# lucazanella/AnomalyCLIP

Measured on AMD Instinct MI355X. Metric: frames/sec encoded + anomaly-scored (whole node), ViT-B/16 224^2, higher is better.
Workload: dtype f32 (bf16x6 operands, exact 24-bit split, f32 accumulate); 1 GPU; configs[2]: synthetic 224x224 RGB frames, ViT-B/16 encode + selector + axial temporal head + eval post-processing; step = one 512-frame clip per GPU in ONE ViT launch, UCF-Crime head config, random-init weights; text features cached (frozen prompts): leg text_recomputed_every_step runs the text encoder in every step; leg vit_chunk_256 = the config's literal batch of 256; vit_chunk=512, precision=auto

## Files before the change

anomalyclip_amd/_lib.py:

```python
from __future__ import annotations

import ctypes as C
import os
import threading

from . import _build

c_void_p, c_int32, c_int64, c_float, c_size_t = C.c_void_p, C.c_int32, C.c_int64, C.c_float, C.c_size_t

ACX_F32, ACX_BF16, BF16X3, BF16X3P = 0, 1, 2, 3
BF16X2P, ACX_F16, F16X2P = 4, 5, 6
PREC_F32, PREC_BF16, PREC_F32X6, PREC_F32X3, PREC_F16X3 = 0, 1, 2, 3, 4
PREC_BF16X6 = 5
PREC_F32X6_LN16 = 6
PREC_F32X6_R16 = 7
ACT_NONE, ACT_QUICKGELU, ACT_LEAKYRELU, ACT_RELU, ACT_RESRELU = 0, 1, 2, 3, 4
ACT_GELU = 5
AMAP_IDENTITY, AMAP_CONV3X3, AMAP_TESTTILE, AMAP_TILETABLE = 0, 1, 2, 3
NORM_LAYER, NORM_CHAN = 0, 1
OPT_RING_MIN_TILES, OPT_SK_MAX_M, OPT_TN_P256_MIN_ROWS, OPT_X6_CUS, OPT_X6_TAIL_SPLIT = 1, 2, 3, 4, 5
OPT_X6_STRIP_TAIL, OPT_X6_MIN_TILES, OPT_LN_RIDER, OPT_ATTN_F32IN, OPT_CLS_FOLD = 6, 7, 8, 9, 10
ACX_F64, ACX_I64 = 16, 17
COMM_SUM, COMM_MAX, COMM_MIN = 0, 1, 2
COMM_ID_BYTES = 128
SAB_ROUTE_UNSUPPORTED, SAB_ROUTE_TEXT_MFMA, SAB_ROUTE_TEXT_BLOCK, SAB_ROUTE_TEXT_ROWS = 0, 1, 2, 3
SAB_ROUTE_AXIAL_MFMA, SAB_ROUTE_AXIAL_MFMA_PADDED, SAB_ROUTE_GENERIC = 4, 5, 6
AXF_ROUTE_UNSUPPORTED, AXF_ROUTE_PADDED_MFMA, AXF_ROUTE_EXACT_MFMA, AXF_ROUTE_THREAD_PER_ROW = 0, 1, 2, 3
GEMM_ROUTE_NONE, GEMM_ROUTE_X6_TAIL_SPLIT, GEMM_ROUTE_SK, GEMM_ROUTE_X6, GEMM_ROUTE_S64, GEMM_ROUTE_P256, GEMM_ROUTE_W8 = 0, 1, 2, 3, 4, 5, 6
GEMM_ROUTE_W8_CONV, GEMM_ROUTE_RING, GEMM_ROUTE_P8, GEMM_ROUTE_DMA_CONV, GEMM_ROUTE_DMA, GEMM_ROUTE_GENERIC = 7, 8, 9, 10, 11, 12
GEMM_REDUCE_NONE, GEMM_REDUCE_LAUNCH, GEMM_REDUCE_COUNTERS = 0, 1, 2
TN_ROUTE_NONE, TN_ROUTE_W8, TN_ROUTE_P256, TN_ROUTE_X6_256x256, TN_ROUTE_X6_256x128, TN_ROUTE_X6_128x256 = 0, 1, 2, 3, 4, 5
TF_LN_ROWS, TF_LN_PLANES, TF_LN_RIDDEN, TF_LN_CLS = 0, 1, 2, 3
TF_GEMM_ROWS, TF_GEMM_X6 = 0, 1
TF_BUF_NONE, TF_BUF_SPLITK, TF_BUF_H, TF_BUF_QKV, TF_BUF_MLP = 0, 1, 2, 3, 4
TF_ATT_F32, TF_ATT_BF16, TF_ATT_X3_PANEL, TF_ATT_P3N, TF_ATT_P3F, TF_ATT_CLS, TF_ATT_CLS_FOLD = 0, 1, 2, 3, 4, 5, 6


class GemmDesc(C.Structure):
    _fields_ = [
        ("A", c_void_p), ("W", c_void_p), ("C", c_void_p),
        ("M", c_int32), ("N", c_int32), ("K", c_int32),
        ("lda", c_int32), ("ldw", c_int32), ("ldc", c_int32),
        ("a_dtype", c_int32), ("c_dtype", c_int32), ("prec", c_int32),
        ("bias", c_void_p), ("act", c_int32),
        ("residual", c_void_p), ("ldr", c_int32),
        ("a_sub", c_void_p),
        ("amap", c_int32), ("gn", c_int32), ("gl", c_int32), ("cin", c_int32), ("seg", c_int32),
        ("pos0", c_void_p), ("pos1", c_void_p),
        ("workspace", c_void_p), ("workspace_bytes", c_size_t),
        ("zero_page", c_void_p), ("a_act", c_int32), ("gelu_grad_of", c_void_p), ("ldg", c_int32),
        ("a_norm_w", c_void_p), ("a_norm_b", c_void_p), ("a_norm_eps", c_float),
        ("counters", c_void_p), ("n_counters", c_int32),
        ("tile_table", c_void_p),
        ("pairs", c_int32), ("panels", c_int32), ("a_plane_stride", c_int64), ("w_plane_stride", c_int64),
        ("c_plane_rows", c_int64), ("out_scale", c_float), ("c_scale", c_float),
    ]


class GemmScratch(C.Structure):
    _fields_ = [("workspace_bytes", c_size_t), ("counters", c_int32)]


class GemmRoute(C.Structure):
    _fields_ = [("route", c_int32), ("ksplit", c_int32), ("reduce", c_int32), ("reserved", c_int32), ("tiles", c_int64)]


class GemmTnRoute(C.Structure):
    _fields_ = [(n, c_int32) for n in ("kernel", "splits", "rows_per_split", "tiles", "reduce", "clears_zero_page")]


class TfProduct(C.Structure):
    _fields_ = [(n, c_int32) for n in ("kernel", "c_dtype", "scratch", "ln_job")]


class TfLayerPlan(C.Structure):
    _fields_ = [(n, c_int32) for n in ("ln1", "ln1_dtype", "ln2", "ln2_dtype")] + \
               [(n, TfProduct) for n in ("in_proj", "out_proj", "fc", "proj")] + \
               [(n, c_int32) for n in ("att", "att_products", "split_att", "split_mlp", "pruned", "reserved")]


class LnJob(C.Structure):
    _fields_ = [("w", c_void_p), ("b", c_void_p), ("y", c_void_p), ("y_dtype", c_int32), ("eps", c_float), ("mode", c_int32),
                ("y_scale", c_float)]


class BlockWeights(C.Structure):
    _fields_ = [(n, c_void_p) for n in (
        "ln1_w", "ln1_b", "ln2_w", "ln2_b", "in_proj_w", "in_proj_b", "out_proj_w", "out_proj_b",
        "fc_w", "fc_b", "proj_w", "proj_b",
        "in_proj_w_bf16", "out_proj_w_bf16", "fc_w_bf16", "proj_w_bf16")]


class VitWeights(C.Structure):
    _fields_ = [
        ("conv1_w", c_void_p), ("conv1_w_bf16", c_void_p),
        ("class_embedding", c_void_p), ("positional_embedding", c_void_p),
        ("ln_pre_w", c_void_p), ("ln_pre_b", c_void_p), ("ln_post_w", c_void_p), ("ln_post_b", c_void_p),
        ("proj_t", c_void_p), ("proj_t_bf16", c_void_p),
# ... 15 lines not shown
    _fields_ = [("src", c_void_p), ("dst", c_void_p), ("rows", c_int32), ("cols", c_int32), ("src_ld", c_int32),
                ("dst_ld", c_int32), ("transpose", c_int32), ("reserved", c_int32)]


class VitDesc(C.Structure):
    _fields_ = [(n, c_int32) for n in ("resolution", "patch", "width", "layers", "heads", "embed_dim", "prec", "act")]


class ResnetConv(C.Structure):
    _fields_ = [("w", c_void_p), ("b", c_void_p), ("w3", c_void_p)]


class ResnetBlock(C.Structure):
    _fields_ = [("conv1", ResnetConv), ("conv2", ResnetConv), ("conv3", ResnetConv), ("downsample", ResnetConv)]


class ResnetWeights(C.Structure):
    _fields_ = [("stem", ResnetConv * 3), ("blocks", C.POINTER(ResnetBlock)), ("positional_embedding", c_void_p),
                ("q_w", c_void_p), ("q_b", c_void_p), ("kv_w", c_void_p), ("kv_b", c_void_p), ("c_w", c_void_p), ("c_b", c_void_p),
                ("kv_w3", c_void_p)]


class ResnetBn(C.Structure):
    _fields_ = [("weight", c_void_p), ("bias", c_void_p), ("running_mean", c_void_p), ("running_var", c_void_p),
                ("num_batches_tracked", c_void_p)]


class ResnetBlockBn(C.Structure):
    _fields_ = [("bn1", ResnetBn), ("bn2", ResnetBn), ("bn3", ResnetBn), ("downsample", ResnetBn)]


class ResnetTrainBn(C.Structure):
    _fields_ = [("stem", ResnetBn * 3), ("blocks", C.POINTER(ResnetBlockBn)), ("eps", c_float), ("momentum", c_float)]


class ResnetDesc(C.Structure):
    _fields_ = [("resolution", c_int32), ("width", c_int32), ("layers", c_int32 * 4), ("heads", c_int32), ("output_dim", c_int32),
                ("prec", c_int32)]


class JpegInfo(C.Structure):
    _fields_ = [(n, c_int32) for n in ("width", "height", "ncomp", "hmax", "vmax", "mcus_x", "mcus_y", "restart_interval")] + \
               [(n, c_int32 * 4) for n in ("comp_h", "comp_v", "comp_tq", "comp_td", "comp_ta", "comp_width", "comp_height",
                                           "blocks_wide", "blocks_high")] + \
               [("coef_offset", c_int64 * 4), ("coef_elems", c_int64), ("scan_offset", c_int64),
                ("qtab", (C.c_uint16 * 64) * 4), ("qtab_present", C.c_uint8 * 4), ("huff_present", (C.c_uint8 * 4) * 2),
                ("huff_bits", ((C.c_uint8 * 17) * 4) * 2), ("huff_vals", ((C.c_uint8 * 256) * 4) * 2)]


class VizGeom(C.Structure):
    _fields_ = [(n, c_int32) for n in ("Hc", "Wc", "H", "W", "fx", "fy", "fw", "fh", "border", "bx", "by", "bh", "bar_pitch", "bar_w",
                                       "C1", "sx", "sy", "sw", "sh", "cursor_w", "T")] + [("threshold", c_float)]


class JpegHuff(C.Structure):
    _fields_ = [("present", (C.c_uint8 * 4) * 2), ("bits", ((C.c_uint8 * 17) * 4) * 2), ("vals", ((C.c_uint8 * 256) * 4) * 2),
                ("td", C.c_uint8 * 4), ("ta", C.c_uint8 * 4)]


_SIGS = {
    "acx_version": (C.c_int, []),
    "acx_create": (C.c_int, [C.POINTER(c_void_p), C.c_int]),
    "acx_destroy": (None, [c_void_p]),
    "acx_last_error": (C.c_char_p, [c_void_p]),
    "acx_set_option": (C.c_int, [c_void_p, c_int32, c_int64]),
    "acx_get_option": (C.c_int, [c_void_p, c_int32, C.POINTER(c_int64)]),
    "acx_gemm": (C.c_int, [c_void_p, C.POINTER(GemmDesc), c_void_p]),
    "acx_gemm_scratch": (C.c_int, [c_void_p, C.POINTER(GemmDesc), c_int32, C.POINTER(GemmScratch)]),
    "acx_gemm_route": (C.c_int, [c_void_p, C.POINTER(GemmDesc), C.POINTER(GemmRoute)]),
    "acx_gemm_ln": (C.c_int, [c_void_p, C.POINTER(GemmDesc), C.POINTER(LnJob), c_void_p]),
    "acx_gemm_ln_plan": (c_int64, [c_int32, c_int32, c_int32, c_int32, c_int32, C.c_double, C.POINTER(c_int64)]),
    "acx_layernorm": (C.c_int, [c_void_p, c_void_p, c_int64, c_void_p, c_void_p, c_void_p, c_int64, c_int32,
                                c_int64, c_int32, c_float, c_int32, c_void_p]),
    "acx_layernorm_scaled": (C.c_int, [c_void_p, c_void_p, c_int64, c_void_p, c_void_p, c_void_p, c_int64, c_int32, c_float, c_int32,
                                       c_float, c_void_p]),
    "acx_attention": (C.c_int, [c_void_p, c_void_p, c_int64, c_void_p, c_int64, c_int32, c_int32, c_int32,
                                c_int32, c_void_p]),
    "acx_attention_bf16": (C.c_int, [c_void_p, c_void_p, c_int64, c_void_p, c_int64, c_int32, c_int32, c_int32, c_void_p]),
    "acx_attention_x3": (C.c_int, [c_void_p, c_void_p, c_int64, c_void_p, c_int64, c_int32, c_int32, c_int32, c_void_p]),
    "acx_attention_p3": (C.c_int, [c_void_p, c_void_p, c_void_p, c_int32, c_int32, c_int32, c_void_p]),
    "acx_attention_p3n": (C.c_int, [c_void_p, c_void_p, c_void_p, c_int32, c_int32, c_int32, c_int32, c_void_p]),
    "acx_attention_p3f": (C.c_int, [c_void_p, c_void_p, c_int64, c_void_p, c_int32, c_int32, c_int32, c_void_p]),
    "acx_attention_p3f16": (C.c_int, [c_void_p, c_void_p, c_int64, c_void_p, c_float, c_int32, c_int32, c_int32, c_void_p]),
    "acx_attention_x3_panel": (C.c_int, [c_void_p, c_void_p, c_int64, c_void_p, c_int64, c_int32, c_int32, c_int32, c_void_p]),
    "acx_attention_cls": (C.c_int, [c_void_p, c_void_p, c_int64, c_void_p, c_int64, c_int32, c_int32, c_int32, c_void_p]),
    "acx_attention_cls_fold_workspace_bytes": (c_size_t, [c_int32, c_int32]),
    "acx_attention_cls_fold": (C.c_int, [c_void_p, c_void_p, c_void_p, c_void_p, c_float, c_void_p, c_void_p, c_void_p, c_int64, c_void_p,
                                         c_int64, c_int32, c_int32, c_int32, c_int32, c_void_p, c_size_t, c_void_p]),
    "acx_vit_patches": (C.c_int, [c_void_p, c_void_p, c_void_p, c_int32, c_int32, c_int32, c_int32, c_void_p]),
    "acx_vit_embed": (C.c_int, [c_void_p] * 7 + [c_int32, c_int32, c_int32, c_void_p]),
    "acx_resnet_stem_im2col": (C.c_int, [c_void_p, c_void_p, c_void_p, c_int32, c_int32, c_void_p]),
    "acx_avgpool2_nhwc": (C.c_int, [c_void_p, c_void_p, c_void_p, c_int32, c_int32, c_int32, c_int32, c_void_p]),
    "acx_attnpool_tokens": (C.c_int, [c_void_p, c_void_p, c_void_p, c_void_p, c_int32, c_int32, c_int32, c_void_p]),
    "acx_resnet_workspace_bytes": (c_size_t, [C.POINTER(ResnetDesc), c_int32]),
    "acx_bn_apply_nhwc": (C.c_int, [c_void_p, c_void_p, c_void_p, c_void_p, c_void_p, c_void_p, c_void_p, c_void_p, c_int64, c_int32,
                                    c_int32, c_float, c_int32, c_void_p, c_void_p]),
    "acx_resnet_train_workspace_bytes": (c_size_t, [C.POINTER(ResnetDesc), c_int32]),
    "acx_resnet_encode_train": (C.c_int, [c_void_p, C.POINTER(ResnetDesc), C.POINTER(ResnetWeights), C.POINTER(ResnetTrainBn), c_void_p,
                                          c_int32, c_void_p, c_void_p, c_size_t, c_void_p]),
    "acx_resnet_encode": (C.c_int, [c_void_p, C.POINTER(ResnetDesc), C.POINTER(ResnetWeights), c_void_p, c_int32, c_void_p,
                                    c_void_p, c_size_t, c_void_p]),
    "acx_vit_workspace_bytes": (c_size_t, [C.POINTER(VitDesc), c_int32]),
    "acx_vit_encode": (C.c_int, [c_void_p, C.POINTER(VitDesc), C.POINTER(VitWeights), c_void_p, c_int32, c_void_p,
                                 c_void_p, c_size_t, c_void_p]),
    "acx_vit_encode_ln16": (C.c_int, [c_void_p, C.POINTER(VitDesc), C.POINTER(VitWeights), c_void_p, c_void_p, c_int32, c_void_p,
                                      c_void_p, c_size_t, c_void_p]),
    "acx_vit_encode_r16": (C.c_int, [c_void_p, C.POINTER(VitDesc), C.POINTER(VitWeights), c_void_p, c_void_p, c_int32, c_void_p,
                                     c_void_p, c_size_t, c_void_p]),
    "acx_transformer_workspace_bytes": (c_size_t, [c_int32, c_int32]),
    "acx_transformer_workspace_bytes_prec": (c_size_t, [c_int32, c_int32, c_int32]),
    "acx_transformer_forward": (C.c_int, [c_void_p, c_void_p, c_int32, c_int32, c_int32, c_int32, c_int32, c_int32,
                                          c_int32, C.POINTER(BlockWeights), c_void_p, c_size_t, c_void_p]),
    "acx_transformer_forward_act": (C.c_int, [c_void_p, c_void_p, c_int32, c_int32, c_int32, c_int32, c_int32, c_int32,
                                              c_int32, c_int32, C.POINTER(BlockWeights), c_void_p, c_size_t, c_void_p]),
    "acx_transformer_plan": (C.c_int, [c_void_p] + [c_int32] * 10 + [C.POINTER(TfLayerPlan)]),
    "acx_text_directions": (C.c_int, [c_void_p, c_void_p, c_void_p, c_void_p, c_int32, c_int32, c_int32, c_void_p]),
    "acx_selector_project": (C.c_int, [c_void_p, c_void_p, c_void_p, c_void_p, c_void_p, c_int64, c_int32, c_int32,
                                       c_void_p]),
    "acx_probe_mfma": (C.c_int, [c_void_p, c_int32, c_int32, c_int32, c_void_p, C.POINTER(C.c_double), c_void_p]),
    "acx_probe_copy": (C.c_int, [c_void_p, c_void_p, c_void_p, c_int64, c_void_p]),
    "acx_split_bf16x3_multi": (C.c_int, [c_void_p, c_int32, c_void_p, c_void_p, c_void_p, c_void_p]),
    "acx_probe_read": (C.c_int, [c_void_p, c_void_p, c_int64, c_void_p, c_void_p]),
    "acx_comm_unique_id": (C.c_int, [c_void_p, c_size_t]),
    "acx_comm_init": (C.c_int, [c_void_p, c_int32, c_int32, c_void_p]),
    "acx_comm_destroy": (C.c_int, [c_void_p]),
    "acx_comm_info": (C.c_int, [c_void_p, C.POINTER(c_int32), C.POINTER(c_int32)]),
    "acx_allreduce": (C.c_int, [c_void_p, c_void_p, c_int64, c_int32, c_int32, c_void_p]),
    "acx_allgather": (C.c_int, [c_void_p, c_void_p, c_void_p, c_int64, c_int32, c_void_p]),
    "acx_bn_workspace_bytes": (c_size_t, [c_int64, c_int32]),
    "acx_bn_combine": (C.c_int, [c_void_p, c_void_p, c_int32, c_int32, c_void_p, c_void_p, c_void_p, c_void_p, c_void_p]),
    "acx_bn_stats": (C.c_int, [c_void_p, c_void_p, c_int64, c_int32, c_void_p, c_void_p, c_void_p, c_void_p, c_size_t, c_void_p]),
    "acx_selector_project_stats": (C.c_int, [c_void_p, c_void_p, c_void_p, c_void_p, c_void_p, c_int64, c_int32, c_int32,
                                             c_void_p, c_void_p, c_void_p, c_void_p, c_size_t, c_void_p]),
    "acx_selector_bn": (C.c_int, [c_void_p, c_void_p, c_void_p, c_void_p, c_void_p, c_int64, c_int64, c_int32,
                                  c_float, c_void_p]),
    "acx_axial_attention": (C.c_int, [c_void_p, c_void_p, c_void_p, c_int32, c_int32, c_int32, c_int32, c_int32,
                                      c_int32, c_void_p]),
    "acx_axial_attention_route": (C.c_int, [c_void_p] + [c_int32] * 6),
    "acx_cls_head": (C.c_int, [c_void_p] * 8 + [c_int64, c_int32, c_int32, c_int32, c_int32, c_void_p]),
    "acx_cls_head_tiles": (C.c_int, [c_void_p] * 8 + [c_int64, c_int32, c_int32, c_int32, c_void_p, c_void_p]),
    "acx_class_probs": (C.c_int, [c_void_p, c_void_p, c_void_p, c_void_p, c_int64, c_int32, c_void_p]),
    "acx_prompt_embed": (C.c_int, [c_void_p] * 6 + [c_int32] * 6 + [c_void_p]),
    "acx_gather_rows": (C.c_int, [c_void_p, c_void_p, c_void_p, c_void_p, c_int64, c_int32, c_void_p]),
    "acx_add_bcast": (C.c_int, [c_void_p, c_void_p, c_void_p, c_void_p, c_int64, c_int64, c_void_p]),
    "acx_concat_features": (C.c_int, [c_void_p] * 5 + [c_int64, c_int32, c_int32, c_int32, c_void_p]),
    "acx_prof_enable": (C.c_int, [c_void_p, C.c_int]),
    "acx_prof_gemm_flops": (C.c_int, [c_void_p, C.POINTER(C.c_double)]),
    "acx_prof_collect": (C.c_int, [c_void_p, C.POINTER(c_int32), C.POINTER(C.c_double)]),
    "acx_prof_gemm_tn": (C.c_int, [c_void_p, C.POINTER(C.c_double), C.POINTER(C.c_double), C.POINTER(c_int32)]),
    "acx_gemm_tn_workspace_bytes": (c_size_t, [c_int32, c_int32, c_int32]),
    "acx_gemm_tn": (C.c_int, [c_void_p, c_void_p, c_int32, c_void_p, c_int32, c_void_p, c_int32, c_int32, c_int32, c_int32,
                              c_void_p, c_int32, c_int32, c_int32, c_int32, c_void_p, c_size_t, c_void_p]),
    "acx_reduce_rows": (C.c_int, [c_void_p, c_void_p, c_void_p, c_int32, c_int32, c_void_p]),
    "acx_layernorm_bwd": (C.c_int, [c_void_p] * 6 + [c_int64, c_int32, c_float, c_int32, c_float, c_void_p, c_void_p]),
    "acx_cls_head_bwd": (C.c_int, [c_void_p] * 10 + [c_int64, c_int32, c_void_p]),
    "acx_act": (C.c_int, [c_void_p, c_void_p, c_void_p, c_void_p, c_int64, c_int32, c_void_p]),
    "acx_leaky_grad_planes": (C.c_int, [c_void_p, c_void_p, c_void_p, c_void_p, c_void_p, c_int64, c_int64, c_void_p]),
    "acx_add": (C.c_int, [c_void_p, c_void_p, c_void_p, c_void_p, c_int64, c_void_p]),
    "acx_transpose": (C.c_int, [c_void_p, c_void_p, c_void_p, c_int32, c_int32, c_void_p]),
    "acx_conv_weight_dx": (C.c_int, [c_void_p, c_void_p, c_void_p, c_int32, c_int32, c_void_p]),
    "acx_seq_attention_bwd": (C.c_int, [c_void_p] * 4 + [c_int32] * 7 + [c_void_p, c_void_p]),
    "acx_seq_attention_bwd_route": (C.c_int, [c_void_p] + [c_int32] * 8),
    "acx_pos_grad": (C.c_int, [c_void_p] * 5 + [c_int32] * 4 + [c_void_p]),
    "acx_bn_bwd_stats": (C.c_int, [c_void_p] * 4 + [c_int64, c_int32, c_void_p, c_size_t, c_void_p]),
    "acx_bn_bwd_apply": (C.c_int, [c_void_p] * 6 + [c_int32, c_int64, c_int64, c_int32, c_float, c_void_p, c_void_p]),
    "acx_axpby": (C.c_int, [c_void_p, c_void_p, c_void_p, c_int32, c_float, c_float, c_void_p]),
    "acx_colsum_partials": (C.c_int, [c_void_p, c_void_p, c_int32, c_void_p, c_int64, c_int32, c_int32, c_void_p]),
    "acx_text_directions_bwd": (C.c_int, [c_void_p] * 5 + [c_int32] * 3 + [c_void_p]),
    "acx_select_idx": (C.c_int, [c_void_p] * 7 + [c_int32] * 7 + [c_void_p]),
    "acx_gather_segments": (C.c_int, [c_void_p] * 4 + [c_int32] * 5 + [c_void_p]),
    "acx_scatter_segments": (C.c_int, [c_void_p] * 4 + [c_int32] * 5 + [c_void_p]),
    "acx_mil_loss_one": (C.c_int, [c_void_p] * 13 + [c_size_t] + [c_int32] * 6 + [c_void_p, c_void_p, c_void_p, c_void_p]),
    "acx_mil_loss_bn": (C.c_int, [c_void_p] * 14 + [c_size_t, c_void_p, c_size_t] + [c_int32] * 6 + [c_void_p, c_void_p, c_void_p, c_void_p]),
    "acx_mil_loss_bn_fits": (C.c_int, [c_void_p] + [c_int32] * 5),
    "acx_selector_tail": (C.c_int, [c_void_p, c_void_p, c_void_p, c_int32] + [c_void_p] * 7 + [c_float, c_float, c_void_p, c_int64] +
                          [c_void_p] * 6 + [c_int32] * 7 + [c_float, c_void_p]),
    "acx_selector_tail_fits": (C.c_int, [c_void_p] + [c_int32] * 6),
    "acx_text_directions_bwd_parts": (C.c_int, [c_void_p] * 4 + [c_int32, c_int64, c_void_p] + [c_int32] * 3 + [c_void_p]),
    "acx_adamw": (C.c_int, [c_void_p] * 5 + [c_int64] + [c_float] * 5 + [c_int32, c_void_p]),
    "acx_multi_axpy": (C.c_int, [c_void_p, c_int32, C.POINTER(c_void_p), C.POINTER(c_void_p), C.POINTER(c_int64), c_float, c_void_p]),
    "acx_adamw_multi": (C.c_int, [c_void_p, c_int32] + [C.POINTER(c_void_p)] * 4 + [C.POINTER(c_int64), C.POINTER(C.c_double),
                                  C.POINTER(C.c_double), C.c_double, C.c_double, C.c_double, c_int32, c_void_p]),
    "acx_row_parts": (c_int64, [c_int64]),
    "acx_prep_multi": (C.c_int, [c_void_p, c_int32, c_void_p, c_void_p]),
    "acx_multi_copy": (C.c_int, [c_void_p, c_int32, C.POINTER(c_void_p), C.POINTER(c_void_p), C.POINTER(c_int64), c_void_p]),
    "acx_adamw_hyper": (C.c_int, [c_int32, C.POINTER(C.c_double), C.POINTER(C.c_double), C.c_double, C.c_double, c_int32,
                                  C.POINTER(c_float)]),
    "acx_adamw_multi_dev": (C.c_int, [c_void_p, c_int32] + [C.POINTER(c_void_p)] * 4 + [C.POINTER(c_int64), c_void_p, c_float,
                                      C.c_double, C.c_double, C.c_double, c_void_p]),
    "acx_grad_norm_workspace_bytes": (c_size_t, [c_int32, c_int64]),
    "acx_grad_norm": (C.c_int, [c_void_p, c_int32, C.POINTER(c_void_p), C.POINTER(c_int64), c_float, c_float, c_void_p, c_void_p,
# ... 147 lines not shown
```

anomalyclip_amd/components/clip_vit.py:

```python
from __future__ import annotations

import ctypes as C
import math
from typing import List, Optional

import torch
from torch import nn

from .. import _lib as L
from .. import ops

PRECISIONS = {"auto": L.PREC_F32X6, "f32": L.PREC_F32, "bf16": L.PREC_BF16, "f32x6": L.PREC_F32X6, "bf16x3": L.PREC_F32X3,
              "f16x3": L.PREC_F16X3}
F16X3_WSCALE = 1024.0
ACTS = {"quick_gelu": L.ACT_QUICKGELU, "gelu": L.ACT_GELU}


def check_act(act, precision: Optional[str] = None, arch: Optional[str] = None, key: str = "act") -> int:
    if act not in ACTS:
        raise ValueError(f"{key}={act!r}: one of {', '.join(ACTS)}")
    if act == "gelu" and precision == "bf16":
        raise ValueError(f"{key}='gelu' with precision='bf16': the exact GELU runs on the f32-accurate paths only ('auto', 'f32', 'f32x6', 'f16x3')")
    if act == "gelu" and arch is not None and str(arch).startswith("RN"):
        raise ValueError(f"{key}='gelu' with arch={arch!r}: the CLIP ResNet encoders have no GELU (the activation is the ViT MLP's)")
    return ACTS[act]


_NEW_ARCH_VISION = {(224, 32, 768), (224, 14, 1024), (336, 14, 1024)}


def check_vit_precision(precision: str, tokens: int, width: int, arch: str, resolution: int = 0, patch: int = 0):
    if precision == "bf16x6":
        raise ValueError(f"precision 'bf16x6' is a ResNet encoder precision: for {arch} 'auto' already is that arithmetic (every large "
                         "product as an f32-accurate six-product GEMM of bf16 planes); use 'auto'")
    if precision not in PRECISIONS:
        raise ValueError(f"unknown precision {precision!r}: one of {', '.join(PRECISIONS)}")
    if precision in ("bf16x3", "f16x3") and (tokens > 224 or (resolution, patch, width) in _NEW_ARCH_VISION):
        raise ValueError(f"precision {precision!r} is not available for {arch} ({tokens} tokens, width {width}): it is stated for the "
                         "ViT-B/16 geometry, whose planes attention (192 < tokens <= 208) it needs; use 'auto', 'f32' or 'bf16'")
    if tokens > 1024:
        raise ValueError(f"{arch} has {tokens} tokens per frame: the attention kernels take at most 1024")


LN16_TARGET = 2.0 ** 14
LN16_SCALE_RANGE = (2.0 ** -20, 2.0 ** 20)
LN16_WEIGHT_MAX = 2.0 ** 15 / F16X3_WSCALE


def ln16_scale(bound: float) -> Optional[float]:
    if not (math.isfinite(bound) and bound > 0.0):
        return None
    s = 2.0 ** (math.frexp(LN16_TARGET / bound)[1] - 1)
    while s * bound > LN16_TARGET:
        s *= 0.5
    return s if LN16_SCALE_RANGE[0] <= s <= LN16_SCALE_RANGE[1] else None


@torch.no_grad()
def r16_bounds(ln_w, ln_b, w, b):
    g, be, w64, b64 = ln_w.detach().double(), ln_b.detach().double(), w.detach().double(), b.detach().double()
    D = g.numel()
    l1 = (g.abs() * float(D - 1) ** 0.5 + be.abs()).max() * w64.abs().sum(1) + b64.abs()
    l2 = float(D) ** 0.5 * (w64 * g).pow(2).sum(1).sqrt() + (w64 @ be + b64).abs()
    return l1, l2


@torch.no_grad()
def _range_proofs(blocks, width: int):
    vals = []
    D = width
    root = float(D - 1) ** 0.5
    for b in blocks:
        for ln in (b.ln_1, b.ln_2):
            g, be = ln.weight.detach().double(), ln.bias.detach().double()
            vals.append((g.abs() * root + be.abs()).max())
            vals.append((g.abs() + be.abs()).sum())
        for wt in (b.attn.in_proj_weight, b.mlp.c_fc.weight):
            vals.append(wt.detach().abs().max().double())
            vals.append(wt.detach().double().abs().sum())
        for ln, wt, bias in ((b.ln_1, b.attn.in_proj_weight[2 * D:], b.attn.in_proj_bias[2 * D:]), (b.ln_2, b.mlp.c_fc.weight, b.mlp.c_fc.bias)):
            l1, l2 = r16_bounds(ln.weight, ln.bias, wt, bias)
            vals.append(torch.minimum(l1, l2).max() + 0.0 * (l1.sum() + l2.sum()))
        for wt in (b.attn.out_proj.weight, b.mlp.c_proj.weight):
            vals.append(wt.detach().abs().max().double())
            vals.append(wt.detach().double().abs().sum())
    if not vals:
        return None, None
    v = torch.stack(vals).tolist()
    ln16: Optional[List[float]] = []
    r16: Optional[List[float]] = []
    for i in range(0, len(v), 14):
        b1, f1, b2, f2, w1, g1, w2, g2, ba, bh, w3, g3, w4, g4 = v[i:i + 14]
        if ln16 is not None:
            s1, s2 = ln16_scale(b1), ln16_scale(b2)
            if not all(math.isfinite(t) for t in (f1, f2, g1, g2)) or not (w1 <= LN16_WEIGHT_MAX and w2 <= LN16_WEIGHT_MAX) or s1 is None or s2 is None:
                ln16 = r16 = None
            else:
                ln16 += [s1, s2]
        if r16 is not None:
            sa, sh = ln16_scale(ba), ln16_scale(bh)
            if not all(math.isfinite(t) for t in (g3, g4)) or not (w3 <= LN16_WEIGHT_MAX and w4 <= LN16_WEIGHT_MAX) or sa is None or sh is None:
                r16 = None
            else:
                r16 += [sa, sh]
    return ln16, r16


def ln16_scales(blocks, width: int) -> Optional[List[float]]:
    return _range_proofs(blocks, width)[0]


def r16_scales(blocks, width: int) -> Optional[List[float]]:
    return _range_proofs(blocks, width)[1]


HEAD_MAX_AXIS = 128
HEAD_DIMS = (16, 32, 64)
LAYERNORM_WIDTHS = (64, 128, 256, 512, 640, 768, 1024)


def check_head_geometry(num_segments, seg_length, emb_size, heads, dim_heads=None, num_topk=None, num_bottomk=None,
                        kernel_widths: bool = True):
    for key, v in (("num_segments", num_segments), ("seg_length", seg_length)):
        if not isinstance(v, int) or isinstance(v, bool) or v < 1 or v > HEAD_MAX_AXIS:
            raise ValueError(f"{key}={v!r}: the axial attention kernels take an integer axis length of 1 ... {HEAD_MAX_AXIS}")
    if not isinstance(heads, int) or heads < 1:
        raise ValueError(f"heads={heads!r}: need an integer >= 1")
    if kernel_widths:
        if emb_size not in LAYERNORM_WIDTHS:
            raise ValueError(f"emb_size={emb_size!r}: the LayerNorm kernels take the widths {', '.join(map(str, LAYERNORM_WIDTHS))}")
        if dim_heads:
            if dim_heads not in HEAD_DIMS:
                raise ValueError(f"dim_heads={dim_heads!r}: the attention kernels take a head dimension of 16, 32 or 64")
        elif emb_size % heads or emb_size // heads not in HEAD_DIMS:
            raise ValueError(f"heads={heads!r} with emb_size={emb_size}: the head dimension emb_size / heads = {emb_size / heads:g} must "
                             "be 16, 32 or 64 (or set dim_heads)")
    for key, v in (("num_topk", num_topk), ("num_bottomk", num_bottomk)):
        if v is not None and v > num_segments:
            raise ValueError(f"{key}={v} selects more segments than num_segments={num_segments}")


class LayerNorm(nn.Module):
    def __init__(self, width: int):
        super().__init__()
        self.weight = nn.Parameter(torch.ones(width))
        self.bias = nn.Parameter(torch.zeros(width))

    def forward(self, x: torch.Tensor) -> torch.Tensor:
        shp = x.shape
        return ops.layernorm(x.reshape(-1, shp[-1]).contiguous(), self.weight, self.bias).view(shp)


class _Linear(nn.Module):

    def __init__(self, fin: int, fout: int, bias: bool = True):
        super().__init__()
        self.weight = nn.Parameter(torch.empty(fout, fin))
        self.bias = nn.Parameter(torch.zeros(fout)) if bias else None
        nn.init.normal_(self.weight, std=fin ** -0.5)


class _MHA(nn.Module):

    def __init__(self, width: int):
        super().__init__()
        self.in_proj_weight = nn.Parameter(torch.empty(3 * width, width))
        self.in_proj_bias = nn.Parameter(torch.zeros(3 * width))
        self.out_proj = _Linear(width, width)
        nn.init.normal_(self.in_proj_weight, std=width ** -0.5)


class _MLP(nn.Module):
    def __init__(self, width: int):
        super().__init__()
        self.c_fc = _Linear(width, 4 * width)
        self.c_proj = _Linear(4 * width, width)


class ResidualAttentionBlock(nn.Module):
    def __init__(self, width: int, heads: int):
        super().__init__()
        self.attn = _MHA(width)
        self.ln_1 = LayerNorm(width)
        self.mlp = _MLP(width)
        self.ln_2 = LayerNorm(width)


class Transformer(nn.Module):

    def __init__(self, width: int, layers: int, heads: int, causal: bool = False, act: str = "quick_gelu"):
        super().__init__()
        if width != heads * 64:
            raise ValueError("libacx attention kernels are built for head dim 64 (every CLIP ViT/text tower)")
        self.width, self.layers, self.heads, self.causal = width, layers, heads, causal
        check_act(act)
        self.act = act
# ... 13 lines not shown
            w = arr[i]
            w.ln1_w, w.ln1_b = b.ln_1.weight.data_ptr(), b.ln_1.bias.data_ptr()
            w.ln2_w, w.ln2_b = b.ln_2.weight.data_ptr(), b.ln_2.bias.data_ptr()
            w.in_proj_w, w.in_proj_b = b.attn.in_proj_weight.data_ptr(), b.attn.in_proj_bias.data_ptr()
            w.out_proj_w, w.out_proj_b = b.attn.out_proj.weight.data_ptr(), b.attn.out_proj.bias.data_ptr()
            w.fc_w, w.fc_b = b.mlp.c_fc.weight.data_ptr(), b.mlp.c_fc.bias.data_ptr()
            w.proj_w, w.proj_b = b.mlp.c_proj.weight.data_ptr(), b.mlp.c_proj.bias.data_ptr()
            mixed = prec in (L.PREC_F32X6_LN16, L.PREC_F32X6_R16)
            f16w = {"in_proj_w_bf16": mixed, "fc_w_bf16": mixed and ln16_fc, "out_proj_w_bf16": prec == L.PREC_F32X6_R16 and r16[0],
                    "proj_w_bf16": prec == L.PREC_F32X6_R16 and r16[1]}
            if prec in (L.PREC_BF16, L.PREC_F32X6, L.PREC_F32X3, L.PREC_F16X3, L.PREC_F32X6_LN16, L.PREC_F32X6_R16):
                for name, p in (("in_proj_w_bf16", b.attn.in_proj_weight), ("out_proj_w_bf16", b.attn.out_proj.weight),
                                ("fc_w_bf16", b.mlp.c_fc.weight), ("proj_w_bf16", b.mlp.c_proj.weight)):
                    if prec == L.PREC_F16X3 or f16w[name]:
                        t = ops.split_f16x2(p.detach(), panel=True, scale=F16X3_WSCALE)
                    else:
                        t = ops.cast_bf16(p.detach()) if prec == L.PREC_BF16 else ops.split_bf16x3(p.detach(), panel=True)
                    keep.append(t)
                    setattr(w, name, t.data_ptr())
        self._cache = (key, (arr, keep))
        return self._cache[1]

    def forward_(self, x: torch.Tensor, batch: int, seq: int, prec: int = L.PREC_F32) -> torch.Tensor:
        assert x.is_contiguous() and x.dtype == torch.float32 and x.shape == (batch * seq, self.width)
        lib = L.lib()
        nbytes = lib.acx_transformer_workspace_bytes_prec(self.width, batch * seq, prec)
        ws = torch.empty(nbytes, dtype=torch.uint8, device=x.device)
        arr, _keep = self.block_table(prec)
        h = ops._h(x)
        L.check(lib.acx_transformer_forward_act(h, x.data_ptr(), batch, seq, self.width, self.heads, self.layers,
                                                int(self.causal), prec, ACTS[self.act], arr, ws.data_ptr(), nbytes, ops._stream()), h)
        return x


class _Conv(nn.Module):
    def __init__(self, width: int, patch: int):
        super().__init__()
        self.weight = nn.Parameter(torch.empty(width, 3, patch, patch))
        nn.init.normal_(self.weight, std=(3 * patch * patch) ** -0.5)


class VisionTransformer(nn.Module):

    def __init__(self, input_resolution: int, patch_size: int, width: int, layers: int, heads: int,
                 output_dim: int, precision: str = "auto", chunk: int = 512, streams: int = 1, arch: Optional[str] = None,
                 act: str = "quick_gelu"):
        super().__init__()
        self.arch = arch or f"ViT(width {width}, patch {patch_size}, resolution {input_resolution})"
        check_act(act, precision)
        self.act = act
        self.input_resolution, self.patch_size, self.output_dim = input_resolution, patch_size, output_dim
        self.width, self.layers, self.heads = width, layers, heads
        self.conv1 = _Conv(width, patch_size)
        scale = width ** -0.5
        self.class_embedding = nn.Parameter(scale * torch.randn(width))
        self.positional_embedding = nn.Parameter(scale * torch.randn((input_resolution // patch_size) ** 2 + 1, width))
        self.ln_pre = LayerNorm(width)
        self.transformer = Transformer(width, layers, heads, act=act)
        self.ln_post = LayerNorm(width)
        self.proj = nn.Parameter(scale * torch.randn(width, output_dim))
        self.precision = precision
        self.check_precision()
        self.chunk = chunk
        self.streams = streams
        self._wcache = None
        self._ln16 = None
        self._ws: Optional[torch.Tensor] = None
        self._ws2: Optional[torch.Tensor] = None
        self._side = None

    @property
    def tokens(self) -> int:
        return (self.input_resolution // self.patch_size) ** 2 + 1

    def check_precision(self):
        check_vit_precision(self.precision, self.tokens, self.width, self.arch, self.input_resolution, self.patch_size)
        check_act(self.act, self.precision)

    @torch.no_grad()
    def f16x3_range_report(self) -> dict:
        D = self.width
        lim = 65504.0
        worst = {"weight_planes": 0.0, "layernorm_out": 0.0, "attention_out": 0.0, "mlp_hidden": 0.0}

        def ln_bound(ln):
            return float((ln.weight.abs() * (D - 1) ** 0.5 + ln.bias.abs()).max())
        mats = [self.conv1.weight.reshape(D, -1)]
        for b in self.transformer.resblocks:
            l1, l2 = ln_bound(b.ln_1), ln_bound(b.ln_2)
            wv, bv = b.attn.in_proj_weight[2 * D:], b.attn.in_proj_bias[2 * D:]
            worst["layernorm_out"] = max(worst["layernorm_out"], l1, l2)
            worst["attention_out"] = max(worst["attention_out"], float((wv.abs().sum(1) * l1 + bv.abs()).max()))
            worst["mlp_hidden"] = max(worst["mlp_hidden"], float((b.mlp.c_fc.weight.abs().sum(1) * l2 + b.mlp.c_fc.bias.abs()).max()))
            mats += [b.attn.in_proj_weight, b.attn.out_proj.weight, b.mlp.c_fc.weight, b.mlp.c_proj.weight]
        worst["weight_planes"] = F16X3_WSCALE * max(float(m.abs().max()) for m in mats)
        margin = min(lim / max(v, 1e-30) for v in worst.values())
        return {"bounds": worst, "fp16_max": lim, "margin": margin, "safe": margin > 1.0}

    def _ln16_bound(self):
        key = (ops.WEIGHT_EPOCH[0],) + tuple((p.data_ptr(), p._version) for p in self.parameters())
        if self._ln16 is not None and self._ln16[0] == key:
            return self._ln16[1]
        res = None
        if self.width in (768, 1024) and self.layers > 1 and L.exports("acx_vit_encode_ln16"):
            scales, wide = _range_proofs(self.transformer.resblocks, self.width)
            if scales is not None:
                fc16 = ops.transformer_plan(64, 197, 768, 12, 2, prec=L.PREC_F32X6_LN16, prune_last=True)[0]["ln2_dtype"] == L.F16X2P
                r16 = None
                if wide is not None and L.exports("acx_vit_encode_r16"):
                    rec = ops.transformer_plan(64, self.tokens, self.width, self.heads, 2, prec=L.PREC_F32X6_R16, prune_last=True)[0]
                    fmt = (rec["reserved"] == L.F16X2P, rec["fc"]["c_dtype"] == L.F16X2P)
                    if any(fmt):
                        s4 = [t for l in range(self.layers) for t in (scales[2 * l], scales[2 * l + 1], wide[2 * l], wide[2 * l + 1])]
                        r16 = (s4, (C.c_float * len(s4))(*s4), fmt)
                res = (scales, (C.c_float * len(scales))(*scales), fc16, r16)
        self._ln16 = (key, res)
        return res

    def ln16_resolution(self) -> Optional[List[float]]:
        res = self._ln16_bound()
        return None if res is None else res[0]

    def r16_resolution(self) -> Optional[List[float]]:
        res = self._ln16_bound()
        return None if res is None or res[3] is None else res[3][0]

    def _weights(self, prec: int, ln16_fc: bool = True, r16=(True, True)):
        key = (prec, bool(ln16_fc), bool(r16[0]), bool(r16[1]), ops.WEIGHT_EPOCH[0]) + tuple((p.data_ptr(), p._version) for p in self.parameters())
        if self._wcache is not None and self._wcache[0] == key:
            return self._wcache[1]
        keep = []
        w = L.VitWeights()
        conv = self.conv1.weight.detach().reshape(self.width, -1).contiguous()
        proj_t = self.proj.detach().t().contiguous()
        keep += [conv, proj_t]
        w.conv1_w, w.proj_t = conv.data_ptr(), proj_t.data_ptr()
        if prec == L.PREC_BF16:
            cb, pb = ops.cast_bf16(conv), ops.cast_bf16(proj_t)
            keep += [cb, pb]
            w.conv1_w_bf16, w.proj_t_bf16 = cb.data_ptr(), pb.data_ptr()
        elif prec in (L.PREC_F32X6, L.PREC_F32X3, L.PREC_F16X3, L.PREC_F32X6_LN16, L.PREC_F32X6_R16) and self.patch_size % 4 == 0:
            cb = ops.split_f16x2(conv, panel=True, scale=F16X3_WSCALE) if prec == L.PREC_F16X3 else ops.split_bf16x3(conv, panel=True)
            keep.append(cb)
            w.conv1_w_bf16 = cb.data_ptr()
        w.class_embedding = self.class_embedding.data_ptr()
        w.positional_embedding = self.positional_embedding.data_ptr()
        w.ln_pre_w, w.ln_pre_b = self.ln_pre.weight.data_ptr(), self.ln_pre.bias.data_ptr()
        w.ln_post_w, w.ln_post_b = self.ln_post.weight.data_ptr(), self.ln_post.bias.data_ptr()
        arr, keep2 = self.transformer.block_table(prec, ln16_fc, r16)
        w.blocks = C.cast(arr, C.POINTER(L.BlockWeights))
        keep += [arr, keep2]
        self._wcache = (key, (w, keep))
        return self._wcache[1]

    @torch.no_grad()
    def forward(self, x: torch.Tensor) -> torch.Tensor:
        assert x.dim() == 4 and x.shape[1] == 3 and x.shape[2] == x.shape[3] == self.input_resolution
        self.check_precision()
        x = x.contiguous().float()
        prec = PRECISIONS[self.precision]
        lib = L.lib()
        bound = self._ln16_bound() if self.precision == "auto" and x.is_cuda else None
        ln16_fc, r16 = True, (True, True)
        if bound is not None and bound[3] is not None:
            prec = L.PREC_F32X6_R16
            ln16_fc = bound[2]
            _s4, sc4, r16 = bound[3]
            encode = lambda *a: lib.acx_vit_encode_r16(a[0], a[1], a[2], sc4, *a[3:])
        elif bound is not None:
            prec = L.PREC_F32X6_LN16
            _scales, sc, ln16_fc, _ = bound
            encode = lambda *a: lib.acx_vit_encode_ln16(a[0], a[1], a[2], sc, *a[3:])
        else:
            encode = lib.acx_vit_encode
        d = L.VitDesc(self.input_resolution, self.patch_size, self.width, self.layers, self.heads, self.output_dim, prec, ACTS[self.act])
        w, _keep = self._weights(prec, ln16_fc, r16)
        F = x.shape[0]
        out = torch.empty(F, self.output_dim, dtype=torch.float32, device=x.device)
        chunk = min(self.chunk, F)
        nbytes = lib.acx_vit_workspace_bytes(C.byref(d), chunk)
        if self._ws is None or self._ws.numel() < nbytes or self._ws.device != x.device:
            self._ws = torch.empty(nbytes, dtype=torch.uint8, device=x.device)
        h = ops._h(x)
        if self.streams == 2 and chunk >= 32 and x.is_cuda:
            return self._forward_two_streams(x, out, d, w, chunk, nbytes, h, encode)
        s = ops._stream()
        for f0 in range(0, F, chunk):
            n = min(chunk, F - f0)
            L.check(encode(h, C.byref(d), C.byref(w), x[f0:f0 + n].data_ptr(), n, out[f0:f0 + n].data_ptr(),
                           self._ws.data_ptr(), self._ws.numel(), s), h)
        return out

    def _forward_two_streams(self, x, out, d, w, chunk, nbytes, h, encode):
        F = x.shape[0]
        half = (chunk + 1) // 2
        if self._ws2 is None or self._ws2.numel() < nbytes or self._ws2.device != x.device:
            self._ws2 = torch.empty(nbytes, dtype=torch.uint8, device=x.device)
        if self._side is None or self._side[0].device != x.device:
            s0 = torch.cuda.Stream(device=x.device)
            self._side = (s0, ops.side_stream_beside(s0, x.device))
        cur = torch.cuda.current_stream()
        wss = (self._ws, self._ws2)
        for st in self._side:
            st.wait_stream(cur)
        k = 0
        for f0 in range(0, F, half):
            n = min(half, F - f0)
            st, ws = self._side[k % 2], wss[k % 2]
            with torch.cuda.stream(st):
                L.check(encode(h, C.byref(d), C.byref(w), x[f0:f0 + n].data_ptr(), n, out[f0:f0 + n].data_ptr(),
                               ws.data_ptr(), ws.numel(), st.cuda_stream), h)
            k += 1
        for st in self._side:
            cur.wait_stream(st)
        return out
```

anomalyclip_amd/csrc/acx_api.hip:

```cpp
#include "acx_internal.h"

#include <new>
#include <stdlib.h>

#ifndef ACX_ATTN_F32IN_DEFAULT
#define ACX_ATTN_F32IN_DEFAULT 1
#endif

#ifndef ACX_LN16_FC_DEFAULT
#define ACX_LN16_FC_DEFAULT 1
#endif

#ifndef ACX_R16_OUT_DEFAULT
#define ACX_R16_OUT_DEFAULT 1
#endif
#ifndef ACX_R16_PROJ_DEFAULT
#define ACX_R16_PROJ_DEFAULT 1
#endif

#ifndef ACX_CLS_FOLD_DEFAULT
#define ACX_CLS_FOLD_DEFAULT 1
#endif

thread_local char acx_tls_err[512] = {0};

namespace {
struct TfOpts {
  int x6_min_tiles;
  bool attn_f32in, cls_fold;
  bool ln16_fc;
  bool r16_out, r16_proj;
};
constexpr TfOpts kCreateOpts = {18, ACX_ATTN_F32IN_DEFAULT != 0, ACX_CLS_FOLD_DEFAULT != 0, ACX_LN16_FC_DEFAULT != 0, ACX_R16_OUT_DEFAULT != 0,
                                ACX_R16_PROJ_DEFAULT != 0};
constexpr TfOpts kNoCtxOpts = {512, false, false, ACX_LN16_FC_DEFAULT != 0, ACX_R16_OUT_DEFAULT != 0, ACX_R16_PROJ_DEFAULT != 0};
inline TfOpts tf_opts(const acx_ctx* ctx, bool query) {
  if (!ctx) return query ? kCreateOpts : kNoCtxOpts;
  return {ctx->opt_x6_min_tiles, ctx->opt_attn_f32in != 0, ctx->opt_cls_fold != 0, kCreateOpts.ln16_fc, kCreateOpts.r16_out, kCreateOpts.r16_proj};
}
}

extern "C" int acx_attention_cls(acx_ctx* ctx, const float* qkv, int64_t ldqkv, float* out, int64_t ldo, int32_t batch,
                                 int32_t L, int32_t heads, void* stream);

extern "C" int acx_version(void) { return ACX_VERSION; }

extern "C" int acx_create(acx_ctx** out, int device) {
  if (!out) return acx_fail(nullptr, ACX_E_BADARG, "acx_create: null out%s");
  int n = 0;
  hipError_t e = hipGetDeviceCount(&n);
  if (e != hipSuccess || device < 0 || device >= n) {
    snprintf(acx_tls_err, 512, "acx_create: device %d not available (%s, %d devices)", device,
             e == hipSuccess ? "ok" : hipGetErrorString(e), n);
    return ACX_E_HIP;
  }
  hipDeviceProp_t prop;
  e = hipGetDeviceProperties(&prop, device);
  if (e != hipSuccess) {
    snprintf(acx_tls_err, 512, "acx_create: hipGetDeviceProperties: %s", hipGetErrorString(e));
    return ACX_E_HIP;
  }
  if (strncmp(prop.gcnArchName, "gfx950", 6) != 0) {
    snprintf(acx_tls_err, 512, "acx_create: libacx is built for gfx950 only, device %d is %s", device, prop.gcnArchName);
    return ACX_E_UNSUPPORTED;
  }
  acx_ctx* c = new (std::nothrow) acx_ctx;
  if (!c) return acx_fail(nullptr, ACX_E_HIP, "acx_create: out of host memory%s");
  c->device = device;
  c->multiprocessors = prop.multiProcessorCount;
  c->opt_ring_min_tiles = 512;
  c->opt_sk_max_m = 320;
  c->opt_tn_p256_min_rows = 4096;
  c->opt_x6_cus = 0;
  c->opt_x6_tail = 0;
  c->opt_x6_strip = 1;
  c->opt_ln_rider = 1;
  c->opt_attn_f32in = kCreateOpts.attn_f32in;
  c->opt_cls_fold = kCreateOpts.cls_fold;
  c->comm = nullptr; c->comm_rank = 0; c->comm_world = 0;
  c->opt_x6_min_tiles = kCreateOpts.x6_min_tiles;
  c->err[0] = 0;
  c->prof_on = false;
  c->prof_gemm_only = false;
  c->prof_n = c->prof_created = 0;
  c->prof_gemm_flops = 0.0;
  c->prof_tn_flops = c->prof_tn_ms = 0.0; c->prof_tn_count = 0;
  c->prof_ev = new (std::nothrow) hipEvent_t[2 * ACX_PROF_MAX];
  c->prof_kind = new (std::nothrow) unsigned char[ACX_PROF_MAX];
  *out = c;
  return ACX_OK;
}

extern "C" void acx_destroy(acx_ctx* ctx) {
  if (!ctx) return;
  for (int i = 0; i < 2 * ctx->prof_created; ++i) (void)hipEventDestroy(ctx->prof_ev[i]);
  delete[] ctx->prof_ev;
  delete[] ctx->prof_kind;
  delete ctx;
}

extern "C" int acx_prof_enable(acx_ctx* ctx, int on) {
  if (!ctx || !ctx->prof_ev || !ctx->prof_kind) return acx_fail(ctx, ACX_E_BADARG, "acx_prof_enable: no context%s");
  ctx->prof_on = on != 0;
  ctx->prof_gemm_only = on == 2;
  if (on) { ctx->prof_n = 0; ctx->prof_gemm_flops = 0.0; ctx->prof_tn_flops = 0.0; }
  return ACX_OK;
}

extern "C" int acx_prof_gemm_flops(acx_ctx* ctx, double* flops) {
  if (!ctx || !flops) return acx_fail(ctx, ACX_E_BADARG, "acx_prof_gemm_flops: null pointer%s");
  *flops = ctx->prof_gemm_flops;
  return ACX_OK;
}

extern "C" int acx_prof_gemm_tn(acx_ctx* ctx, double* flops, double* total_ms, int32_t* launches) {
  if (!ctx || !flops || !total_ms || !launches) return acx_fail(ctx, ACX_E_BADARG, "acx_prof_gemm_tn: null pointer%s");
  *flops = ctx->prof_tn_flops; *total_ms = ctx->prof_tn_ms; *launches = ctx->prof_tn_count;
  return ACX_OK;
}

extern "C" int acx_prof_collect(acx_ctx* ctx, int32_t* counts, double* total_ms) {
// ... 15 lines not shown
  }
  ctx->prof_n = 0;
  return ACX_OK;
}

extern "C" int acx_set_option(acx_ctx* ctx, int32_t option, int64_t value) {
  if (!ctx) return acx_fail(ctx, ACX_E_BADARG, "acx_set_option: no context%s");
  switch (option) {
    case ACX_OPT_RING_MIN_TILES:
      if (value < 1) return acx_fail(ctx, ACX_E_BADARG, "acx_set_option: ring_min_tiles must be >= 1%s");
      ctx->opt_ring_min_tiles = (int)value;
      return ACX_OK;
    case ACX_OPT_TN_P256_MIN_ROWS:
      if (value < 1) return acx_fail(ctx, ACX_E_BADARG, "acx_set_option: tn_p256_min_rows must be >= 1%s");
      ctx->opt_tn_p256_min_rows = (int)(value > 0x7fffffff ? 0x7fffffff : value);
      return ACX_OK;
    case ACX_OPT_X6_TAIL_SPLIT:
      ctx->opt_x6_tail = value != 0;
      return ACX_OK;
    case ACX_OPT_X6_STRIP_TAIL:
      if (value < 0 || value > 3) return acx_fail(ctx, ACX_E_BADARG, "acx_set_option: x6_strip_tail is 0 (off), 1 (cost model), 2 or 3 (forced strip width)%s");
      ctx->opt_x6_strip = (int)value;
      return ACX_OK;
    case ACX_OPT_LN_RIDER:
      if (value < 0) return acx_fail(ctx, ACX_E_BADARG, "acx_set_option: ln_rider is 0 (off), 1 (cost model) or a row count%s");
      ctx->opt_ln_rider = (long long)value;
      return ACX_OK;
    case ACX_OPT_ATTN_F32IN:
      ctx->opt_attn_f32in = value != 0;
      return ACX_OK;
    case ACX_OPT_CLS_FOLD:
      ctx->opt_cls_fold = value != 0;
      return ACX_OK;
    case ACX_OPT_X6_MIN_TILES:
      if (value < 1) return acx_fail(ctx, ACX_E_BADARG, "acx_set_option: x6_min_tiles must be >= 1%s");
      ctx->opt_x6_min_tiles = (int)(value > 0x7fffffff ? 0x7fffffff : value);
      return ACX_OK;
    case ACX_OPT_X6_CUS:
      if (value < 0) return acx_fail(ctx, ACX_E_BADARG, "acx_set_option: x6_cus must be >= 0%s");
      ctx->opt_x6_cus = (int)(value > 4096 ? 4096 : value);
      return ACX_OK;
    case ACX_OPT_SK_MAX_M:
      if (value < 0) return acx_fail(ctx, ACX_E_BADARG, "acx_set_option: sk_max_m must be >= 0%s");
      ctx->opt_sk_max_m = (int)value;
      return ACX_OK;
    default:
      return acx_fail(ctx, ACX_E_UNSUPPORTED, "acx_set_option: unknown option %s%ld", "", (long)option);
  }
}

extern "C" int acx_get_option(acx_ctx* ctx, int32_t option, int64_t* value) {
  if (!ctx || !value) return acx_fail(ctx, ACX_E_BADARG, "acx_get_option: no context or no result pointer%s");
  switch (option) {
    case ACX_OPT_RING_MIN_TILES: *value = ctx->opt_ring_min_tiles; return ACX_OK;
    case ACX_OPT_SK_MAX_M: *value = ctx->opt_sk_max_m; return ACX_OK;
    case ACX_OPT_TN_P256_MIN_ROWS: *value = ctx->opt_tn_p256_min_rows; return ACX_OK;
    case ACX_OPT_X6_CUS: *value = ctx->opt_x6_cus; return ACX_OK;
    case ACX_OPT_X6_TAIL_SPLIT: *value = ctx->opt_x6_tail; return ACX_OK;
    case ACX_OPT_X6_STRIP_TAIL: *value = ctx->opt_x6_strip; return ACX_OK;
    case ACX_OPT_X6_MIN_TILES: *value = ctx->opt_x6_min_tiles; return ACX_OK;
    case ACX_OPT_LN_RIDER: *value = ctx->opt_ln_rider; return ACX_OK;
    case ACX_OPT_ATTN_F32IN: *value = ctx->opt_attn_f32in; return ACX_OK;
    case ACX_OPT_CLS_FOLD: *value = ctx->opt_cls_fold; return ACX_OK;
    default:
      return acx_fail(ctx, ACX_E_UNSUPPORTED, "acx_get_option: unknown option %s%ld", "", (long)option);
  }
}

extern "C" const char* acx_last_error(acx_ctx* ctx) { return ctx ? ctx->err : acx_tls_err; }

namespace {

inline size_t al(size_t x) { return (x + 255) & ~(size_t)255; }

struct TfWs {
  char *h, *qkv, *att, *mlp, *splitk;
  char *hp, *mp;
  char* qkv3;
  size_t splitk_bytes, total;
};

static inline bool is_xmode(int prec) {
  return prec == ACX_PREC_F32X6 || prec == ACX_PREC_F32X3 || prec == ACX_PREC_F16X3 || prec == ACX_PREC_F32X6_LN16 ||
         prec == ACX_PREC_F32X6_R16;
}
static inline bool is_ln16(int prec) { return prec == ACX_PREC_F32X6_LN16 || prec == ACX_PREC_F32X6_R16; }
struct XMode {
  int pairs;
  bool f16;
};
static inline XMode xmode_of(int prec) { return {(prec == ACX_PREC_F32X3 || prec == ACX_PREC_F16X3) ? 3 : 6, prec == ACX_PREC_F16X3}; }
static inline int plane_dtype_of(int prec) { return prec == ACX_PREC_F16X3 ? ACX_F16X2P : prec == ACX_PREC_F32X3 ? ACX_BF16X2P : ACX_BF16X3P; }

TfWs carve_tf(char* base, int64_t rows, int W, int prec = ACX_PREC_F32) {
  TfWs w;
  size_t off = 0;
  w.h = base + off;   off += al((size_t)rows * W * 4);
  w.qkv = base + off; off += al((size_t)rows * 3 * W * 4);
  w.att = base + off; off += al((size_t)rows * W * 4);
  w.mlp = base + off; off += al((size_t)rows * 4 * W * 4);
  w.splitk_bytes = rows <= 4096 ? (size_t)8 * rows * 4 * W * 4 : (size_t)4 * 256 * 128 * 128 * 4;
  w.splitk = base + off; off += al(w.splitk_bytes);
  w.hp = w.mp = w.qkv3 = nullptr;
  if (is_xmode(prec)) {
    w.hp = base + off; off += al((size_t)3 * rows * W * 2);
    w.mp = base + off; off += al((size_t)3 * rows * 4 * W * 2);
    w.qkv3 = base + off; off += al((size_t)3 * rows * 3 * W * 2);
  }
  w.total = off;
  return w;
}

struct ClsWs {
  float *xc, *attc, *x1;
  char *hc, *mc;
};
inline size_t cls_ws_bytes(int batch, int W) { return (size_t)8 * batch * W * 4; }
ClsWs carve_cls(float* base, int batch, int W) {
  const size_t n = (size_t)batch * W;
  return {base, base + n, base + 2 * n, (char*)(base + 3 * n), (char*)(base + 4 * n)};
}

bool x6_takes(const TfOpts& o, bool planes_ws, int64_t M, int N, int K, int lda) {
  if (!planes_ws || !ACX_DBG_SWITCH("X6", true)) return false;
  const int64_t rtiles = ((M + 255) / 256) * ((N + 255) / 256);
  return rtiles >= o.x6_min_tiles && K % 256 == 0 && N % 8 == 0 && (size_t)M * lda * 2 < ((size_t)1 << 32) &&
         (size_t)N * K * 2 < ((size_t)1 << 32);
}

struct Product {
  int kernel;
  const void* A; int a_dtype, lda;
  const float* Wf;
  const void* Wb;
  int64_t w_plane_bytes;
  int ldw, M, N, K;
  const float* bias; int act;
  const float* residual; int ldr;
  void* C; int c_dtype, ldc;
  void* scratch; size_t scratch_bytes;
  const acx_ln_job* ln;
  float a_scale;
  float c_scale;
};

struct TfMode {
  int prec;
  int hdt, pdt;
  XMode xm;
};

int missing_weights(acx_ctx* ctx, bool planes, int prec) {
  if (planes) return acx_fail(ctx, ACX_E_BADARG, "driver: missing bf16 x 3 weight planes for ACX_PREC_F32X6%s");
  return acx_fail(ctx, ACX_E_BADARG, "driver: missing %s weight copy for the requested precision", prec == ACX_PREC_BF16 ? "bf16" : "f32");
}

acx_gemm_desc desc_of(const Product& p) {
  acx_gemm_desc d;
  memset(&d, 0, sizeof(d));
  d.A = p.A; d.C = p.C;
  d.M = p.M; d.N = p.N; d.K = p.K; d.lda = p.lda; d.ldw = p.ldw; d.ldc = p.ldc;
  d.a_dtype = p.a_dtype; d.c_dtype = p.c_dtype;
  d.bias = p.bias; d.act = p.act; d.residual = p.residual; d.ldr = p.ldr ? p.ldr : p.ldc;
  return d;
}

int run_x6(acx_ctx* ctx, XMode xm, const Product& p, hipStream_t s) {
  acx_gemm_desc d = desc_of(p);
  d.W = p.Wb;
  if (p.a_scale > 0.f) xm = {3, true};
  d.a_dtype = xm.f16 ? ACX_F16 : ACX_BF16; d.prec = ACX_PREC_BF16; d.pairs = xm.pairs; d.panels = 3;
  d.out_scale = p.a_scale > 0.f ? 1.f / (ACX_F16X3_WSCALE * p.a_scale) : xm.f16 ? 1.f / ACX_F16X3_WSCALE : 0.f;
  d.c_scale = p.c_scale;
  d.a_plane_stride = (int64_t)p.M * p.lda * 2;
  d.w_plane_stride = p.w_plane_bytes ? p.w_plane_bytes : (int64_t)p.N * p.K * 2;
  d.workspace = p.scratch; d.workspace_bytes = p.scratch ? p.scratch_bytes : 0;
  return p.ln ? acx_gemm_ln(ctx, &d, p.ln, s) : acx_gemm(ctx, &d, s);
}

int run_rows1(acx_ctx* ctx, int prec, const Product& p, hipStream_t s) {
  acx_gemm_desc d = desc_of(p);
  d.W = prec == ACX_PREC_BF16 ? p.Wb : (const void*)p.Wf;
  if (!d.W) return missing_weights(ctx, false, prec);
  d.prec = prec;
  d.workspace = p.scratch_bytes ? p.scratch : nullptr; d.workspace_bytes = p.scratch_bytes;
  return acx_gemm(ctx, &d, s);
}

int run_rows(acx_ctx* ctx, int prec, const Product& p, hipStream_t s) {
  bool tail_split = ACX_DBG_SWITCH("TAIL_SPLIT", true);
  if (tail_split && !p.ldr) {
    acx_gemm_desc d = desc_of(p);
    d.prec = prec;
    if (acx_gemm_takes_strip_stream(&d)) tail_split = false;
  }
  const int tiles_n = (p.N + 127) / 128, tiles_m = (p.M + 127) / 128;
  const long tiles = (long)tiles_m * tiles_n;
  const long full = tiles / 512;
  const long rem = tiles - full * 512;
  if (tail_split && p.scratch && full >= 2 && rem > 0 && rem <= 256 && !p.ldr) {
    const int head_rows = (int)((full * 512) / tiles_n) * 128;
    const int tail_rows = p.M - head_rows;
    if (head_rows > 0 && tail_rows > 0 && (size_t)4 * tail_rows * p.N * sizeof(float) <= p.scratch_bytes) {
      const size_t asz = p.a_dtype == ACX_BF16 ? 2 : 4, csz = p.c_dtype == ACX_BF16 ? 2 : 4;
      Product head = p, tail = p;
      head.M = head_rows; head.scratch = nullptr; head.scratch_bytes = 0;
      tail.M = tail_rows;
      tail.A = (const char*)p.A + (size_t)head_rows * p.lda * asz;
      tail.C = (char*)p.C + (size_t)head_rows * p.ldc * csz;
      if (p.residual) tail.residual = p.residual + (size_t)head_rows * p.ldc;
      if (prec == ACX_PREC_F32) { tail.scratch = nullptr; tail.scratch_bytes = 0; }
      const int rc = run_rows1(ctx, prec, head, s);
      return rc ? rc : run_rows1(ctx, prec, tail, s);
    }
  }
  return run_rows1(ctx, prec, p, s);
}

int run(acx_ctx* ctx, const TfMode& m, const Product& p, hipStream_t s) {
  return p.kernel == ACX_TF_GEMM_X6 ? run_x6(ctx, m.xm, p, s) : run_rows(ctx, m.prec, p, s);
}

struct TfGeom {
  int batch, L, W, heads, layers, causal, prec;
  bool prune;
  bool planes_ws;
  int act;
};

int tf_act(acx_ctx* ctx, const char* who, int32_t given, int prec, int* act) {
  if (given != 0 && given != ACX_ACT_QUICKGELU && given != ACX_ACT_GELU)
    return acx_fail(ctx, ACX_E_BADARG, "%s: act must be 0 / ACX_ACT_QUICKGELU or ACX_ACT_GELU", who);
  if (given == ACX_ACT_GELU && prec == ACX_PREC_BF16)
    return acx_fail(ctx, ACX_E_UNSUPPORTED, "%s: ACX_ACT_GELU with ACX_PREC_BF16 (the bf16 MFMA routes are no parity path)", who);
  *act = given == ACX_ACT_GELU ? ACX_ACT_GELU : ACX_ACT_QUICKGELU;
  return ACX_OK;
}
struct TfHave { bool f32[4], alt[4]; };
struct TfPlan {
  TfMode mode;
  bool ln16_qkv, ln16_fc;
  bool r16_out, r16_proj;
  acx_tf_layer_plan_t body, before_pruned, pruned;
  bool prune;
};

acx_tf_layer_plan_t tf_layer(const TfPlan& p, int l, int layers) {
  acx_tf_layer_plan_t r = p.prune && l == layers - 1 ? p.pruned : p.prune && l == layers - 2 ? p.before_pruned : p.body;
  if (l == 0 && r.ln1 == ACX_TF_LN_RIDDEN) r.ln1 = ACX_TF_LN_PLANES;
  if (l == layers - 1) r.proj.ln_job = 0;
  return r;
}

inline acx_tf_product_t tf_rows(int c_dtype, int scratch) { return {ACX_TF_GEMM_ROWS, c_dtype, scratch, 0}; }
inline acx_tf_product_t tf_x6(int c_dtype, int scratch, bool ln_job) { return {ACX_TF_GEMM_X6, c_dtype, scratch, ln_job ? 1 : 0}; }

int tf_plan(acx_ctx* err, const TfGeom& g, const TfHave& have, const TfOpts& o, TfPlan* p) {
  memset(p, 0, sizeof(*p));
  const int W = g.W, L = g.L;
  const int64_t rows = (int64_t)g.batch * L;
  const bool xmode = is_xmode(g.prec);
  TfMode& m = p->mode;
  m.xm = xmode_of(g.prec);
  m.pdt = plane_dtype_of(g.prec);
  m.prec = xmode ? ACX_PREC_F32 : g.prec;
  m.hdt = m.prec == ACX_PREC_BF16 ? ACX_BF16 : ACX_F32;
  p->prune = g.prune;
  const int cpl = m.xm.f16 ? ACX_F16X2P : ACX_BF16X3P;
  auto x6 = [&](int N, int K) { return xmode && x6_takes(o, g.planes_ws, rows, N, K, K); };
  const bool x6_qkv = x6(3 * W, W), x6_out = x6(W, W), x6_fc = x6(4 * W, W), x6_proj = x6(W, 4 * W), x6_kv = x6(2 * W, W);
  const bool ln_ride = m.pdt == ACX_BF16X3P;
  const bool ln16 = is_ln16(g.prec), r16 = g.prec == ACX_PREC_F32X6_R16;
  if (ln16 && W != 768 && W != 1024)
    return acx_fail(err, ACX_E_UNSUPPORTED, "driver: %s is built for widths 768 and 1024", r16 ? "ACX_PREC_F32X6_R16" : "ACX_PREC_F32X6_LN16");
  p->ln16_qkv = ln16 && x6_qkv;
  p->ln16_fc = ln16 && x6_fc && o.ln16_fc;
  const bool ab = m.prec == ACX_PREC_BF16 && !g.causal && L <= 224 && ACX_DBG_SWITCH("ATTN_BF16", true);
  const bool att_p3 = x6_qkv && x6_out && !g.causal && L > 192 && L <= 208 && ACX_DBG_SWITCH("ATTN_P3", true);
  p->r16_out = r16 && o.r16_out && att_p3;
  p->r16_proj = r16 && o.r16_proj && p->ln16_fc && x6_proj;
  const bool att_p3f = att_p3 && ln_ride && (o.attn_f32in || p->r16_out);
  const bool qkv_planes = att_p3 && !att_p3f;
  const bool att_x3 = x6_out && !g.causal && L > 128 && L <= 1024 && (L > 224 || ACX_DBG_SWITCH("ATTN16", true));
  const bool cls_fold = g.prune && m.prec != ACX_PREC_BF16 && o.cls_fold && L <= 1024 &&
                        acx_attention_cls_fold_workspace_bytes(g.batch, g.heads) <= (size_t)rows * 3 * W * 4;
  const bool kv_planes = g.prune && !cls_fold && x6_kv;

  auto need = [&](bool planes, int i) { return (planes || m.prec == ACX_PREC_BF16 ? have.alt[i] : have.f32[i]) ? 0 : missing_weights(err, planes, m.prec); };
  int rc;
  if (g.layers > (g.prune ? 1 : 0)) {
    if ((rc = need(x6_qkv, 0))) return rc;
    if (m.xm.f16 && (x6_qkv || x6_out || x6_fc || x6_proj) && !(att_p3 && x6_fc && x6_proj))
      return acx_fail(err, ACX_E_UNSUPPORTED, "driver: ACX_PREC_F16X3 needs the planes attention (192 < L <= 208) and all four products on the plane kernel%s");
    if ((rc = need(x6_out, 1)) || (rc = need(x6_fc, 2)) || (rc = need(x6_proj, 3))) return rc;
  }
  if (g.prune && g.layers > 0) {
    if (kv_planes && (rc = need(true, 0))) return rc;
    for (int i = 0; i < 4; ++i) if ((rc = need(false, i))) return rc;
  }

  acx_tf_layer_plan_t& b = p->body;
  b.ln1 = !x6_qkv ? ACX_TF_LN_ROWS : ln_ride && x6_proj ? ACX_TF_LN_RIDDEN : ACX_TF_LN_PLANES;
  b.ln1_dtype = p->ln16_qkv ? ACX_F16X2P : x6_qkv ? m.pdt : m.hdt;
  b.in_proj = !x6_qkv ? tf_rows(ab ? ACX_BF16 : ACX_F32, ACX_TF_BUF_SPLITK)
                      : qkv_planes ? tf_x6(cpl, ACX_TF_BUF_QKV, false) : tf_x6(ACX_F32, ACX_TF_BUF_H, false);
  b.att = ab ? ACX_TF_ATT_BF16 : att_p3f ? ACX_TF_ATT_P3F : att_p3 ? ACX_TF_ATT_P3N : att_x3 ? ACX_TF_ATT_X3_PANEL : ACX_TF_ATT_F32;
  b.att_products = b.att == ACX_TF_ATT_P3N ? (m.xm.f16 ? 103 : m.xm.pairs) : 0;
  b.att_out_dtype = p->r16_out ? ACX_F16X2P : 0;
  b.split_att = x6_out && !att_x3 && !att_p3;
  b.out_proj = x6_out ? tf_x6(ACX_F32, ACX_TF_BUF_H, ln_ride && x6_fc) : tf_rows(ACX_F32, ACX_TF_BUF_SPLITK);
  b.ln2 = !x6_fc ? ACX_TF_LN_ROWS : b.out_proj.ln_job ? ACX_TF_LN_RIDDEN : ACX_TF_LN_PLANES;
  b.ln2_dtype = p->ln16_fc ? ACX_F16X2P : x6_fc ? m.pdt : m.hdt;
  b.fc = !x6_fc ? tf_rows(m.hdt, ACX_TF_BUF_SPLITK) : x6_proj ? tf_x6(p->r16_proj ? ACX_F16X2P : cpl, ACX_TF_BUF_MLP, false) : tf_x6(ACX_F32, ACX_TF_BUF_H, false);
  b.split_mlp = x6_proj && !x6_fc;
  b.proj = x6_proj ? tf_x6(ACX_F32, ACX_TF_BUF_H, ln_ride && x6_qkv) : tf_rows(ACX_F32, ACX_TF_BUF_SPLITK);
  p->before_pruned = b;
  p->before_pruned.proj.ln_job = x6_proj && ln_ride && kv_planes;

  acx_tf_layer_plan_t& c = p->pruned;
  c.pruned = 1;
  c.ln1 = cls_fold ? ACX_TF_LN_CLS : !kv_planes ? ACX_TF_LN_ROWS : p->before_pruned.proj.ln_job ? ACX_TF_LN_RIDDEN : ACX_TF_LN_PLANES;
  c.ln1_dtype = kv_planes ? (p->ln16_qkv ? ACX_F16X2P : m.pdt) : m.hdt;
  c.in_proj = kv_planes ? tf_x6(ACX_F32, ACX_TF_BUF_NONE, false) : tf_rows(ACX_F32, ACX_TF_BUF_NONE);
  c.att = cls_fold ? ACX_TF_ATT_CLS_FOLD : ACX_TF_ATT_CLS;
  c.out_proj = c.proj = tf_rows(ACX_F32, ACX_TF_BUF_NONE);
  c.ln2 = ACX_TF_LN_CLS;
  c.ln2_dtype = m.hdt;
  c.fc = tf_rows(m.hdt, ACX_TF_BUF_NONE);
  return ACX_OK;
}

int tf_plan_call(acx_ctx* ctx, const TfGeom& g, const acx_block_weights* blk, TfPlan* p) {
  TfHave have;
  for (int i = 0; i < 4; ++i) have.f32[i] = have.alt[i] = true;
  for (int l = 0; l < g.layers; ++l) {
    const void* f32[4] = {blk[l].in_proj_w, blk[l].out_proj_w, blk[l].fc_w, blk[l].proj_w};
    const void* alt[4] = {blk[l].in_proj_w_bf16, blk[l].out_proj_w_bf16, blk[l].fc_w_bf16, blk[l].proj_w_bf16};
    for (int i = 0; i < 4; ++i) { have.f32[i] &= f32[i] != nullptr; have.alt[i] &= alt[i] != nullptr; }
  }
  return tf_plan(ctx, g, have, tf_opts(ctx, false), p);
}

struct TfRun {
  acx_ctx* ctx; const TfGeom& g; const TfMode& m; const TfWs& ws; hipStream_t s;
  const float* ln_scales;
  int64_t rows() const { return (int64_t)g.batch * g.L; }
  bool r16() const { return g.prec == ACX_PREC_F32X6_R16; }
  float lnsc(int dtype, int l, int which) const { return is_ln16(g.prec) && dtype == ACX_F16X2P ? ln_scales[(r16() ? 4 : 2) * l + which] : 0.f; }
  float r16sc(int dtype, int l, int which) const { return r16() && dtype == ACX_F16X2P ? ln_scales[4 * l + which] : 0.f; }

  Product product(const acx_block_weights& b, int i, const acx_tf_product_t& r, int64_t M) const {
    const int W = g.W;
    Product p;
    memset(&p, 0, sizeof(p));
    p.kernel = r.kernel; p.c_dtype = r.c_dtype; p.M = (int)M;
    switch (i) {
      case 0: p.Wf = b.in_proj_w; p.Wb = b.in_proj_w_bf16; p.bias = b.in_proj_b; p.N = 3 * W; p.K = W; break;
      case 1: p.Wf = b.out_proj_w; p.Wb = b.out_proj_w_bf16; p.bias = b.out_proj_b; p.N = W; p.K = W; break;
      case 2: p.Wf = b.fc_w; p.Wb = b.fc_w_bf16; p.bias = b.fc_b; p.N = 4 * W; p.K = W; p.act = g.act; break;
      default: p.Wf = b.proj_w; p.Wb = b.proj_w_bf16; p.bias = b.proj_b; p.N = W; p.K = 4 * W; break;
    }
    p.lda = p.ldw = p.K; p.ldc = p.N; p.a_dtype = m.hdt;
    const size_t f = (size_t)rows() * W * 4;
    switch (r.scratch) {
      case ACX_TF_BUF_SPLITK: p.scratch = ws.splitk; p.scratch_bytes = ws.splitk_bytes; break;
      case ACX_TF_BUF_H: p.scratch = ws.h; p.scratch_bytes = f; break;
      case ACX_TF_BUF_QKV: p.scratch = ws.qkv; p.scratch_bytes = 3 * f; break;
      case ACX_TF_BUF_MLP: p.scratch = ws.mlp; p.scratch_bytes = 4 * f; break;
      default: break;
    }
    return p;
  }
  int norm(const float* x, int64_t ldx, const float* w, const float* b, void* y, int64_t ldy, int dtype, int64_t n, float sc = 0.f) const {
    if (sc > 0.f) return acx_layernorm_rows(ctx, x, ldx, w, b, y, dtype, sc, n, 0, g.W, 1e-5f, ACX_NORM_LAYER, s);
    return acx_layernorm(ctx, x, ldx, w, b, y, ldy, dtype, n, g.W, 1e-5f, ACX_NORM_LAYER, s);
  }
  int norm_all(int kind, int dtype, const float* x, const float* w, const float* b, float sc) const {
    if (kind == ACX_TF_LN_RIDDEN) return ACX_OK;
    return norm(x, g.W, w, b, kind == ACX_TF_LN_PLANES ? ws.hp : ws.h, g.W, dtype, rows(), kind == ACX_TF_LN_PLANES ? sc : 0.f);
  }
  acx_ln_job job(const float* w, const float* b, float sc = 0.f) const {
    return {w, b, ws.hp, sc > 0.f ? ACX_F16X2P : m.pdt, 1e-5f, ACX_NORM_LAYER, sc};
  }
  int go(const Product& p) const { return run(ctx, m, p, s); }

  int body(const acx_tf_layer_plan_t& r, const acx_block_weights& b, const acx_block_weights* next, float* x, int l, int next_ln1_dtype) const {
    const int W = g.W, batch = g.batch, L = g.L, heads = g.heads;
    auto planes = [](const acx_tf_product_t& q) { return q.c_dtype != ACX_F32 && q.c_dtype != ACX_BF16; };
    const float sc1 = lnsc(r.ln1_dtype, l, 0), sc2 = lnsc(r.ln2_dtype, l, 1);
    const float s_att = r16sc(r.att_out_dtype, l, 2), s_hid = r16sc(r.fc.c_dtype, l, 3);
    int rc;
    if ((rc = norm_all(r.ln1, r.ln1_dtype, x, b.ln1_w, b.ln1_b, sc1))) return rc;
    Product p = product(b, 0, r.in_proj, rows());
    p.a_scale = r.in_proj.kernel == ACX_TF_GEMM_X6 ? sc1 : 0.f;
    p.A = r.in_proj.kernel == ACX_TF_GEMM_X6 ? ws.hp : ws.h;
    p.C = planes(r.in_proj) ? ws.qkv3 : ws.qkv;
    if ((rc = go(p))) return rc;
    switch (r.att) {
      case ACX_TF_ATT_BF16: rc = acx_attention_bf16(ctx, ws.qkv, 3 * W, ws.att, W, batch, L, heads, s); break;
      case ACX_TF_ATT_P3F:
        rc = s_att > 0.f ? acx_attention_p3f16(ctx, (const float*)ws.qkv, 3 * W, ws.hp, s_att, batch, L, heads, s)
                         : acx_attention_p3f(ctx, (const float*)ws.qkv, 3 * W, ws.hp, batch, L, heads, s);
        break;
      case ACX_TF_ATT_P3N: rc = acx_attention_p3n(ctx, ws.qkv3, ws.hp, batch, L, heads, r.att_products, s); break;
      case ACX_TF_ATT_X3_PANEL: rc = acx_attention_x3_panel(ctx, (const float*)ws.qkv, 3 * W, ws.hp, W, batch, L, heads, s); break;
      default: rc = acx_attention(ctx, (const float*)ws.qkv, 3 * W, (float*)ws.att, W, batch, L, heads, g.causal, s); break;
    }
    if (rc) return rc;
    if (r.split_att && (rc = acx_split_bf16x3_panel(ctx, (const float*)ws.att, W, ws.hp, rows() * W * 2, rows(), W, s))) return rc;
    const acx_ln_job ln2 = job(b.ln2_w, b.ln2_b, sc2);
    p = product(b, 1, r.out_proj, rows());
    p.a_scale = r.out_proj.kernel == ACX_TF_GEMM_X6 ? s_att : 0.f;
    p.A = r.out_proj.kernel == ACX_TF_GEMM_X6 ? ws.hp : ws.att;
    p.a_dtype = r.att == ACX_TF_ATT_BF16 ? ACX_BF16 : ACX_F32;
    p.C = x; p.residual = x;
    p.ln = r.out_proj.ln_job ? &ln2 : nullptr;
    if ((rc = go(p))) return rc;
    if ((rc = norm_all(r.ln2, r.ln2_dtype, x, b.ln2_w, b.ln2_b, sc2))) return rc;
    p = product(b, 2, r.fc, rows());
    p.a_scale = r.fc.kernel == ACX_TF_GEMM_X6 ? sc2 : 0.f;
    p.c_scale = s_hid;
    p.A = r.fc.kernel == ACX_TF_GEMM_X6 ? ws.hp : ws.h;
    p.C = planes(r.fc) ? ws.mp : ws.mlp;
    if ((rc = go(p))) return rc;
    if (r.split_mlp && (rc = acx_split_bf16x3_panel(ctx, (const float*)ws.mlp, 4 * W, ws.mp, rows() * 4 * W * 2, rows(), 4 * W, s))) return rc;
    const acx_ln_job ln1 = r.proj.ln_job ? job(next->ln1_w, next->ln1_b, lnsc(next_ln1_dtype, l + 1, 0)) : job(nullptr, nullptr);
    p = product(b, 3, r.proj, rows());
    p.a_scale = r.proj.kernel == ACX_TF_GEMM_X6 ? s_hid : 0.f;
    p.A = r.proj.kernel == ACX_TF_GEMM_X6 ? ws.mp : ws.mlp;
    p.C = x; p.residual = x;
    p.ln = r.proj.ln_job ? &ln1 : nullptr;
    return go(p);
  }

  int pruned(const acx_tf_layer_plan_t& r, const acx_block_weights& b, const float* x, const ClsWs& c, int l) const {
    const int W = g.W, batch = g.batch, L = g.L;
    const float sc1 = lnsc(r.ln1_dtype, l, 0);
    int rc;
    Product p = product(b, 0, r.in_proj, rows());
    if (r.att == ACX_TF_ATT_CLS_FOLD) {
      if ((rc = norm(x, (int64_t)L * W, b.ln1_w, b.ln1_b, c.hc, W, r.ln1_dtype, batch))) return rc;
      p.M = batch; p.N = W;
      p.A = c.hc;
      p.C = c.mc; p.ldc = W;
      if ((rc = go(p))) return rc;
      if ((rc = acx_attention_cls_fold(ctx, x, b.ln1_w, b.ln1_b, 1e-5f, b.in_proj_w, b.in_proj_b, (const float*)c.mc, W, c.attc, W, batch, L, W,
                                       g.heads, ws.qkv, (size_t)rows() * 3 * W * 4, s))) return rc;
    } else {
      if ((rc = norm_all(r.ln1, r.ln1_dtype, x, b.ln1_w, b.ln1_b, sc1))) return rc;
      p.N = 2 * W; p.bias = b.in_proj_b + W;
      p.C = (float*)ws.qkv + W; p.ldc = 3 * W;
      if (r.in_proj.kernel == ACX_TF_GEMM_X6) {
        if ((rc = norm(x, (int64_t)L * W, b.ln1_w, b.ln1_b, ws.h, (int64_t)L * W, m.hdt, batch))) return rc;
        p.A = ws.hp; p.a_scale = sc1;
        p.Wb = (const char*)b.in_proj_w_bf16 + (size_t)W * 64;
        p.w_plane_bytes = (int64_t)3 * W * W * 2;
      } else {
        p.A = ws.h;
        p.Wf = b.in_proj_w + (size_t)W * W;
        p.Wb = b.in_proj_w_bf16 ? (const char*)b.in_proj_w_bf16 + (size_t)W * W * 2 : nullptr;
      }
      if ((rc = go(p))) return rc;
      Product q = product(b, 0, tf_rows(ACX_F32, ACX_TF_BUF_NONE), batch);
      q.N = W;
      q.A = ws.h; q.lda = L * W;
      q.C = ws.qkv; q.ldc = L * 3 * W;
      if ((rc = go(q))) return rc;
      if ((rc = acx_attention_cls(ctx, (const float*)ws.qkv, 3 * W, c.attc, W, batch, L, g.heads, s))) return rc;
    }
    p = product(b, 1, r.out_proj, batch);
    p.A = c.attc; p.a_dtype = ACX_F32;
    p.C = c.x1; p.residual = x; p.ldr = L * W;
    if ((rc = go(p))) return rc;
    if ((rc = norm(c.x1, W, b.ln2_w, b.ln2_b, c.hc, W, r.ln2_dtype, batch))) return rc;
    p = product(b, 2, r.fc, batch);
    p.A = c.hc;
    p.C = c.mc;
    if ((rc = go(p))) return rc;
    p = product(b, 3, r.proj, batch);
    p.A = c.mc;
    p.C = c.xc; p.residual = c.x1;
    return go(p);
  }
};

int transformer_layers(acx_ctx* ctx, float* x, const TfGeom& g, const TfPlan& plan, const acx_block_weights* blk, const TfWs& ws,
                       hipStream_t s, float* cls_ws = nullptr, const float* ln_scales = nullptr) {
  if (g.prec == ACX_PREC_F32X6_LN16) {
    if (!ln_scales) return acx_fail(ctx, ACX_E_BADARG, "driver: ACX_PREC_F32X6_LN16 needs the LayerNorm plane scales (acx_vit_encode_ln16)%s");
    for (int i = 0; i < 2 * g.layers; ++i) {
      int e = 0;
      const float sc = ln_scales[i];
      if (!(sc >= 0x1p-20f && sc <= 0x1p20f) || frexpf(sc, &e) != 0.5f)
        return acx_fail(ctx, ACX_E_BADARG, "driver: ACX_PREC_F32X6_LN16: a LayerNorm plane scale is not a power of two in [2^-20, 2^20]%s");
    }
  }
  if (g.prec == ACX_PREC_F32X6_R16) {
    if (!ln_scales) return acx_fail(ctx, ACX_E_BADARG, "driver: ACX_PREC_F32X6_R16 needs the plane scales (acx_vit_encode_r16)%s");
    for (int i = 0; i < 4 * g.layers; ++i) {
      int e = 0;
      const float sc = ln_scales[i];
      if (!(sc >= 0x1p-20f && sc <= 0x1p20f) || frexpf(sc, &e) != 0.5f)
        return acx_fail(ctx, ACX_E_BADARG, "driver: ACX_PREC_F32X6_R16: a plane scale is not a power of two in [2^-20, 2^20]%s");
    }
  }
  const TfRun exec = {ctx, g, plan.mode, ws, s, ln_scales};
  for (int l = 0; l < g.layers; ++l) {
    const acx_tf_layer_plan_t r = tf_layer(plan, l, g.layers);
    const int next_ln1 = l + 1 < g.layers ? tf_layer(plan, l + 1, g.layers).ln1_dtype : 0;
    const int rc = r.pruned ? exec.pruned(r, blk[l], x, carve_cls(cls_ws, g.batch, g.W), l)
                            : exec.body(r, blk[l], l + 1 < g.layers ? &blk[l + 1] : nullptr, x, l, next_ln1);
    if (rc) return rc;
  }
  return ACX_OK;
}

}

extern "C" size_t acx_transformer_workspace_bytes(int32_t width, int32_t rows) {
  return carve_tf(nullptr, rows, width).total;
}
extern "C" size_t acx_transformer_workspace_bytes_prec(int32_t width, int32_t rows, int32_t prec) {
  return carve_tf(nullptr, rows, width, prec).total;
}

extern "C" int acx_transformer_plan(const acx_ctx* ctx, int32_t batch, int32_t L, int32_t width, int32_t heads, int32_t layers,
                                    int32_t causal, int32_t prec, int32_t prune_last, int32_t has_weight_planes,
                                    int32_t workspace_is_prec_sized, acx_tf_layer_plan_t* out) {
  acx_ctx* err = const_cast<acx_ctx*>(ctx);
  if (!out || batch <= 0 || L <= 0 || layers < 0) return acx_fail(err, ACX_E_BADARG, "acx_transformer_plan: no result array or an empty geometry%s");
  memset(out, 0, sizeof(*out) * layers);
  const TfGeom g = {batch, L, width, heads, layers, causal, prec, prune_last != 0, is_xmode(prec) && workspace_is_prec_sized, ACX_ACT_QUICKGELU};
  const bool alt = has_weight_planes != 0;
  const TfHave have = {{true, true, true, true}, {alt, alt, alt, alt}};
  TfPlan plan;
  const int rc = tf_plan(err, g, have, tf_opts(ctx, true), &plan);
  for (int l = 0; !rc && l < layers; ++l) out[l] = tf_layer(plan, l, layers);
  return rc;
}

extern "C" int acx_transformer_forward(acx_ctx* ctx, float* x, int32_t batch, int32_t L, int32_t width, int32_t heads,
                                       int32_t layers, int32_t causal, int32_t prec, const acx_block_weights* blocks,
                                       void* workspace, size_t workspace_bytes, void* stream) {
  return acx_transformer_forward_act(ctx, x, batch, L, width, heads, layers, causal, prec, ACX_ACT_QUICKGELU, blocks, workspace, workspace_bytes, stream);
}

extern "C" int acx_transformer_forward_act(acx_ctx* ctx, float* x, int32_t batch, int32_t L, int32_t width, int32_t heads,
                                           int32_t layers, int32_t causal, int32_t prec, int32_t act, const acx_block_weights* blocks,
                                           void* workspace, size_t workspace_bytes, void* stream) {
  if (!x || !blocks || !workspace) return acx_fail(ctx, ACX_E_BADARG, "acx_transformer_forward: null pointer%s");
  int mlp_act = 0, rc0;
  if ((rc0 = tf_act(ctx, "acx_transformer_forward", act, prec, &mlp_act))) return rc0;
  if (width != heads * 64) return acx_fail(ctx, ACX_E_UNSUPPORTED, "acx_transformer_forward: head dim must be 64%s");
  TfWs ws = carve_tf((char*)workspace, (int64_t)batch * L, width, prec);
  if (ws.total > workspace_bytes && is_xmode(prec)) ws = carve_tf((char*)workspace, (int64_t)batch * L, width);
  if (ws.total > workspace_bytes) return acx_fail(ctx, ACX_E_WORKSPACE, "acx_transformer_forward: workspace too small%s");
  const TfGeom g = {batch, L, width, heads, layers, causal, prec, false, ws.hp != nullptr, mlp_act};
  TfPlan plan;
  const int rc = tf_plan_call(ctx, g, blocks, &plan);
  return rc ? rc : transformer_layers(ctx, x, g, plan, blocks, ws, (hipStream_t)stream);
}

namespace {
struct VitWs {
  char *patches, *patch_out, *x, *cls, *cls_ws;
  size_t tf_off, total;
};
VitWs carve_vit(char* base, const acx_vit_desc* d, int F) {
  const int g = d->resolution / d->patch, T = g * g, W = d->width;
  const int K = 3 * d->patch * d->patch;
  VitWs w;
  size_t off = 0;
  w.patches = base + off;   off += al((size_t)F * T * K * (is_xmode(d->prec) ? 6 : 4));
  w.patch_out = base + off; off += al((size_t)F * T * W * 4);
  w.x = base + off;         off += al((size_t)F * (T + 1) * W * 4);
  w.cls = base + off;       off += al((size_t)F * W * 4);
  w.cls_ws = base + off;    off += al(cls_ws_bytes(F, W));
  w.tf_off = off;
  off += carve_tf(nullptr, (int64_t)F * (T + 1), W, d->prec).total;
  w.total = off;
  return w;
}
}

extern "C" size_t acx_vit_workspace_bytes(const acx_vit_desc* d, int32_t frames) {
  if (!d || frames <= 0) return 0;
  return carve_vit(nullptr, d, frames).total;
}

static int vit_encode(acx_ctx* ctx, const acx_vit_desc* d, const acx_vit_weights* w, const float* ln_scales, const float* frames,
                      int32_t nframes, float* features, void* workspace, size_t workspace_bytes, void* stream) {
  if (!d || !w || !frames || !features || !workspace) return acx_fail(ctx, ACX_E_BADARG, "acx_vit_encode: null pointer%s");
  if (d->prec == ACX_PREC_F32X6_LN16 && !ln_scales)
    return acx_fail(ctx, ACX_E_BADARG, "acx_vit_encode: ACX_PREC_F32X6_LN16 needs the LayerNorm plane scales (acx_vit_encode_ln16)%s");
  if (d->prec == ACX_PREC_F32X6_R16 && !ln_scales)
    return acx_fail(ctx, ACX_E_BADARG, "acx_vit_encode: ACX_PREC_F32X6_R16 needs the plane scales (acx_vit_encode_r16)%s");
  int mlp_act = 0, rc0;
  if ((rc0 = tf_act(ctx, "acx_vit_encode", d->act, d->prec, &mlp_act))) return rc0;
  if (nframes <= 0) return ACX_OK;
  if (d->width != d->heads * 64) return acx_fail(ctx, ACX_E_UNSUPPORTED, "acx_vit_encode: head dim must be 64%s");
  if (d->patch <= 0 || d->resolution % d->patch || d->patch % 2)
    return acx_fail(ctx, ACX_E_BADARG, "acx_vit_encode: bad patch geometry (need resolution %% patch == 0 and an even patch)%s");
  const int g = d->resolution / d->patch, T = g * g, W = d->width, F = nframes;
  const int K = 3 * d->patch * d->patch;
  if (T + 1 > 1024)
    return acx_fail(ctx, ACX_E_UNSUPPORTED, "acx_vit_encode: %s%ld tokens per frame, the attention kernels take at most 1024", "", (long)(T + 1));
  const VitWs ws = carve_vit((char*)workspace, d, F);
  if (ws.total > workspace_bytes) return acx_fail(ctx, ACX_E_WORKSPACE, "acx_vit_encode: workspace too small%s");
  hipStream_t s = (hipStream_t)stream;
  const TfWs tf = carve_tf((char*)workspace + ws.tf_off, (int64_t)F * (T + 1), W, d->prec);
  const bool prune = ACX_DBG_SWITCH("VIT_PRUNE", true);
  const TfGeom geom = {F, T + 1, W, d->heads, d->layers, 0, d->prec, prune, tf.hp != nullptr, mlp_act};
  TfPlan plan;
  int rc;
  if ((rc = tf_plan_call(ctx, geom, w->blocks, &plan))) return rc;
  const TfMode& m = plan.mode;
  Product p;
  memset(&p, 0, sizeof(p));
  p.A = ws.patches; p.lda = K;
  p.Wf = w->conv1_w; p.Wb = w->conv1_w_bf16; p.ldw = K;
  p.M = F * T; p.N = W; p.K = K;
  p.C = ws.patch_out; p.c_dtype = ACX_F32; p.ldc = W;
  if (is_xmode(d->prec) && w->conv1_w_bf16 && K % 32 == 0 && x6_takes(tf_opts(ctx, false), tf.hp != nullptr, (int64_t)F * T, W, K, K)) {
    p.kernel = ACX_TF_GEMM_X6;
    p.a_dtype = m.pdt;
    p.scratch = tf.qkv; p.scratch_bytes = (size_t)F * (T + 1) * 3 * W * 4;
  } else {
    p.kernel = ACX_TF_GEMM_ROWS;
    p.a_dtype = d->patch % 4 ? ACX_F32 : m.hdt;
  }
  if ((rc = acx_vit_patches(ctx, frames, ws.patches, p.a_dtype, F, d->resolution, d->patch, s))) return rc;
  if ((rc = p.kernel == ACX_TF_GEMM_X6 ? run_x6(ctx, m.xm, p, s) : run_rows(ctx, p.a_dtype == ACX_BF16 ? ACX_PREC_BF16 : ACX_PREC_F32, p, s))) return rc;
  if ((rc = acx_vit_embed(ctx, (const float*)ws.patch_out, w->class_embedding, w->positional_embedding, w->ln_pre_w,
                          w->ln_pre_b, (float*)ws.x, F, T, W, s))) return rc;
  if ((rc = transformer_layers(ctx, (float*)ws.x, geom, plan, w->blocks, tf, s, (float*)ws.cls_ws, ln_scales))) return rc;
  if ((rc = acx_layernorm(ctx, prune ? (const float*)ws.cls_ws : (const float*)ws.x, prune ? (int64_t)W : (int64_t)(T + 1) * W,
                          w->ln_post_w, w->ln_post_b, ws.cls, W, ACX_F32, F, W, 1e-5f, ACX_NORM_LAYER, s))) return rc;
  memset(&p, 0, sizeof(p));
  p.A = ws.cls; p.a_dtype = ACX_F32; p.lda = W;
  p.Wf = w->proj_t; p.Wb = w->proj_t_bf16; p.ldw = W;
  p.M = F; p.N = d->embed_dim; p.K = W;
  p.C = features; p.c_dtype = ACX_F32; p.ldc = d->embed_dim;
  return run_rows(ctx, m.prec, p, s);
}


extern "C" int acx_vit_encode(acx_ctx* ctx, const acx_vit_desc* d, const acx_vit_weights* w, const float* frames,
                              int32_t nframes, float* features, void* workspace, size_t workspace_bytes, void* stream) {
  return vit_encode(ctx, d, w, nullptr, frames, nframes, features, workspace, workspace_bytes, stream);
}

extern "C" int acx_vit_encode_ln16(acx_ctx* ctx, const acx_vit_desc* d, const acx_vit_weights* w, const float* ln_scales, const float* frames,
                                   int32_t nframes, float* features, void* workspace, size_t workspace_bytes, void* stream) {
  if (!d || d->prec != ACX_PREC_F32X6_LN16 || !ln_scales)
    return acx_fail(ctx, ACX_E_BADARG, "acx_vit_encode_ln16: needs desc->prec = ACX_PREC_F32X6_LN16 and the LayerNorm plane scales%s");
  return vit_encode(ctx, d, w, ln_scales, frames, nframes, features, workspace, workspace_bytes, stream);
}

extern "C" int acx_vit_encode_r16(acx_ctx* ctx, const acx_vit_desc* d, const acx_vit_weights* w, const float* scales, const float* frames,
                                  int32_t nframes, float* features, void* workspace, size_t workspace_bytes, void* stream) {
  if (!d || d->prec != ACX_PREC_F32X6_R16 || !scales)
    return acx_fail(ctx, ACX_E_BADARG, "acx_vit_encode_r16: needs desc->prec = ACX_PREC_F32X6_R16 and the plane scales%s");
  return vit_encode(ctx, d, w, scales, frames, nframes, features, workspace, workspace_bytes, stream);
}
```

anomalyclip_amd/csrc/acx_attn.hip:

```cpp
#include "acx_internal.h"

#include <stdlib.h>

namespace {
#include "acx_attn_f32.h"
#include "acx_attn_p3.h"
#include "acx_attn_bf16.h"
#include "acx_attn_cls.h"
}

static int attention_impl(acx_ctx* ctx, const float* qkv, int64_t ldqkv, float* out, int64_t ldo,
                          int32_t batch, int32_t L, int32_t heads, int32_t causal, void* stream, int x3) {
  if (!qkv || !out) return acx_fail(ctx, ACX_E_BADARG, "acx_attention: null pointer%s");
  if (batch <= 0) return ACX_OK;
  if (L <= 0 || L > (causal ? 224 : 1024) || heads <= 0)
    return acx_fail(ctx, ACX_E_UNSUPPORTED, "acx_attention: need 0 < L <= 224 (causal) or 0 < L <= 1024 (non-causal)%s");
  if (L > 224 && !ctx) return acx_fail(ctx, ACX_E_UNSUPPORTED, "acx_attention: L > 224 needs a context%s");
  if (ldqkv % 4 || ((uintptr_t)qkv & 15)) return acx_fail(ctx, ACX_E_BADARG, "acx_attention: qkv must be 16-byte aligned, ld%%4==0%s");
  const int nt = (L + 31) / 32;
  const bool nw4 = ACX_DBG_SWITCH("ATTN_NW4", false);
  const dim3 grid((unsigned)(batch * heads));
  hipStream_t s = (hipStream_t)stream;
  AcxProfScope prof__(ctx, ACX_K_ATTN, (hipStream_t)stream);
  if (!causal && L > 128 && ldo % 4 == 0 && !((uintptr_t)out & 15) && (L > 224 || ACX_DBG_SWITCH("ATTN16", true))) {
    const int nqb = L > 256 ? ((L + 15) / 16 + 15) / 16 : 1;
    const int nitems = batch * heads * nqb;
    const int ncu = ctx && ctx->multiprocessors > 0 ? ctx->multiprocessors : 256;
    const int slots = 2 * ncu;
    const dim3 grid16((unsigned)(nitems < slots ? nitems : slots));
    const int64_t x3plane = x3 ? (int64_t)batch * L * ldo : (int64_t)0, prows = x3 == 2 ? (int64_t)batch * L : (int64_t)0;
    if (nqb == 1)
      hipLaunchKernelGGL(attn16_kernel<false>, grid16, dim3(512), 2 * A16_STAGE_B, s, qkv, ldqkv, out, ldo, L, heads, nitems, x3plane, prows);
    else
      hipLaunchKernelGGL(attn16_kernel<true>, grid16, dim3(512), 2 * A16_STAGE_B, s, qkv, ldqkv, out, ldo, L, heads, nitems, x3plane, prows);
    ACX_CHECK_LAUNCH(ctx, "acx_attention");
    return ACX_OK;
  }
  if (x3) return acx_fail(ctx, ACX_E_UNSUPPORTED, "acx_attention_x3: the ViT kernel only (non-causal, 128 < L <= 1024, out 16-byte aligned)%s");
  if (L > 224) return acx_fail(ctx, ACX_E_UNSUPPORTED, "acx_attention: L > 224 needs the streaming kernel (out 16-byte aligned, ldo %% 4 == 0)%s");
  const int dev_slot = (ctx ? ctx->device : 0) & 63;
#define ACX_ATTN(NT, NW)                                                                           \
  acx_launch_lds<attn_kernel<NT, NW>>(dev_slot, grid, dim3(NW * 64), (size_t)NT * 32 * (KROW + VROW) * 4 + NW * 32 * 4 + 16, s, \
                                      qkv, ldqkv, out, ldo, L, heads, causal)
  switch (nt) {
    case 1: ACX_ATTN(1, 4); break;
    case 2: ACX_ATTN(2, 4); break;
    case 3: ACX_ATTN(3, 4); break;
    case 4: ACX_ATTN(4, 4); break;
    case 5: ACX_ATTN(5, 8); break;
    case 6: ACX_ATTN(6, 8); break;
    default:
      if (nw4) ACX_ATTN(7, 4); else ACX_ATTN(7, 8);
      break;
  }
#undef ACX_ATTN
  ACX_CHECK_LAUNCH(ctx, "acx_attention");
  return ACX_OK;
}

extern "C" int acx_attention(acx_ctx* ctx, const float* qkv, int64_t ldqkv, float* out, int64_t ldo,
                             int32_t batch, int32_t L, int32_t heads, int32_t causal, void* stream) {
  return attention_impl(ctx, qkv, ldqkv, out, ldo, batch, L, heads, causal, stream, 0);
}

static int ap3_launch(acx_ctx* ctx, int form, const void* src, int64_t ldqkv, void* out_planes, int32_t batch, int32_t L, int32_t heads,
                      void* stream, const char* name, float oscale = 1.f) {
  const int64_t rows = (int64_t)batch * L;
  const int nitems = batch * heads;
  const int ncu = ctx && ctx->multiprocessors > 0 ? ctx->multiprocessors : 256;
  hipStream_t s = (hipStream_t)stream;
  AcxProfScope prof__(ctx, ACX_K_ATTN, s);
  const int dev_slot = (ctx ? ctx->device : 0) & 63;
#if AP3_TRACE
  long long* trace_ = getenv("ACX_TRACE_PTR") ? (long long*)strtoull(getenv("ACX_TRACE_PTR"), nullptr, 0) : nullptr;
#else
  long long* trace_ = nullptr;
#endif
  const dim3 grid((unsigned)(nitems < ncu ? nitems : ncu));
#define ACX_AP3(LD, ...)                                                                                                        \
  acx_launch_lds<attn_p3_kernel<__VA_ARGS__>>(dev_slot, grid, dim3(512), (size_t)AP3_LDS_B, s, (const u16*)src, (int64_t)(LD), rows, \
                                              (u16*)out_planes, rows * heads * 64, L, heads, nitems, trace_)
  if (form == 103) ACX_AP3(rows * 3 * heads * 64, 3, 1);
  else if (form == 3) ACX_AP3(rows * 3 * heads * 64, 3);
  else if (form == 6) ACX_AP3(rows * 3 * heads * 64, 6);
  else if (form == 16)
    acx_launch_lds<attn_p3_o16_kernel>(dev_slot, grid, dim3(512), (size_t)AP3_LDS_B, s, (const u16*)src, ldqkv, rows, (u16*)out_planes,
                                       rows * heads * 64, L, heads, nitems, trace_, oscale);
  else ACX_AP3(ldqkv, 6, 0, 1);
#undef ACX_AP3
  ACX_CHECK_LAUNCH(ctx, name);
  return ACX_OK;
}

extern "C" int acx_attention_p3(acx_ctx* ctx, const void* qkv_planes, void* out_planes, int32_t batch, int32_t L, int32_t heads,
                                void* stream) {
  return acx_attention_p3n(ctx, qkv_planes, out_planes, batch, L, heads, 6, stream);
}
extern "C" int acx_attention_p3n(acx_ctx* ctx, const void* qkv_planes, void* out_planes, int32_t batch, int32_t L, int32_t heads,
                                 int32_t products, void* stream) {
  if (!qkv_planes || !out_planes) return acx_fail(ctx, ACX_E_BADARG, "acx_attention_p3: null pointer%s");
  const bool f16 = products == 103;
  if (f16) products = 3;
  if (products != 6 && products != 3) return acx_fail(ctx, ACX_E_BADARG, "acx_attention_p3n: products must be 6, 3 or 103 (3 on fp16 planes)%s");
  if (batch <= 0) return ACX_OK;
  if (L <= 192 || L > AP3_ROWS || heads <= 0 || (((uintptr_t)qkv_planes | (uintptr_t)out_planes) & 15))
    return acx_fail(ctx, ACX_E_UNSUPPORTED, "acx_attention_p3: 192 < L <= 208, 16-byte aligned planes%s");
  return ap3_launch(ctx, f16 ? 103 : products, qkv_planes, 0, out_planes, batch, L, heads, stream, "acx_attention_p3");
}

extern "C" int acx_attention_p3f(acx_ctx* ctx, const float* qkv, int64_t ldqkv, void* out_planes, int32_t batch, int32_t L, int32_t heads,
                                 void* stream) {
  if (!qkv || !out_planes) return acx_fail(ctx, ACX_E_BADARG, "acx_attention_p3f: null pointer%s");
  if (batch <= 0) return ACX_OK;
  if (L <= 192 || L > AP3_ROWS || heads <= 0 || ldqkv < (int64_t)3 * heads * 64 || (ldqkv & 3) || (((uintptr_t)qkv | (uintptr_t)out_planes) & 15))
    return acx_fail(ctx, ACX_E_UNSUPPORTED, "acx_attention_p3f: 192 < L <= 208, 16-byte aligned qkv and planes, ldqkv %% 4 == 0 and >= 3 heads * 64%s");
  return ap3_launch(ctx, 0, qkv, ldqkv, out_planes, batch, L, heads, stream, "acx_attention_p3f");
}

extern "C" int acx_attention_p3f16(acx_ctx* ctx, const float* qkv, int64_t ldqkv, void* out_planes, float out_scale, int32_t batch, int32_t L,
                                   int32_t heads, void* stream) {
  if (!qkv || !out_planes) return acx_fail(ctx, ACX_E_BADARG, "acx_attention_p3f16: null pointer%s");
  int e = 0;
  if (!(out_scale >= 0x1p-20f && out_scale <= 0x1p20f) || frexpf(out_scale, &e) != 0.5f)
    return acx_fail(ctx, ACX_E_BADARG, "acx_attention_p3f16: out_scale must be a power of two in [2^-20, 2^20]%s");
  if (batch <= 0) return ACX_OK;
  if (L <= 192 || L > AP3_ROWS || heads <= 0 || ldqkv < (int64_t)3 * heads * 64 || (ldqkv & 3) || (((uintptr_t)qkv | (uintptr_t)out_planes) & 15))
    return acx_fail(ctx, ACX_E_UNSUPPORTED, "acx_attention_p3f16: 192 < L <= 208, 16-byte aligned qkv and planes, ldqkv %% 4 == 0 and >= 3 heads * 64%s");
  return ap3_launch(ctx, 16, qkv, ldqkv, out_planes, batch, L, heads, stream, "acx_attention_p3f16", out_scale);
}

extern "C" int acx_attention_x3(acx_ctx* ctx, const float* qkv, int64_t ldqkv, void* out_planes, int64_t ldo,
                                int32_t batch, int32_t L, int32_t heads, void* stream) {
  return attention_impl(ctx, qkv, ldqkv, (float*)out_planes, ldo, batch, L, heads, 0, stream, 1);
}
extern "C" int acx_attention_x3_panel(acx_ctx* ctx, const float* qkv, int64_t ldqkv, void* out_planes, int64_t ldo,
                                      int32_t batch, int32_t L, int32_t heads, void* stream) {
  if (ldo != (int64_t)heads * 64) return acx_fail(ctx, ACX_E_BADARG, "acx_attention_x3_panel: dense planes (ldo == heads * 64)%s");
  return attention_impl(ctx, qkv, ldqkv, (float*)out_planes, ldo, batch, L, heads, 0, stream, 2);
}

extern "C" int acx_attention_bf16(acx_ctx* ctx, const void* qkv, int64_t ldqkv, void* out, int64_t ldo, int32_t batch,
                                  int32_t L, int32_t heads, void* stream) {
  if (!qkv || !out) return acx_fail(ctx, ACX_E_BADARG, "acx_attention_bf16: null pointer%s");
  if (batch <= 0) return ACX_OK;
  if (L <= 0 || L > 224 || heads <= 0) return acx_fail(ctx, ACX_E_UNSUPPORTED, "acx_attention_bf16: need 0 < L <= 224%s");
  if (ldqkv % 8 || ldo % 4 || ((uintptr_t)qkv & 15) || ((uintptr_t)out & 7))
    return acx_fail(ctx, ACX_E_BADARG, "acx_attention_bf16: qkv 16-byte aligned with ld%%8==0, out 8-byte aligned with ld%%4==0%s");
  const int nt = (L + 31) / 32;
  const dim3 grid((unsigned)(batch * heads));
  hipStream_t s = (hipStream_t)stream;
  AcxProfScope prof__(ctx, ACX_K_ATTN, s);
  const int dev_slot = (ctx ? ctx->device : 0) & 63;
#define ACX_ATTNB(NT)                                                                              \
  acx_launch_lds<attn_bf16_kernel<NT>>(dev_slot, grid, dim3(256), (size_t)NT * 32 * BK_ROWB + 2 * BV_PANEL_B, s, (const u16*)qkv, ldqkv, \
                                       (u16*)out, ldo, L, heads)
  switch (nt) {
    case 1: ACX_ATTNB(1); break;
    case 2: ACX_ATTNB(2); break;
    case 3: ACX_ATTNB(3); break;
    case 4: ACX_ATTNB(4); break;
    case 5: ACX_ATTNB(5); break;
    case 6: ACX_ATTNB(6); break;
    default: ACX_ATTNB(7); break;
  }
#undef ACX_ATTNB
  ACX_CHECK_LAUNCH(ctx, "acx_attention_bf16");
  return ACX_OK;
}

extern "C" int acx_attention_cls(acx_ctx* ctx, const float* qkv, int64_t ldqkv, float* out, int64_t ldo, int32_t batch,
                                 int32_t L, int32_t heads, void* stream) {
  if (!qkv || !out) return acx_fail(ctx, ACX_E_BADARG, "acx_attention_cls: null pointer%s");
  if (batch <= 0) return ACX_OK;
  if (L <= 0 || L > 1024 || heads <= 0) return acx_fail(ctx, ACX_E_UNSUPPORTED, "acx_attention_cls: need 0 < L <= 1024%s");
  if (ldqkv % 4 || ((uintptr_t)qkv & 15)) return acx_fail(ctx, ACX_E_BADARG, "acx_attention_cls: alignment%s");
  hipStream_t s = (hipStream_t)stream;
  AcxProfScope prof__(ctx, ACX_K_ATTN, s);
  const int64_t n = (int64_t)batch * heads;
  hipLaunchKernelGGL(attn_cls_kernel, dim3((unsigned)((n + 3) / 4)), dim3(256), 0, s, qkv, ldqkv, out, ldo, batch, L, heads);
  ACX_CHECK_LAUNCH(ctx, "acx_attention_cls");
  return ACX_OK;
}

extern "C" size_t acx_attention_cls_fold_workspace_bytes(int32_t batch, int32_t heads) {
  if (batch <= 0 || heads <= 0) return 0;
  return (size_t)2 * batch * heads * heads * 64 * sizeof(float);
}

extern "C" int acx_attention_cls_fold(acx_ctx* ctx, const float* x, const float* ln_w, const float* ln_b, float eps,
                                      const float* in_proj_w, const float* in_proj_b, const float* q, int64_t ldq, float* out,
                                      int64_t ldo, int32_t batch, int32_t L, int32_t W, int32_t heads, void* workspace,
                                      size_t workspace_bytes, void* stream) {
  if (!x || !ln_w || !ln_b || !in_proj_w || !in_proj_b || !q || !out || !workspace)
    return acx_fail(ctx, ACX_E_BADARG, "acx_attention_cls_fold: null pointer%s");
  if (batch <= 0) return ACX_OK;
  if (L <= 0 || L > 1024) return acx_fail(ctx, ACX_E_UNSUPPORTED, "acx_attention_cls_fold: need 0 < L <= 1024%s");
  if (heads <= 0 || W != heads * 64) return acx_fail(ctx, ACX_E_UNSUPPORTED, "acx_attention_cls_fold: head dim must be 64%s");
  switch (heads) {
    case 1: case 2: case 4: case 8: case 10: case 12: case 16: break;
    default: return acx_fail(ctx, ACX_E_UNSUPPORTED, "acx_attention_cls_fold: width %s%ld not in {64,128,256,512,640,768,1024}", "", (long)W);
  }
  if (((uintptr_t)x & 15) || ((uintptr_t)workspace & 15)) return acx_fail(ctx, ACX_E_BADARG, "acx_attention_cls_fold: x and workspace must be 16-byte aligned%s");
  if (workspace_bytes < acx_attention_cls_fold_workspace_bytes(batch, heads))
    return acx_fail(ctx, ACX_E_WORKSPACE, "acx_attention_cls_fold: workspace too small%s");
  hipStream_t s = (hipStream_t)stream;
  const int dev_slot = (ctx ? ctx->device : 0) & 63;
  float* u = (float*)workspace;
  float* z = u + (size_t)batch * heads * W;
  const float* wk = in_proj_w + (size_t)W * W;
  const float* wv = in_proj_w + (size_t)2 * W * W;
  const int HP = (heads + 3) & ~3;
// ... 22 lines not shown
```

anomalyclip_amd/csrc/acx_attn_p3.h:

```cpp
#ifndef AP3_TRACE
#define AP3_TRACE 0
#endif
constexpr int AP3_ROWS = 208;
constexpr int AP3_BLK_B = AP3_ROWS * 64;
constexpr int AP3_LDS_B = 12 * AP3_BLK_B;

typedef short ap3_s16x4 __attribute__((ext_vector_type(4)));
typedef __attribute__((address_space(3))) ap3_s16x4 ap3_lds_s16x4;
typedef __attribute__((address_space(3))) void ap3_lds_void;

template <int F16 = 0>
__device__ __forceinline__ void ap3_split8(const float (&p)[8], bf16x8& hi, bf16x8& mid, bf16x8& lo) {
  uint32_t h[4], m[4], l[4];
#pragma unroll
  for (int e = 0; e < 4; ++e) {
    h[e] = acx_pk2<F16>(p[2 * e], p[2 * e + 1]);
    const float r0 = p[2 * e] - acx_unpk_lo<F16>(h[e]), r1 = p[2 * e + 1] - acx_unpk_hi<F16>(h[e]);
    m[e] = acx_pk2<F16>(r0, r1);
    l[e] = f2bf2(r0 - acx_unpk_lo<F16>(m[e]), r1 - acx_unpk_hi<F16>(m[e]));
  }
  typedef uint32_t u32x4_ __attribute__((ext_vector_type(4)));
  const u32x4_ hv = {h[0], h[1], h[2], h[3]}, mv = {m[0], m[1], m[2], m[3]}, lv = {l[0], l[1], l[2], l[3]};
  hi = __builtin_bit_cast(bf16x8, hv); mid = __builtin_bit_cast(bf16x8, mv); lo = __builtin_bit_cast(bf16x8, lv);
}

template <int F16>
__device__ __forceinline__ f32x16 ap3_mfma(const bf16x8 a, const bf16x8 b, const f32x16 c) {
  if constexpr (F16 != 0) {
    typedef _Float16 ap3_h8 __attribute__((ext_vector_type(8)));
    return __builtin_amdgcn_mfma_f32_32x32x16_f16(__builtin_bit_cast(ap3_h8, a), __builtin_bit_cast(ap3_h8, b), c, 0, 0, 0);
  } else {
    return __builtin_amdgcn_mfma_f32_32x32x16_bf16(a, b, c, 0, 0, 0);
  }
}
__device__ __forceinline__ const float4* ap3f_src(const float* __restrict__ qkv, int64_t ld, int64_t row0, int col0, int L, int wi, int lane) {
  const int r_ = min(8 * wi + ((lane >> 2) & 7), L - 1);
  return reinterpret_cast<const float4*>(qkv + (row0 + r_) * ld + (col0 + (lane >> 5) * 32 + (lane & 3) * 8));
}
template <int SWZ>
__device__ __forceinline__ void ap3f_put(char* smem, const float4 a, const float4 b, int blk0, int wi, int lane) {
  const float v[8] = {a.x, a.y, a.z, a.w, b.x, b.y, b.z, b.w};
  bf16x8 hi, mid, lo;
  ap3_split8<0>(v, hi, mid, lo);
  const int row = 8 * wi + ((lane >> 2) & 7), ch = lane & 3;
  char* dst = smem + (blk0 + (lane >> 5)) * AP3_BLK_B + row * 64 + (SWZ ? (ch ^ ((row >> 2) & 3)) : ch) * 16;
  *reinterpret_cast<bf16x8*>(dst) = hi;
  *reinterpret_cast<bf16x8*>(dst + 2 * AP3_BLK_B) = mid;
  *reinterpret_cast<bf16x8*>(dst + 4 * AP3_BLK_B) = lo;
}
__device__ __forceinline__ void ap3f_stage_k(char* smem, const float* __restrict__ qkv, int64_t ld, int64_t row0, int col0, int L, int lane) {
#pragma unroll 1
  for (int w0 = 0; w0 < 26; w0 += 13) {
    float4 ka_[13], kb_[13];
#pragma unroll
    for (int j = 0; j < 13; ++j) { const float4* p_ = ap3f_src(qkv, ld, row0, col0, L, w0 + j, lane); ka_[j] = p_[0]; kb_[j] = p_[1]; }
    __builtin_amdgcn_sched_barrier(0);
#pragma unroll
    for (int j = 0; j < 13; ++j) ap3f_put<1>(smem, ka_[j], kb_[j], 0, w0 + j, lane);
  }
}


template <int NPROD, int F16, int F32IN, int O16>
__device__ __forceinline__ void attn_p3_body(const u16* __restrict__ qkv3, int64_t plane_elems, int64_t rows_total,
                                             u16* __restrict__ out3, int64_t out_plane_elems, int L, int heads, int nitems,
                                             long long* __restrict__ trace, float oscale) {
  static_assert(O16 == 0 || (F32IN != 0 && F16 == 0 && NPROD == 6), "fp16 output planes behind bf16 products: the f32-rows arm");
  constexpr int NPL = NPROD == 3 ? 2 : 3;
  constexpr int OF = (F16 != 0 || O16 != 0) ? 1 : 0;
  constexpr int ONPL = O16 ? 2 : NPL;
#if AP3_TRACE
#ifndef AP3_TRACE_FIRST
#define AP3_TRACE_FIRST 0
#endif
#define AP3_STAMP(ord, pt) do { if (trace && blockIdx.x == 0 && (ord) >= AP3_TRACE_FIRST && (ord) < AP3_TRACE_FIRST + 16 && lane == 0) trace[(((ord) - AP3_TRACE_FIRST) * 8 + wave) * 8 + (pt)] = (long long)__builtin_amdgcn_s_memrealtime(); } while (0)
#else
#define AP3_STAMP(ord, pt) do { (void)(ord); } while (0)
#endif
  int ord = 0;
  extern __shared__ __attribute__((aligned(1024))) char smem[];
  const int t = threadIdx.x, lane = t & 63;
  const int wave = __builtin_amdgcn_readfirstlane(t >> 6);
  const int li = lane & 31, hh = lane >> 5;
  const int W = heads * 64;
  const int np = W / 32;
  const unsigned lds0 = (unsigned)(uintptr_t)(ap3_lds_void*)smem;
#define AP3_GLDS(base, voff, ldsaddr)                                                              \
  do {                                                                                             \
    asm volatile("s_mov_b32 m0, %1\n\ts_nop 0\n\tglobal_load_lds_dwordx4 %0, %2" : : "v"(voff), "s"(ldsaddr), "s"(base) : "memory"); \
  } while (0)
#define AP3_STAGE(it, which, blk0, SWZ)                                                            \
  do {                                                                                             \
    const int b_ = (it) / heads, h_ = (it) - b_ * heads;                                           \
    const unsigned vc_ = (unsigned)(((SWZ) ? ((lane & 3) ^ ((lane >> 4) & 3)) : (lane & 3)) * 16); \
    _Pragma("unroll 1") for (int pc = 0; pc < 2 * NPL; ++pc) {                                     \
      const u16* src_ = qkv3 + (int64_t)(pc >> 1) * plane_elems + ((int64_t)((which) * np + 2 * h_ + (pc & 1)) * rows_total + (int64_t)b_ * L) * 32; \
      _Pragma("unroll 1") for (int j = 0; j < 13; ++j) {                                           \
        const unsigned r_ = min(16u * (unsigned)j + (unsigned)(lane >> 2), (unsigned)(L - 1));    \
        AP3_GLDS(src_, r_ * 64u + vc_, lds0 + (unsigned)(((blk0) + pc) * AP3_BLK_B + j * 1024));   \
      }                                                                                            \
    }                                                                                              \
  } while (0)

#define AP3_STAGE_SHARED(it, which, blk0, SWZ)                                                     \
  do {                                                                                             \
    const int b_ = (it) / heads, h_ = (it) - b_ * heads;                                           \
    const unsigned vc_ = (unsigned)(((SWZ) ? ((lane & 3) ^ ((lane >> 4) & 3)) : (lane & 3)) * 16); \
    _Pragma("unroll 1") for (int idx = wave; idx < 26 * NPL; idx += 8) {                           \
      const int pc = idx / 13, j = idx - 13 * pc;                                                  \
      const u16* src_ = qkv3 + (int64_t)(pc >> 1) * plane_elems + ((int64_t)((which) * np + 2 * h_ + (pc & 1)) * rows_total + (int64_t)b_ * L) * 32; \
      const unsigned r_ = min(16u * (unsigned)j + (unsigned)(lane >> 2), (unsigned)(L - 1));       \
      AP3_GLDS(src_, r_ * 64u + vc_, lds0 + (unsigned)(((blk0) + pc) * AP3_BLK_B + j * 1024));     \
    }                                                                                              \
  } while (0)

  const float* qf32 = reinterpret_cast<const float*>(qkv3);

  int item = blockIdx.x;
  if (item >= nitems) return;
  const float sc = 0.125f * 1.44269504088896340736f;
  if (wave == 7) {
    if constexpr (F32IN) ap3f_stage_k(smem, qf32, plane_elems, (int64_t)(item / heads) * L, W + (item % heads) * 64, L, lane); else
    AP3_STAGE(item, 1, 0, 1);
    for (; item < nitems; item += (int)gridDim.x) {
      AP3_STAMP(ord, 0);
      if constexpr (F32IN) asm volatile("s_waitcnt lgkmcnt(0)" ::: "memory");
      else
      asm volatile("s_waitcnt vmcnt(0)" ::: "memory");
      AP3_STAMP(ord, 1);
      __builtin_amdgcn_s_barrier();
      AP3_STAMP(ord, 2);
      const int nxt = item + (int)gridDim.x, nxb = nxt / heads;
      if constexpr (F32IN) {
        asm volatile("" ::: "memory");
#pragma unroll 1
        for (int wi = 7; wi < 26; wi += 8) {
          const float4* p_ = ap3f_src(qf32, plane_elems, (int64_t)(item / heads) * L, 2 * W + (item % heads) * 64, L, wi, lane);
          ap3f_put<0>(smem, p_[0], p_[1], 6, wi, lane);
        }
        asm volatile("s_waitcnt lgkmcnt(0)" ::: "memory");
      } else {
      AP3_STAGE_SHARED(item, 2, 6, 0);
      asm volatile("s_waitcnt vmcnt(0)" ::: "memory");
      }
      AP3_STAMP(ord, 3);
      __builtin_amdgcn_s_barrier();
      AP3_STAMP(ord, 4);
      if constexpr (F32IN) {
        asm volatile("" ::: "memory");
        if (nxt < nitems) ap3f_stage_k(smem, qf32, plane_elems, (int64_t)nxb * L, W + (nxt % heads) * 64, L, lane);
      } else
      if (nxt < nitems) AP3_STAGE(nxt, 1, 0, 1);
      AP3_STAMP(ord, 5);
      ++ord;
    }
    asm volatile("s_waitcnt vmcnt(0)" ::: "memory");
    return;
  }
  const int i16 = lane & 15;
  int va = 6 * AP3_BLK_B + (4 * hh + (i16 >> 2)) * 64 + (16 * ((lane >> 4) & 1) + 4 * (i16 & 3)) * 2;
  int va2 = va + 4 * AP3_BLK_B;
  const int swk = (li >> 2) & 3;
  int ka0 = li * 64 + ((0 + hh) ^ swk) * 16, ka1 = li * 64 + ((2 + hh) ^ swk) * 16;
  int ka0l = ka0 + 4 * AP3_BLK_B, ka1l = ka1 + 4 * AP3_BLK_B;
  asm volatile("" : "+v"(va), "+v"(va2), "+v"(ka0), "+v"(ka1), "+v"(ka0l), "+v"(ka1l));
  const int qrow = min(32 * wave + li, L - 1);
  for (; item < nitems; item += (int)gridDim.x) {
    const int b = item / heads, h = item - b * heads;
    bf16x8 qf[3][4];
    if constexpr (F32IN) {
      const float4* qp = reinterpret_cast<const float4*>(qf32 + ((int64_t)b * L + qrow) * plane_elems + (h * 64 + 8 * hh));
      float4 qa[4], qb[4];
#pragma unroll
      for (int ks = 0; ks < 4; ++ks) { qa[ks] = qp[4 * ks]; qb[ks] = qp[4 * ks + 1]; }
#pragma unroll
      for (int ks = 0; ks < 4; ++ks) {
        const float qv[8] = {qa[ks].x, qa[ks].y, qa[ks].z, qa[ks].w, qb[ks].x, qb[ks].y, qb[ks].z, qb[ks].w};
        ap3_split8<0>(qv, qf[0][ks], qf[1][ks], qf[2][ks]);
      }
    } else
#pragma unroll
    for (int p = 0; p < NPL; ++p)
#pragma unroll
      for (int ks = 0; ks < 4; ++ks)
        qf[p][ks] = *reinterpret_cast<const bf16x8*>(qkv3 + (int64_t)p * plane_elems +
                                                     ((int64_t)(2 * h + (ks >> 1)) * rows_total + (int64_t)b * L + qrow) * 32 + ((ks & 1) * 2 + hh) * 8);
    AP3_STAMP(ord, 0);
    __builtin_amdgcn_s_barrier();
    AP3_STAMP(ord, 1);
    float4 sva[4], svb[4];
    if constexpr (F32IN) {
      asm volatile("" ::: "memory");
#pragma unroll
      for (int z = 0; z < 4; ++z) {
        sva[z] = svb[z] = make_float4(0.f, 0.f, 0.f, 0.f);
        if (z < 3 || wave < 2) {
          const float4* p_ = ap3f_src(qf32, plane_elems, (int64_t)b * L, 2 * W + h * 64, L, wave + 8 * z, lane);
          sva[z] = p_[0]; svb[z] = p_[1];
        }
      }
      __builtin_amdgcn_sched_barrier(0);
    } else
    AP3_STAGE_SHARED(item, 2, 6, 0);
// ... 61 lines not shown
      const int kt = st >> 1, u = st & 1;
      const float pv[8] = {sacc[kt][8 * u], sacc[kt][8 * u + 1], sacc[kt][8 * u + 2], sacc[kt][8 * u + 3],
                           sacc[kt][8 * u + 4], sacc[kt][8 * u + 5], sacc[kt][8 * u + 6], sacc[kt][8 * u + 7]};
      bf16x8 ph, pm, pl;
      ap3_split8<F16>(pv, ph, pm, pl);
#pragma unroll
      for (int dt = 0; dt < 2; ++dt) {
        bf16x8 vf[3];
#pragma unroll
        for (int p = 0; p < NPL; ++p) {
          const char* vb = smem + (p == 2 ? va2 : va) + ((p == 2 ? 0 : 2 * p) + dt) * AP3_BLK_B + (16 * st) * 64;
          const ap3_s16x4 lo4 = __builtin_amdgcn_ds_read_tr16_b64_v4i16((ap3_lds_s16x4*)(vb));
          const ap3_s16x4 hi4 = __builtin_amdgcn_ds_read_tr16_b64_v4i16((ap3_lds_s16x4*)(vb + 8 * 64));
          typedef short s16x8_ __attribute__((ext_vector_type(8)));
          const s16x8_ v8 = {lo4[0], lo4[1], lo4[2], lo4[3], hi4[0], hi4[1], hi4[2], hi4[3]};
          vf[p] = __builtin_bit_cast(bf16x8, v8);
        }
        if constexpr (NPROD == 6) {
        oacc[dt] = __builtin_amdgcn_mfma_f32_32x32x16_bf16(vf[2], ph, oacc[dt], 0, 0, 0);
        oacc[dt] = __builtin_amdgcn_mfma_f32_32x32x16_bf16(vf[1], pm, oacc[dt], 0, 0, 0);
        oacc[dt] = __builtin_amdgcn_mfma_f32_32x32x16_bf16(vf[0], pl, oacc[dt], 0, 0, 0);
        }
        oacc[dt] = ap3_mfma<F16>(vf[1], ph, oacc[dt]);
        oacc[dt] = ap3_mfma<F16>(vf[0], pm, oacc[dt]);
        oacc[dt] = ap3_mfma<F16>(vf[0], ph, oacc[dt]);
      }
      __builtin_amdgcn_sched_barrier(0);
    }
    AP3_STAMP(ord, 6);
    const float inv = O16 ? (1.f / sum) * oscale : 1.f / sum;
    const int q = 32 * wave + li;
    const bool st_ok = q < L;
#pragma unroll
    for (int dt = 0; dt < 2; ++dt)
#pragma unroll
      for (int gp = 0; gp < 2; ++gp) {
        uint2 pl_[2][3];
#pragma unroll
        for (int z = 0; z < 2; ++z) {
          const int g4 = 2 * gp + z;
          const float ov[4] = {oacc[dt][4 * g4] * inv, oacc[dt][4 * g4 + 1] * inv, oacc[dt][4 * g4 + 2] * inv, oacc[dt][4 * g4 + 3] * inv};
          uint2 ph2, pm2, pl2;
          ph2.x = acx_pk2<OF>(ov[0], ov[1]); ph2.y = acx_pk2<OF>(ov[2], ov[3]);
          const float r0 = ov[0] - acx_unpk_lo<OF>(ph2.x), r1 = ov[1] - acx_unpk_hi<OF>(ph2.x);
          const float r2 = ov[2] - acx_unpk_lo<OF>(ph2.y), r3 = ov[3] - acx_unpk_hi<OF>(ph2.y);
          pm2.x = acx_pk2<OF>(r0, r1); pm2.y = acx_pk2<OF>(r2, r3);
          pl2.x = f2bf2(r0 - __uint_as_float(pm2.x << 16), r1 - __uint_as_float(pm2.x & 0xffff0000u));
          pl2.y = f2bf2(r2 - __uint_as_float(pm2.y << 16), r3 - __uint_as_float(pm2.y & 0xffff0000u));
          pl_[z][0] = ph2; pl_[z][1] = pm2; pl_[z][2] = pl2;
        }
#pragma unroll
        for (int p = 0; p < ONPL; ++p) {
          typedef unsigned ap3_u2 __attribute__((ext_vector_type(2)));
          const ap3_u2 w0 = __builtin_amdgcn_permlane32_swap(pl_[0][p].x, pl_[1][p].x, false, false);
          const ap3_u2 w1 = __builtin_amdgcn_permlane32_swap(pl_[0][p].y, pl_[1][p].y, false, false);
          const uint4 v16 = make_uint4(w0[0], w1[0], w0[1], w1[1]);
          if (st_ok) {
            u16* dst = out3 + (int64_t)p * out_plane_elems + ((int64_t)(2 * h + dt) * rows_total + (int64_t)b * L + q) * 32 + 8 * (2 * gp + hh);
            *reinterpret_cast<uint4*>(dst) = v16;
          }
        }
      }
    AP3_STAMP(ord, 7);
    ++ord;
  }
#undef AP3_STAMP
#undef AP3_STAGE_SHARED
#undef AP3_STAGE
#undef AP3_GLDS
}

template <int NPROD, int F16 = 0, int F32IN = 0>
__global__ __launch_bounds__(512, 2) void attn_p3_kernel(const u16* __restrict__ qkv3, int64_t plane_elems, int64_t rows_total,
                                                         u16* __restrict__ out3, int64_t out_plane_elems, int L, int heads, int nitems,
                                                         long long* __restrict__ trace) {
  attn_p3_body<NPROD, F16, F32IN, 0>(qkv3, plane_elems, rows_total, out3, out_plane_elems, L, heads, nitems, trace, 1.f);
}

__global__ __launch_bounds__(512, 2) void attn_p3_o16_kernel(const u16* __restrict__ qkv3, int64_t plane_elems, int64_t rows_total,
                                                             u16* __restrict__ out3, int64_t out_plane_elems, int L, int heads, int nitems,
                                                             long long* __restrict__ trace, float oscale) {
  attn_p3_body<6, 0, 1, 1>(qkv3, plane_elems, rows_total, out3, out_plane_elems, L, heads, nitems, trace, oscale);
}
```

anomalyclip_amd/ops.py:

```python
from __future__ import annotations

import contextlib
import ctypes as C
import gc
import threading
from typing import Optional, Sequence

import torch

from . import _lib as L

_BF16 = torch.bfloat16

WEIGHT_EPOCH = [0]


def _ptr(t: Optional[torch.Tensor]):
    return None if t is None else t.data_ptr()


def _stream():
    return torch.cuda.current_stream().cuda_stream


# ... 360 lines not shown


def layernorm(x: torch.Tensor, w: torch.Tensor, b: torch.Tensor, *, eps=1e-5, mode=L.NORM_LAYER,
              out_dtype=torch.float32, rows: Optional[int] = None, ldx: Optional[int] = None, planes_out: bool = False,
              panel_out: bool = False) -> torch.Tensor:
    D = w.numel()
    if rows is None:
        rows = x.numel() // D
        ldx = D
    y = torch.empty((3, rows, D) if planes_out else (rows, D), dtype=_BF16 if planes_out else out_dtype, device=x.device)
    h = _h(x)
    L.check(L.lib().acx_layernorm(h, x.data_ptr(), ldx, w.data_ptr(), b.data_ptr(), y.data_ptr(), D,
                                  (L.BF16X3P if panel_out else L.BF16X3) if planes_out else _dt(y), rows, D, eps, mode, _stream()), h)
    return y


def layernorm_f16x2(x: torch.Tensor, w: torch.Tensor, b: torch.Tensor, scale: float = 1.0, *, eps=1e-5, mode=L.NORM_LAYER) -> torch.Tensor:
    D = w.numel()
    rows = x.numel() // D
    y = torch.empty(2, rows, D, dtype=torch.float16, device=x.device)
    h = _h(x)
    L.check(L.lib().acx_layernorm_scaled(h, x.data_ptr(), D, w.data_ptr(), b.data_ptr(), y.data_ptr(), rows, D, eps, mode, float(scale),
                                         _stream()), h)
    return y


def attention(qkv: torch.Tensor, batch: int, L_: int, heads: int, causal: bool) -> torch.Tensor:
    assert qkv.is_contiguous() and qkv.shape == (batch * L_, 3 * heads * 64)
    out = torch.empty(batch * L_, heads * 64, dtype=torch.float32, device=qkv.device)
    h = _h(qkv)
    L.check(L.lib().acx_attention(h, qkv.data_ptr(), qkv.stride(0), out.data_ptr(), out.stride(0), batch, L_, heads,
                                  int(causal), _stream()), h)
    return out


def attention_cls_fold(x: torch.Tensor, ln_w: torch.Tensor, ln_b: torch.Tensor, in_proj_w: torch.Tensor, in_proj_b: torch.Tensor,
                       q: torch.Tensor, batch: int, L_: int, heads: int, eps: float = 1e-5) -> torch.Tensor:
    W = heads * 64
    assert x.is_contiguous() and x.shape == (batch * L_, W) and q.shape == (batch, W) and q.stride(1) == 1
    assert in_proj_w.is_contiguous() and in_proj_w.shape == (3 * W, W) and in_proj_b.numel() == 3 * W
    out = torch.empty(batch, W, dtype=torch.float32, device=x.device)
    nbytes = L.lib().acx_attention_cls_fold_workspace_bytes(batch, heads)
    ws = torch.empty(max(nbytes, 16), dtype=torch.uint8, device=x.device)
    h = _h(x)
    L.check(L.lib().acx_attention_cls_fold(h, x.data_ptr(), ln_w.data_ptr(), ln_b.data_ptr(), float(eps), in_proj_w.data_ptr(),
                                           in_proj_b.data_ptr(), q.data_ptr(), q.stride(0), out.data_ptr(), out.stride(0), batch, L_,
                                           W, heads, ws.data_ptr(), nbytes, _stream()), h)
    return out


def attention_p3(qkv3: torch.Tensor, batch: int, L_: int, heads: int, products: int = 6) -> torch.Tensor:
    W = heads * 64
    if products == 103:
        assert qkv3.dtype == torch.float16 and qkv3.is_contiguous() and qkv3.shape == (2, batch * L_, 3 * W)
        out = torch.empty(2, batch * L_, W, dtype=torch.float16, device=qkv3.device)
        h = _h(qkv3)
        L.check(L.lib().acx_attention_p3n(h, qkv3.data_ptr(), out.data_ptr(), batch, L_, heads, 103, _stream()), h)
        return out
    assert qkv3.dtype == _BF16 and qkv3.is_contiguous() and qkv3.shape == (3, batch * L_, 3 * W)
    out = (torch.zeros if products == 3 else torch.empty)(3, batch * L_, W, dtype=_BF16, device=qkv3.device)
    h = _h(qkv3)
    L.check(L.lib().acx_attention_p3n(h, qkv3.data_ptr(), out.data_ptr(), batch, L_, heads, int(products), _stream()), h)
    return out


def attention_p3_f32(qkv: torch.Tensor, batch: int, L_: int, heads: int) -> torch.Tensor:
    W = heads * 64
    assert qkv.dtype == torch.float32 and qkv.shape == (batch * L_, 3 * W) and qkv.stride(1) == 1
    out = torch.empty(3, batch * L_, W, dtype=_BF16, device=qkv.device)
    h = _h(qkv)
    L.check(L.lib().acx_attention_p3f(h, qkv.data_ptr(), qkv.stride(0), out.data_ptr(), batch, L_, heads, _stream()), h)
    return out


def attention_p3_f32_f16(qkv: torch.Tensor, batch: int, L_: int, heads: int, scale: float = 1.0) -> torch.Tensor:
    W = heads * 64
    assert qkv.dtype == torch.float32 and qkv.shape == (batch * L_, 3 * W) and qkv.stride(1) == 1
    out = torch.empty(2, batch * L_, W, dtype=torch.float16, device=qkv.device)
    h = _h(qkv)
    L.check(L.lib().acx_attention_p3f16(h, qkv.data_ptr(), qkv.stride(0), out.data_ptr(), float(scale), batch, L_, heads, _stream()), h)
    return out


def attention_bf16(qkv: torch.Tensor, batch: int, L_: int, heads: int) -> torch.Tensor:
    assert qkv.dtype == torch.bfloat16 and qkv.is_contiguous()
    W = heads * 64
    out = torch.empty(batch * L_, W, dtype=torch.bfloat16, device=qkv.device)
    h = _h(qkv)
    L.check(L.lib().acx_attention_bf16(h, qkv.data_ptr(), qkv.stride(0), out.data_ptr(), W, batch, L_, heads, _stream()), h)
    return out


def text_directions(text: torch.Tensor, ncentroid: torch.Tensor, normal_id: int) -> torch.Tensor:
    Cc, D = text.shape
    dirs = torch.empty(Cc - 1, D, dtype=torch.float32, device=text.device)
    h = _h(text)
    L.check(L.lib().acx_text_directions(h, text.data_ptr(), ncentroid.data_ptr(), dirs.data_ptr(), Cc, D, normal_id,
                                        _stream()), h)
    return dirs


def selector_project(x: torch.Tensor, ncentroid: torch.Tensor, dirs: torch.Tensor) -> torch.Tensor:
    x = x.reshape(-1, x.shape[-1])
    assert x.is_contiguous()
    rows, D = x.shape
    C1 = dirs.shape[0]
    raw = torch.empty(rows, C1, dtype=torch.float32, device=x.device)
    h = _h(x)
    L.check(L.lib().acx_selector_project(h, x.data_ptr(), ncentroid.data_ptr(), dirs.data_ptr(), raw.data_ptr(), rows, D,
                                         C1, _stream()), h)
    return raw


def bn_combine(gathered: torch.Tensor, C1: int):
    assert gathered.is_cuda and gathered.dtype == torch.float32 and gathered.is_contiguous() and gathered.shape[1] == 2 * C1 + 1
    out = torch.empty(3 * C1 + 1, dtype=torch.float32, device=gathered.device)
    h = _h(gathered)
    L.check(L.lib().acx_bn_combine(h, gathered.data_ptr(), gathered.shape[0], C1, out.data_ptr(), out[C1:].data_ptr(),
                                   out[2 * C1:].data_ptr(), out[3 * C1:].data_ptr(), _stream()), h)
    return out[:C1], out[C1:2 * C1], out[2 * C1:3 * C1], out[3 * C1:]


def _bn_workspace(t: torch.Tensor, rows: int, C1: int) -> torch.Tensor:
    return torch.empty(int(L.lib().acx_bn_workspace_bytes(rows, C1)) // 8, dtype=torch.float64, device=t.device)


def bn_stats(raw: torch.Tensor):
    rows, C1 = raw.shape
    st = torch.empty(3, C1, dtype=torch.float32, device=raw.device)
    h = _h(raw)
    ws = _bn_workspace(raw, rows, C1)
    L.check(L.lib().acx_bn_stats(h, raw.data_ptr(), rows, C1, st[0].data_ptr(), st[1].data_ptr(), st[2].data_ptr(),
                                 ws.data_ptr(), ws.numel() * 8, _stream()), h)
    return st[0], st[1], st[2]


def selector_project_stats(x: torch.Tensor, ncentroid: torch.Tensor, dirs: torch.Tensor):
    x = x.reshape(-1, x.shape[-1])
    assert x.is_contiguous()
    rows, D = x.shape
    C1 = dirs.shape[0]
    raw = torch.empty(rows, C1, dtype=torch.float32, device=x.device)
    st = torch.empty(3, C1, dtype=torch.float32, device=x.device)
    ws = _bn_workspace(x, rows, C1)
    h = _h(x)
    L.check(L.lib().acx_selector_project_stats(h, x.data_ptr(), ncentroid.data_ptr(), dirs.data_ptr(), raw.data_ptr(), rows, D,
                                               C1, st[0].data_ptr(), st[1].data_ptr(), st[2].data_ptr(), ws.data_ptr(),
                                               ws.numel() * 8, _stream()), h)
    return raw, st[0], st[1], st[2]


def selector_bn(raw: torch.Tensor, mean: torch.Tensor, var: torch.Tensor, eps=1e-5,
                out: Optional[torch.Tensor] = None) -> torch.Tensor:
    rows, C1 = raw.shape
    if out is None:
        out = torch.empty(rows, C1, dtype=torch.float32, device=raw.device)
    h = _h(raw)
    L.check(L.lib().acx_selector_bn(h, raw.data_ptr(), mean.data_ptr(), var.data_ptr(), out.data_ptr(), out.stride(0),
                                    rows, C1, eps, _stream()), h)
    return out


def axial_attention(qkv: torch.Tensor, tiles: int, gn: int, gl: int, heads: int, e: int, axis: int) -> torch.Tensor:
    assert qkv.is_contiguous() and qkv.shape == (tiles * gn * gl, 3 * heads * e)
    out = torch.empty(tiles * gn * gl, heads * e, dtype=torch.float32, device=qkv.device)
    h = _h(qkv)
# ... 1082 lines not shown
```

include/acx.h:

```cpp
#ifndef ACX_H_
#define ACX_H_

#include <stddef.h>
#include <stdint.h>

#ifdef __cplusplus
extern "C" {
#endif

#define ACX_VERSION 100

enum {
  ACX_OK = 0,
  ACX_E_BADARG = -1,
  ACX_E_UNSUPPORTED = -2,
  ACX_E_HIP = -3,
  ACX_E_WORKSPACE = -4,
  ACX_E_RCCL = -5
};

enum { ACX_F32 = 0, ACX_BF16 = 1,
       ACX_BF16X3 = 2,
       ACX_BF16X3P = 3 };
enum { ACX_F16 = 5,
       ACX_F16X2P = 6 };
enum { ACX_BF16X2P = 4 };
enum { ACX_PREC_F32 = 0, ACX_PREC_BF16 = 1,
       ACX_PREC_F32X3 = 3,
       ACX_PREC_F16X3 = 4,
       ACX_PREC_F32X6 = 2 };
enum { ACX_PREC_BF16X6 = 5 };
enum { ACX_PREC_F32X6_LN16 = 6 };
enum { ACX_PREC_F32X6_R16 = 7 };
#define ACX_F16X3_WSCALE 1024.0f
enum { ACX_ACT_NONE = 0, ACX_ACT_QUICKGELU = 1, ACX_ACT_LEAKYRELU = 2,
       ACX_ACT_RELU = 3,
       ACX_ACT_RESRELU = 4 };
enum { ACX_ACT_GELU = 5 };
enum { ACX_AMAP_IDENTITY = 0, ACX_AMAP_CONV3X3 = 1, ACX_AMAP_TESTTILE = 2, ACX_AMAP_TILETABLE = 3 };
enum { ACX_NORM_LAYER = 0, ACX_NORM_CHAN = 1 };

typedef struct acx_ctx acx_ctx;

int acx_version(void);
int acx_create(acx_ctx** out, int device);
void acx_destroy(acx_ctx* ctx);
const char* acx_last_error(acx_ctx* ctx);

enum { ACX_OPT_RING_MIN_TILES = 1, ACX_OPT_SK_MAX_M = 2, ACX_OPT_TN_P256_MIN_ROWS = 3, ACX_OPT_X6_CUS = 4, ACX_OPT_X6_TAIL_SPLIT = 5,
       ACX_OPT_X6_STRIP_TAIL = 6, ACX_OPT_X6_MIN_TILES = 7, ACX_OPT_LN_RIDER = 8, ACX_OPT_ATTN_F32IN = 9, ACX_OPT_CLS_FOLD = 10 };
int acx_set_option(acx_ctx* ctx, int32_t option, int64_t value);
int acx_get_option(acx_ctx* ctx, int32_t option, int64_t* value);

typedef struct acx_gemm_desc {
  const void* A;
  const void* W;
  void* C;
  int32_t M, N, K;
  int32_t lda, ldw, ldc;
  int32_t a_dtype, c_dtype;
  int32_t prec;
  const float* bias;
  int32_t act;
  const float* residual;
  int32_t ldr;
  const float* a_sub;
  int32_t amap;
  int32_t gn, gl;
  int32_t cin;
  int32_t seg;
  const float* pos0;
  const float* pos1;
  void* workspace;
  size_t workspace_bytes;
  const void* zero_page;
  int32_t a_act;
  const float* gelu_grad_of;
  int32_t ldg;
  const float* a_norm_w;
  const float* a_norm_b;
  float a_norm_eps;
  uint32_t* counters;
  int32_t n_counters;
  const int32_t* tile_table;
  int32_t pairs;
  int32_t panels;
  int64_t a_plane_stride, w_plane_stride;
  int64_t c_plane_rows;
  float out_scale;
  float c_scale;
} acx_gemm_desc;
int acx_gemm(acx_ctx* ctx, const acx_gemm_desc* d, void* stream);

typedef struct acx_gemm_scratch_t {
  size_t workspace_bytes;
  int32_t counters;
} acx_gemm_scratch_t;
int acx_gemm_scratch(const acx_ctx* ctx, const acx_gemm_desc* d, int32_t allow_split, acx_gemm_scratch_t* out);

enum { ACX_GEMM_ROUTE_NONE = 0, ACX_GEMM_ROUTE_X6_TAIL_SPLIT = 1, ACX_GEMM_ROUTE_SK = 2, ACX_GEMM_ROUTE_X6 = 3, ACX_GEMM_ROUTE_S64 = 4,
       ACX_GEMM_ROUTE_P256 = 5, ACX_GEMM_ROUTE_W8 = 6, ACX_GEMM_ROUTE_W8_CONV = 7, ACX_GEMM_ROUTE_RING = 8, ACX_GEMM_ROUTE_P8 = 9,
       ACX_GEMM_ROUTE_DMA_CONV = 10, ACX_GEMM_ROUTE_DMA = 11, ACX_GEMM_ROUTE_GENERIC = 12 };
typedef struct acx_gemm_route_t {
  int32_t route, ksplit, reduce;
  int32_t reserved;
  int64_t tiles;
} acx_gemm_route_t;
int acx_gemm_route(const acx_ctx* ctx, const acx_gemm_desc* d, acx_gemm_route_t* out);

typedef struct acx_ln_job {
  const float* w;
  const float* b;
  void* y;
  int32_t y_dtype;
  float eps;
  int32_t mode;
  float y_scale;
} acx_ln_job;
int acx_gemm_ln(acx_ctx* ctx, const acx_gemm_desc* d, const acx_ln_job* job, void* stream);
int64_t acx_gemm_ln_plan(int32_t M, int32_t N, int32_t K, int32_t ncu, int32_t ksplit, double rate, int64_t* rows_ready);

int acx_layernorm(acx_ctx* ctx, const float* x, int64_t ldx, const float* w, const float* b,
                  void* y, int64_t ldy, int32_t y_dtype, int64_t rows, int32_t D, float eps,
                  int32_t mode, void* stream);
int acx_layernorm_scaled(acx_ctx* ctx, const float* x, int64_t ldx, const float* w, const float* b, void* y, int64_t rows,
                         int32_t D, float eps, int32_t mode, float y_scale, void* stream);

int acx_attention(acx_ctx* ctx, const float* qkv, int64_t ldqkv, float* out, int64_t ldo,
                  int32_t batch, int32_t L, int32_t heads, int32_t causal, void* stream);
int acx_attention_x3(acx_ctx* ctx, const float* qkv, int64_t ldqkv, void* out_planes, int64_t ldo,
                     int32_t batch, int32_t L, int32_t heads, void* stream);
int acx_attention_p3(acx_ctx* ctx, const void* qkv_planes, void* out_planes, int32_t batch, int32_t L, int32_t heads, void* stream);
int acx_attention_p3n(acx_ctx* ctx, const void* qkv_planes, void* out_planes, int32_t batch, int32_t L, int32_t heads, int32_t products,
                      void* stream);
int acx_attention_p3f(acx_ctx* ctx, const float* qkv, int64_t ldqkv, void* out_planes, int32_t batch, int32_t L, int32_t heads,
                      void* stream);
int acx_attention_p3f16(acx_ctx* ctx, const float* qkv, int64_t ldqkv, void* out_planes, float out_scale, int32_t batch, int32_t L,
                        int32_t heads, void* stream);
int acx_attention_x3_panel(acx_ctx* ctx, const float* qkv, int64_t ldqkv, void* out_planes, int64_t ldo,
                           int32_t batch, int32_t L, int32_t heads, void* stream);

int acx_attention_bf16(acx_ctx* ctx, const void* qkv, int64_t ldqkv, void* out, int64_t ldo, int32_t batch,
                       int32_t L, int32_t heads, void* stream);
int acx_attention_cls(acx_ctx* ctx, const float* qkv, int64_t ldqkv, float* out, int64_t ldo,
                      int32_t batch, int32_t L, int32_t heads, void* stream);
size_t acx_attention_cls_fold_workspace_bytes(int32_t batch, int32_t heads);
int acx_attention_cls_fold(acx_ctx* ctx, const float* x, const float* ln_w, const float* ln_b, float eps, const float* in_proj_w,
                           const float* in_proj_b, const float* q, int64_t ldq, float* out, int64_t ldo, int32_t batch, int32_t L,
                           int32_t W, int32_t heads, void* workspace, size_t workspace_bytes, void* stream);

int acx_vit_patches(acx_ctx* ctx, const float* frames, void* patches, int32_t out_dtype,
                    int32_t F, int32_t R, int32_t P, void* stream);
int acx_vit_embed(acx_ctx* ctx, const float* patch_out, const float* cls, const float* pos,
                  const float* ln_w, const float* ln_b, float* x, int32_t F, int32_t T, int32_t W,
                  void* stream);

typedef struct acx_block_weights {
  const float *ln1_w, *ln1_b, *ln2_w, *ln2_b;
  const float *in_proj_w, *in_proj_b;
  const float *out_proj_w, *out_proj_b;
  const float *fc_w, *fc_b;
  const float *proj_w, *proj_b;
  const void *in_proj_w_bf16, *out_proj_w_bf16, *fc_w_bf16, *proj_w_bf16;
} acx_block_weights;

typedef struct acx_vit_weights {
  const float* conv1_w;
  const void* conv1_w_bf16;
  const float* class_embedding;
  const float* positional_embedding;
  const float *ln_pre_w, *ln_pre_b, *ln_post_w, *ln_post_b;
  const float* proj_t;
  const void* proj_t_bf16;
  const acx_block_weights* blocks;
} acx_vit_weights;

typedef struct acx_vit_desc {
  int32_t resolution, patch, width, layers, heads, embed_dim;
  int32_t prec;
  int32_t act;
} acx_vit_desc;

size_t acx_vit_workspace_bytes(const acx_vit_desc* d, int32_t frames);
int acx_vit_encode(acx_ctx* ctx, const acx_vit_desc* d, const acx_vit_weights* w,
                   const float* frames, int32_t nframes, float* features, void* workspace,
                   size_t workspace_bytes, void* stream);
int acx_vit_encode_ln16(acx_ctx* ctx, const acx_vit_desc* d, const acx_vit_weights* w, const float* ln_scales, const float* frames,
                        int32_t nframes, float* features, void* workspace, size_t workspace_bytes, void* stream);
int acx_vit_encode_r16(acx_ctx* ctx, const acx_vit_desc* d, const acx_vit_weights* w, const float* scales, const float* frames,
                       int32_t nframes, float* features, void* workspace, size_t workspace_bytes, void* stream);


int acx_resnet_stem_im2col(acx_ctx* ctx, const float* frames, float* cols, int32_t F, int32_t R, void* stream);
int acx_avgpool2_nhwc(acx_ctx* ctx, const float* in, float* out, int32_t F, int32_t H, int32_t W, int32_t C, void* stream);
int acx_attnpool_tokens(acx_ctx* ctx, const float* x, const float* pos, float* tokens, int32_t F, int32_t HW, int32_t E, void* stream);

typedef struct acx_resnet_conv {
  const float* w;
  const float* b;
  const void* w3;
} acx_resnet_conv;
typedef struct acx_resnet_block {
  acx_resnet_conv conv1, conv2, conv3;
  acx_resnet_conv downsample;
} acx_resnet_block;
typedef struct acx_resnet_weights {
  acx_resnet_conv stem[3];
  const acx_resnet_block* blocks;
  const float* positional_embedding;
  const float *q_w, *q_b;
  const float *kv_w, *kv_b;
  const float *c_w, *c_b;
  const void* kv_w3;
} acx_resnet_weights;
typedef struct acx_resnet_desc {
  int32_t resolution, width;
  int32_t layers[4];
  int32_t heads, output_dim;
  int32_t prec;
} acx_resnet_desc;
size_t acx_resnet_workspace_bytes(const acx_resnet_desc* d, int32_t frames);
int acx_resnet_encode(acx_ctx* ctx, const acx_resnet_desc* d, const acx_resnet_weights* w, const float* frames, int32_t nframes,
                      float* features, void* workspace, size_t workspace_bytes, void* stream);

typedef struct acx_resnet_bn {
  const float *weight, *bias;
  float *running_mean, *running_var;
  int64_t* num_batches_tracked;
} acx_resnet_bn;
typedef struct acx_resnet_block_bn {
  acx_resnet_bn bn1, bn2, bn3, downsample;
} acx_resnet_block_bn;
typedef struct acx_resnet_train_bn {
  acx_resnet_bn stem[3];
  const acx_resnet_block_bn* blocks;
  float eps, momentum;
} acx_resnet_train_bn;
int acx_bn_apply_nhwc(acx_ctx* ctx, const float* x, const float* mean, const float* var_biased, const float* gamma, const float* beta,
                      const float* residual, float* y, int64_t rows, int32_t C, int32_t Cp, float eps, int32_t relu, float* scratch,
                      void* stream);
size_t acx_resnet_train_workspace_bytes(const acx_resnet_desc* d, int32_t frames);
int acx_resnet_encode_train(acx_ctx* ctx, const acx_resnet_desc* d, const acx_resnet_weights* w, const acx_resnet_train_bn* bn,
                            const float* frames, int32_t F, float* features, void* workspace, size_t workspace_bytes, void* stream);

size_t acx_transformer_workspace_bytes(int32_t width, int32_t rows);
size_t acx_transformer_workspace_bytes_prec(int32_t width, int32_t rows, int32_t prec);
int acx_transformer_forward(acx_ctx* ctx, float* x, int32_t batch, int32_t L, int32_t width,
                            int32_t heads, int32_t layers, int32_t causal, int32_t prec,
                            const acx_block_weights* blocks, void* workspace,
                            size_t workspace_bytes, void* stream);
int acx_transformer_forward_act(acx_ctx* ctx, float* x, int32_t batch, int32_t L, int32_t width,
                                int32_t heads, int32_t layers, int32_t causal, int32_t prec, int32_t act,
                                const acx_block_weights* blocks, void* workspace,
                                size_t workspace_bytes, void* stream);

enum { ACX_TF_LN_ROWS = 0, ACX_TF_LN_PLANES = 1, ACX_TF_LN_RIDDEN = 2, ACX_TF_LN_CLS = 3 };
enum { ACX_TF_GEMM_ROWS = 0, ACX_TF_GEMM_X6 = 1 };
enum { ACX_TF_BUF_NONE = 0, ACX_TF_BUF_SPLITK = 1, ACX_TF_BUF_H = 2, ACX_TF_BUF_QKV = 3, ACX_TF_BUF_MLP = 4 };
enum { ACX_TF_ATT_F32 = 0, ACX_TF_ATT_BF16 = 1, ACX_TF_ATT_X3_PANEL = 2, ACX_TF_ATT_P3N = 3, ACX_TF_ATT_P3F = 4, ACX_TF_ATT_CLS = 5,
       ACX_TF_ATT_CLS_FOLD = 6 };
typedef struct acx_tf_product_t {
  int32_t kernel, c_dtype, scratch, ln_job;
} acx_tf_product_t;
typedef struct acx_tf_layer_plan_t {
  int32_t ln1, ln1_dtype, ln2, ln2_dtype;
  acx_tf_product_t in_proj, out_proj, fc, proj;
  int32_t att, att_products, split_att, split_mlp;
  int32_t pruned;
  int32_t att_out_dtype;
} acx_tf_layer_plan_t;
int acx_transformer_plan(const acx_ctx* ctx, int32_t batch, int32_t L, int32_t width, int32_t heads, int32_t layers,
                         int32_t causal, int32_t prec, int32_t prune_last, int32_t has_weight_planes,
                         int32_t workspace_is_prec_sized, acx_tf_layer_plan_t* out );
// ... 359 lines not shown
```

Before: 10310 frames/s.

## Emit QKV as scaled fp16 two-plane output and attend with fp16 products

Adds a new precision mode, F32X6_QKV16. The QKV in-projection writes range-proved, power-of-two-scaled fp16 two-plane output instead of f32 rows. A new attention kernel variant then reads those planes using 3 fp16 products, with the inverse scale folded into the softmax scale. The goal is to cut QKV write and read bandwidth and the per-element splitting work inside attention. The cost is extra range-proof bookkeeping, and the path is gated on weight bounds and on the in-projection not needing a split-K route.

```diff
diff --git a/anomalyclip_amd/_lib.py b/anomalyclip_amd/_lib.py
--- a/anomalyclip_amd/_lib.py
+++ b/anomalyclip_amd/_lib.py
@@ -14,6 +14,7 @@
 PREC_BF16X6 = 5
 PREC_F32X6_LN16 = 6
 PREC_F32X6_R16 = 7
+PREC_F32X6_QKV16 = 8
 ACT_NONE, ACT_QUICKGELU, ACT_LEAKYRELU, ACT_RELU, ACT_RESRELU = 0, 1, 2, 3, 4
 ACT_GELU = 5
 AMAP_IDENTITY, AMAP_CONV3X3, AMAP_TESTTILE, AMAP_TILETABLE = 0, 1, 2, 3
@@ -195,6 +196,7 @@
     "acx_attention_p3n": (C.c_int, [c_void_p, c_void_p, c_void_p, c_int32, c_int32, c_int32, c_int32, c_void_p]),
     "acx_attention_p3f": (C.c_int, [c_void_p, c_void_p, c_int64, c_void_p, c_int32, c_int32, c_int32, c_void_p]),
     "acx_attention_p3f16": (C.c_int, [c_void_p, c_void_p, c_int64, c_void_p, c_float, c_int32, c_int32, c_int32, c_void_p]),
+    "acx_attention_p3h16": (C.c_int, [c_void_p, c_void_p, c_float, c_void_p, c_float, c_int32, c_int32, c_int32, c_void_p]),
     "acx_attention_x3_panel": (C.c_int, [c_void_p, c_void_p, c_int64, c_void_p, c_int64, c_int32, c_int32, c_int32, c_void_p]),
     "acx_attention_cls": (C.c_int, [c_void_p, c_void_p, c_int64, c_void_p, c_int64, c_int32, c_int32, c_int32, c_void_p]),
     "acx_attention_cls_fold_workspace_bytes": (c_size_t, [c_int32, c_int32]),
@@ -220,6 +222,8 @@
                                       c_void_p, c_size_t, c_void_p]),
     "acx_vit_encode_r16": (C.c_int, [c_void_p, C.POINTER(VitDesc), C.POINTER(VitWeights), c_void_p, c_void_p, c_int32, c_void_p,
                                      c_void_p, c_size_t, c_void_p]),
+    "acx_vit_encode_qkv16": (C.c_int, [c_void_p, C.POINTER(VitDesc), C.POINTER(VitWeights), c_void_p, c_void_p, c_int32, c_void_p,
+                                       c_void_p, c_size_t, c_void_p]),
     "acx_transformer_workspace_bytes": (c_size_t, [c_int32, c_int32]),
     "acx_transformer_workspace_bytes_prec": (c_size_t, [c_int32, c_int32, c_int32]),
     "acx_transformer_forward": (C.c_int, [c_void_p, c_void_p, c_int32, c_int32, c_int32, c_int32, c_int32, c_int32,
diff --git a/anomalyclip_amd/components/clip_vit.py b/anomalyclip_amd/components/clip_vit.py
--- a/anomalyclip_amd/components/clip_vit.py
+++ b/anomalyclip_amd/components/clip_vit.py
@@ -78,32 +78,40 @@
         for wt in (b.attn.in_proj_weight, b.mlp.c_fc.weight):
             vals.append(wt.detach().abs().max().double())
             vals.append(wt.detach().double().abs().sum())
-        for ln, wt, bias in ((b.ln_1, b.attn.in_proj_weight[2 * D:], b.attn.in_proj_bias[2 * D:]), (b.ln_2, b.mlp.c_fc.weight, b.mlp.c_fc.bias)):
-            l1, l2 = r16_bounds(ln.weight, ln.bias, wt, bias)
+        q1, q2 = r16_bounds(b.ln_1.weight, b.ln_1.bias, b.attn.in_proj_weight, b.attn.in_proj_bias)
+        for l1, l2 in ((q1[2 * D:], q2[2 * D:]), r16_bounds(b.ln_2.weight, b.ln_2.bias, b.mlp.c_fc.weight, b.mlp.c_fc.bias)):
             vals.append(torch.minimum(l1, l2).max() + 0.0 * (l1.sum() + l2.sum()))
         for wt in (b.attn.out_proj.weight, b.mlp.c_proj.weight):
             vals.append(wt.detach().abs().max().double())
             vals.append(wt.detach().double().abs().sum())
+        vals.append(torch.minimum(q1, q2).max() + 0.0 * (q1.sum() + q2.sum()))
     if not vals:
-        return None, None
+        return None, None, None
     v = torch.stack(vals).tolist()
     ln16: Optional[List[float]] = []
     r16: Optional[List[float]] = []
-    for i in range(0, len(v), 14):
-        b1, f1, b2, f2, w1, g1, w2, g2, ba, bh, w3, g3, w4, g4 = v[i:i + 14]
+    qkv: Optional[List[float]] = []
+    for i in range(0, len(v), 15):
+        b1, f1, b2, f2, w1, g1, w2, g2, ba, bh, w3, g3, w4, g4, bq = v[i:i + 15]
         if ln16 is not None:
             s1, s2 = ln16_scale(b1), ln16_scale(b2)
             if not all(math.isfinite(t) for t in (f1, f2, g1, g2)) or not (w1 <= LN16_WEIGHT_MAX and w2 <= LN16_WEIGHT_MAX) or s1 is None or s2 is None:
-                ln16 = r16 = None
+                ln16 = r16 = qkv = None
             else:
                 ln16 += [s1, s2]
         if r16 is not None:
             sa, sh = ln16_scale(ba), ln16_scale(bh)
             if not all(math.isfinite(t) for t in (g3, g4)) or not (w3 <= LN16_WEIGHT_MAX and w4 <= LN16_WEIGHT_MAX) or sa is None or sh is None:
-                r16 = None
+                r16 = qkv = None
             else:
                 r16 += [sa, sh]
-    return ln16, r16
+        if qkv is not None:
+            sq = ln16_scale(bq)
+            if sq is None:
+                qkv = None
+            else:
+                qkv.append(sq)
+    return ln16, r16, qkv
 
 
 def ln16_scales(blocks, width: int) -> Optional[List[float]]:
@@ -112,6 +120,10 @@
 
 def r16_scales(blocks, width: int) -> Optional[List[float]]:
     return _range_proofs(blocks, width)[1]
+
+
+def qkv16_scales(blocks, width: int) -> Optional[List[float]]:
+    return _range_proofs(blocks, width)[2]
 
 
 HEAD_MAX_AXIS = 128
@@ -291,6 +303,7 @@
         D = self.width
         lim = 65504.0
         worst = {"weight_planes": 0.0, "layernorm_out": 0.0, "attention_out": 0.0, "mlp_hidden": 0.0}
+        qkv = {"q": 0.0, "k": 0.0, "v": 0.0}
 
         def ln_bound(ln):
             return float((ln.weight.abs() * (D - 1) ** 0.5 + ln.bias.abs()).max())
@@ -300,19 +313,22 @@
             wv, bv = b.attn.in_proj_weight[2 * D:], b.attn.in_proj_bias[2 * D:]
             worst["layernorm_out"] = max(worst["layernorm_out"], l1, l2)
             worst["attention_out"] = max(worst["attention_out"], float((wv.abs().sum(1) * l1 + bv.abs()).max()))
+            for t, name in enumerate(("q", "k", "v")):
+                wt, bt = b.attn.in_proj_weight[t * D:(t + 1) * D], b.attn.in_proj_bias[t * D:(t + 1) * D]
+                qkv[name] = max(qkv[name], float((wt.abs().sum(1) * l1 + bt.abs()).max()))
             worst["mlp_hidden"] = max(worst["mlp_hidden"], float((b.mlp.c_fc.weight.abs().sum(1) * l2 + b.mlp.c_fc.bias.abs()).max()))
             mats += [b.attn.in_proj_weight, b.attn.out_proj.weight, b.mlp.c_fc.weight, b.mlp.c_proj.weight]
         worst["weight_planes"] = F16X3_WSCALE * max(float(m.abs().max()) for m in mats)
-        margin = min(lim / max(v, 1e-30) for v in worst.values())
-        return {"bounds": worst, "fp16_max": lim, "margin": margin, "safe": margin > 1.0}
+        margin = min(lim / max(v, 1e-30) for v in list(worst.values()) + list(qkv.values()))
+        return {"bounds": worst, "qkv": qkv, "fp16_max": lim, "margin": margin, "safe": margin > 1.0}
 
     def _ln16_bound(self):
         key = (ops.WEIGHT_EPOCH[0],) + tuple((p.data_ptr(), p._version) for p in self.parameters())
         if self._ln16 is not None and self._ln16[0] == key:
             return self._ln16[1]
-        res = None
+        res = qkv16 = None
         if self.width in (768, 1024) and self.layers > 1 and L.exports("acx_vit_encode_ln16"):
-            scales, wide = _range_proofs(self.transformer.resblocks, self.width)
+            scales, wide, sq = _range_proofs(self.transformer.resblocks, self.width)
             if scales is not None:
                 fc16 = ops.transformer_plan(64, 197, 768, 12, 2, prec=L.PREC_F32X6_LN16, prune_last=True)[0]["ln2_dtype"] == L.F16X2P
                 r16 = None
@@ -322,9 +338,16 @@
                     if any(fmt):
                         s4 = [t for l in range(self.layers) for t in (scales[2 * l], scales[2 * l + 1], wide[2 * l], wide[2 * l + 1])]
                         r16 = (s4, (C.c_float * len(s4))(*s4), fmt)
+                        if sq is not None and fmt[0] and L.exports("acx_vit_encode_qkv16"):
+                            s5 = [t for l in range(self.layers) for t in (*s4[4 * l:4 * l + 4], sq[l])]
+                            qkv16 = (s5, (C.c_float * len(s5))(*s5))
                 res = (scales, (C.c_float * len(scales))(*scales), fc16, r16)
-        self._ln16 = (key, res)
+        self._ln16 = (key, res, qkv16)
         return res
+
+    def _qkv16_bound(self):
+        self._ln16_bound()
+        return self._ln16[2]
 
     def ln16_resolution(self) -> Optional[List[float]]:
         res = self._ln16_bound()
@@ -333,6 +356,10 @@
     def r16_resolution(self) -> Optional[List[float]]:
         res = self._ln16_bound()
         return None if res is None or res[3] is None else res[3][0]
+
+    def qkv16_resolution(self) -> Optional[List[float]]:
+        res = self._qkv16_bound()
+        return None if res is None else res[0]
 
     def _weights(self, prec: int, ln16_fc: bool = True, r16=(True, True)):
         key = (prec, bool(ln16_fc), bool(r16[0]), bool(r16[1]), ops.WEIGHT_EPOCH[0]) + tuple((p.data_ptr(), p._version) for p in self.parameters())
@@ -371,7 +398,15 @@
         lib = L.lib()
         bound = self._ln16_bound() if self.precision == "auto" and x.is_cuda else None
         ln16_fc, r16 = True, (True, True)
-        if bound is not None and bound[3] is not None:
+        wprec = None
+        qkv16 = self._qkv16_bound() if bound is not None and bound[3] is not None else None
+        if qkv16 is not None:
+            prec, wprec = L.PREC_F32X6_QKV16, L.PREC_F32X6_R16
+            ln16_fc = bound[2]
+            r16 = bound[3][2]
+            sc5 = qkv16[1]
+            encode = lambda *a: lib.acx_vit_encode_qkv16(a[0], a[1], a[2], sc5, *a[3:])
+        elif bound is not None and bound[3] is not None:
             prec = L.PREC_F32X6_R16
             ln16_fc = bound[2]
             _s4, sc4, r16 = bound[3]
@@ -383,7 +418,7 @@
         else:
             encode = lib.acx_vit_encode
         d = L.VitDesc(self.input_resolution, self.patch_size, self.width, self.layers, self.heads, self.output_dim, prec, ACTS[self.act])
-        w, _keep = self._weights(prec, ln16_fc, r16)
+        w, _keep = self._weights(prec if wprec is None else wprec, ln16_fc, r16)
         F = x.shape[0]
         out = torch.empty(F, self.output_dim, dtype=torch.float32, device=x.device)
         chunk = min(self.chunk, F)
diff --git a/anomalyclip_amd/csrc/acx_api.hip b/anomalyclip_amd/csrc/acx_api.hip
--- a/anomalyclip_amd/csrc/acx_api.hip
+++ b/anomalyclip_amd/csrc/acx_api.hip
@@ -18,6 +18,10 @@
 #define ACX_R16_PROJ_DEFAULT 1
 #endif
 
+#ifndef ACX_QKV16_DEFAULT
+#define ACX_QKV16_DEFAULT 1
+#endif
+
 #ifndef ACX_CLS_FOLD_DEFAULT
 #define ACX_CLS_FOLD_DEFAULT 1
 #endif
@@ -30,13 +34,16 @@
   bool attn_f32in, cls_fold;
   bool ln16_fc;
   bool r16_out, r16_proj;
+  bool qkv16;
 };
 constexpr TfOpts kCreateOpts = {18, ACX_ATTN_F32IN_DEFAULT != 0, ACX_CLS_FOLD_DEFAULT != 0, ACX_LN16_FC_DEFAULT != 0, ACX_R16_OUT_DEFAULT != 0,
-                                ACX_R16_PROJ_DEFAULT != 0};
-constexpr TfOpts kNoCtxOpts = {512, false, false, ACX_LN16_FC_DEFAULT != 0, ACX_R16_OUT_DEFAULT != 0, ACX_R16_PROJ_DEFAULT != 0};
+                                ACX_R16_PROJ_DEFAULT != 0, ACX_QKV16_DEFAULT != 0};
+constexpr TfOpts kNoCtxOpts = {512, false, false, ACX_LN16_FC_DEFAULT != 0, ACX_R16_OUT_DEFAULT != 0, ACX_R16_PROJ_DEFAULT != 0,
+                              ACX_QKV16_DEFAULT != 0};
 inline TfOpts tf_opts(const acx_ctx* ctx, bool query) {
   if (!ctx) return query ? kCreateOpts : kNoCtxOpts;
-  return {ctx->opt_x6_min_tiles, ctx->opt_attn_f32in != 0, ctx->opt_cls_fold != 0, kCreateOpts.ln16_fc, kCreateOpts.r16_out, kCreateOpts.r16_proj};
+  return {ctx->opt_x6_min_tiles, ctx->opt_attn_f32in != 0, ctx->opt_cls_fold != 0, kCreateOpts.ln16_fc, kCreateOpts.r16_out, kCreateOpts.r16_proj,
+          kCreateOpts.qkv16};
 }
 }
 
@@ -218,9 +225,14 @@
 
 static inline bool is_xmode(int prec) {
   return prec == ACX_PREC_F32X6 || prec == ACX_PREC_F32X3 || prec == ACX_PREC_F16X3 || prec == ACX_PREC_F32X6_LN16 ||
-         prec == ACX_PREC_F32X6_R16;
-}
-static inline bool is_ln16(int prec) { return prec == ACX_PREC_F32X6_LN16 || prec == ACX_PREC_F32X6_R16; }
+         prec == ACX_PREC_F32X6_R16 || prec == ACX_PREC_F32X6_QKV16;
+}
+static inline bool is_r16(int prec) { return prec == ACX_PREC_F32X6_R16 || prec == ACX_PREC_F32X6_QKV16; }
+static inline bool is_ln16(int prec) { return prec == ACX_PREC_F32X6_LN16 || is_r16(prec); }
+static inline int scales_per_layer(int prec) { return prec == ACX_PREC_F32X6_QKV16 ? 5 : prec == ACX_PREC_F32X6_R16 ? 4 : 2; }
+static inline const char* ln16_name(int prec) {
+  return prec == ACX_PREC_F32X6_QKV16 ? "ACX_PREC_F32X6_QKV16" : prec == ACX_PREC_F32X6_R16 ? "ACX_PREC_F32X6_R16" : "ACX_PREC_F32X6_LN16";
+}
 struct XMode {
   int pairs;
   bool f16;
@@ -377,6 +389,7 @@
   TfMode mode;
   bool ln16_qkv, ln16_fc;
   bool r16_out, r16_proj;
+  bool qkv16;
   acx_tf_layer_plan_t body, before_pruned, pruned;
   bool prune;
 };
@@ -390,6 +403,21 @@
 
 inline acx_tf_product_t tf_rows(int c_dtype, int scratch) { return {ACX_TF_GEMM_ROWS, c_dtype, scratch, 0}; }
 inline acx_tf_product_t tf_x6(int c_dtype, int scratch, bool ln_job) { return {ACX_TF_GEMM_X6, c_dtype, scratch, ln_job ? 1 : 0}; }
+
+bool in_proj_splits(acx_ctx* ctx, const TfGeom& g, int64_t rows) {
+  acx_gemm_desc d;
+  memset(&d, 0, sizeof(d));
+  d.A = d.W = d.C = d.workspace = (void*)(uintptr_t)256;
+  d.M = (int)rows; d.N = 3 * g.W; d.K = g.W; d.lda = d.ldw = g.W; d.ldc = 3 * g.W; d.ldr = d.ldc;
+  d.a_dtype = ACX_F16; d.c_dtype = ACX_F32; d.prec = ACX_PREC_BF16; d.pairs = 3; d.panels = 3;
+  d.out_scale = 1.f / ACX_F16X3_WSCALE;
+  d.a_plane_stride = rows * g.W * 2; d.w_plane_stride = (int64_t)3 * g.W * g.W * 2;
+  d.workspace_bytes = (size_t)rows * g.W * 4;
+  acx_gemm_scratch_t sc;
+  if (acx_gemm_scratch(ctx, &d, 1, &sc) != ACX_OK || sc.workspace_bytes > 0) return true;
+  acx_gemm_route_t r;
+  return acx_gemm_route(ctx, &d, &r) != ACX_OK || r.ksplit > 1;
+}
 
 int tf_plan(acx_ctx* err, const TfGeom& g, const TfHave& have, const TfOpts& o, TfPlan* p) {
   memset(p, 0, sizeof(*p));
@@ -406,9 +434,9 @@
   auto x6 = [&](int N, int K) { return xmode && x6_takes(o, g.planes_ws, rows, N, K, K); };
   const bool x6_qkv = x6(3 * W, W), x6_out = x6(W, W), x6_fc = x6(4 * W, W), x6_proj = x6(W, 4 * W), x6_kv = x6(2 * W, W);
   const bool ln_ride = m.pdt == ACX_BF16X3P;
-  const bool ln16 = is_ln16(g.prec), r16 = g.prec == ACX_PREC_F32X6_R16;
+  const bool ln16 = is_ln16(g.prec), r16 = is_r16(g.prec);
   if (ln16 && W != 768 && W != 1024)
-    return acx_fail(err, ACX_E_UNSUPPORTED, "driver: %s is built for widths 768 and 1024", r16 ? "ACX_PREC_F32X6_R16" : "ACX_PREC_F32X6_LN16");
+    return acx_fail(err, ACX_E_UNSUPPORTED, "driver: %s is built for widths 768 and 1024", ln16_name(g.prec));
   p->ln16_qkv = ln16 && x6_qkv;
   p->ln16_fc = ln16 && x6_fc && o.ln16_fc;
   const bool ab = m.prec == ACX_PREC_BF16 && !g.causal && L <= 224 && ACX_DBG_SWITCH("ATTN_BF16", true);
@@ -416,6 +444,7 @@
   p->r16_out = r16 && o.r16_out && att_p3;
   p->r16_proj = r16 && o.r16_proj && p->ln16_fc && x6_proj;
   const bool att_p3f = att_p3 && ln_ride && (o.attn_f32in || p->r16_out);
+  p->qkv16 = g.prec == ACX_PREC_F32X6_QKV16 && o.qkv16 && p->r16_out && p->ln16_qkv && att_p3f && !in_proj_splits(err, g, rows);
   const bool qkv_planes = att_p3 && !att_p3f;
   const bool att_x3 = x6_out && !g.causal && L > 128 && L <= 1024 && (L > 224 || ACX_DBG_SWITCH("ATTN16", true));
   const bool cls_fold = g.prune && m.prec != ACX_PREC_BF16 && o.cls_fold && L <= 1024 &&
@@ -443,6 +472,11 @@
   b.att = ab ? ACX_TF_ATT_BF16 : att_p3f ? ACX_TF_ATT_P3F : att_p3 ? ACX_TF_ATT_P3N : att_x3 ? ACX_TF_ATT_X3_PANEL : ACX_TF_ATT_F32;
   b.att_products = b.att == ACX_TF_ATT_P3N ? (m.xm.f16 ? 103 : m.xm.pairs) : 0;
   b.att_out_dtype = p->r16_out ? ACX_F16X2P : 0;
+  if (p->qkv16) {
+    b.in_proj = tf_x6(ACX_F16X2P, ACX_TF_BUF_QKV, false);
+    b.att = ACX_TF_ATT_P3N;
+    b.att_products = 103;
+  }
   b.split_att = x6_out && !att_x3 && !att_p3;
   b.out_proj = x6_out ? tf_x6(ACX_F32, ACX_TF_BUF_H, ln_ride && x6_fc) : tf_rows(ACX_F32, ACX_TF_BUF_SPLITK);
   b.ln2 = !x6_fc ? ACX_TF_LN_ROWS : b.out_proj.ln_job ? ACX_TF_LN_RIDDEN : ACX_TF_LN_PLANES;
@@ -481,9 +515,10 @@
   acx_ctx* ctx; const TfGeom& g; const TfMode& m; const TfWs& ws; hipStream_t s;
   const float* ln_scales;
   int64_t rows() const { return (int64_t)g.batch * g.L; }
-  bool r16() const { return g.prec == ACX_PREC_F32X6_R16; }
-  float lnsc(int dtype, int l, int which) const { return is_ln16(g.prec) && dtype == ACX_F16X2P ? ln_scales[(r16() ? 4 : 2) * l + which] : 0.f; }
-  float r16sc(int dtype, int l, int which) const { return r16() && dtype == ACX_F16X2P ? ln_scales[4 * l + which] : 0.f; }
+  bool r16() const { return is_r16(g.prec); }
+  int nsc() const { return scales_per_layer(g.prec); }
+  float lnsc(int dtype, int l, int which) const { return is_ln16(g.prec) && dtype == ACX_F16X2P ? ln_scales[nsc() * l + which] : 0.f; }
+  float r16sc(int dtype, int l, int which) const { return r16() && dtype == ACX_F16X2P ? ln_scales[nsc() * l + which] : 0.f; }
 
   Product product(const acx_block_weights& b, int i, const acx_tf_product_t& r, int64_t M) const {
     const int W = g.W;
@@ -525,12 +560,17 @@
     auto planes = [](const acx_tf_product_t& q) { return q.c_dtype != ACX_F32 && q.c_dtype != ACX_BF16; };
     const float sc1 = lnsc(r.ln1_dtype, l, 0), sc2 = lnsc(r.ln2_dtype, l, 1);
     const float s_att = r16sc(r.att_out_dtype, l, 2), s_hid = r16sc(r.fc.c_dtype, l, 3);
+    const float s_qkv = g.prec == ACX_PREC_F32X6_QKV16 ? r16sc(r.in_proj.c_dtype, l, 4) : 0.f;
     int rc;
     if ((rc = norm_all(r.ln1, r.ln1_dtype, x, b.ln1_w, b.ln1_b, sc1))) return rc;
     Product p = product(b, 0, r.in_proj, rows());
     p.a_scale = r.in_proj.kernel == ACX_TF_GEMM_X6 ? sc1 : 0.f;
     p.A = r.in_proj.kernel == ACX_TF_GEMM_X6 ? ws.hp : ws.h;
     p.C = planes(r.in_proj) ? ws.qkv3 : ws.qkv;
+    if (s_qkv > 0.f) {
+      p.C = ws.qkv; p.c_scale = s_qkv;
+      p.scratch = nullptr; p.scratch_bytes = 0;
+    }
     if ((rc = go(p))) return rc;
     switch (r.att) {
       case ACX_TF_ATT_BF16: rc = acx_attention_bf16(ctx, ws.qkv, 3 * W, ws.att, W, batch, L, heads, s); break;
@@ -538,7 +578,10 @@
         rc = s_att > 0.f ? acx_attention_p3f16(ctx, (const float*)ws.qkv, 3 * W, ws.hp, s_att, batch, L, heads, s)
                          : acx_attention_p3f(ctx, (const float*)ws.qkv, 3 * W, ws.hp, batch, L, heads, s);
         break;
-      case ACX_TF_ATT_P3N: rc = acx_attention_p3n(ctx, ws.qkv3, ws.hp, batch, L, heads, r.att_products, s); break;
+      case ACX_TF_ATT_P3N:
+        rc = s_qkv > 0.f ? acx_attention_p3h16(ctx, ws.qkv, s_qkv, ws.hp, s_att, batch, L, heads, s)
+                         : acx_attention_p3n(ctx, ws.qkv3, ws.hp, batch, L, heads, r.att_products, s);
+        break;
       case ACX_TF_ATT_X3_PANEL: rc = acx_attention_x3_panel(ctx, (const float*)ws.qkv, 3 * W, ws.hp, W, batch, L, heads, s); break;
       default: rc = acx_attention(ctx, (const float*)ws.qkv, 3 * W, (float*)ws.att, W, batch, L, heads, g.causal, s); break;
     }
@@ -631,13 +674,16 @@
         return acx_fail(ctx, ACX_E_BADARG, "driver: ACX_PREC_F32X6_LN16: a LayerNorm plane scale is not a power of two in [2^-20, 2^20]%s");
     }
   }
-  if (g.prec == ACX_PREC_F32X6_R16) {
-    if (!ln_scales) return acx_fail(ctx, ACX_E_BADARG, "driver: ACX_PREC_F32X6_R16 needs the plane scales (acx_vit_encode_r16)%s");
-    for (int i = 0; i < 4 * g.layers; ++i) {
+  if (is_r16(g.prec)) {
+    const bool q = g.prec == ACX_PREC_F32X6_QKV16;
+    if (!ln_scales)
+      return acx_fail(ctx, ACX_E_BADARG, q ? "driver: ACX_PREC_F32X6_QKV16 needs the plane scales (acx_vit_encode_qkv16)%s"
+                                           : "driver: ACX_PREC_F32X6_R16 needs the plane scales (acx_vit_encode_r16)%s");
+    for (int i = 0; i < scales_per_layer(g.prec) * g.layers; ++i) {
       int e = 0;
       const float sc = ln_scales[i];
       if (!(sc >= 0x1p-20f && sc <= 0x1p20f) || frexpf(sc, &e) != 0.5f)
-        return acx_fail(ctx, ACX_E_BADARG, "driver: ACX_PREC_F32X6_R16: a plane scale is not a power of two in [2^-20, 2^20]%s");
+        return acx_fail(ctx, ACX_E_BADARG, "driver: %s: a plane scale is not a power of two in [2^-20, 2^20]", ln16_name(g.prec));
     }
   }
   const TfRun exec = {ctx, g, plan.mode, ws, s, ln_scales};
@@ -731,6 +777,8 @@
     return acx_fail(ctx, ACX_E_BADARG, "acx_vit_encode: ACX_PREC_F32X6_LN16 needs the LayerNorm plane scales (acx_vit_encode_ln16)%s");
   if (d->prec == ACX_PREC_F32X6_R16 && !ln_scales)
     return acx_fail(ctx, ACX_E_BADARG, "acx_vit_encode: ACX_PREC_F32X6_R16 needs the plane scales (acx_vit_encode_r16)%s");
+  if (d->prec == ACX_PREC_F32X6_QKV16 && !ln_scales)
+    return acx_fail(ctx, ACX_E_BADARG, "acx_vit_encode: ACX_PREC_F32X6_QKV16 needs the plane scales (acx_vit_encode_qkv16)%s");
   int mlp_act = 0, rc0;
   if ((rc0 = tf_act(ctx, "acx_vit_encode", d->act, d->prec, &mlp_act))) return rc0;
   if (nframes <= 0) return ACX_OK;
@@ -799,3 +847,10 @@
     return acx_fail(ctx, ACX_E_BADARG, "acx_vit_encode_r16: needs desc->prec = ACX_PREC_F32X6_R16 and the plane scales%s");
   return vit_encode(ctx, d, w, scales, frames, nframes, features, workspace, workspace_bytes, stream);
 }
+
+extern "C" int acx_vit_encode_qkv16(acx_ctx* ctx, const acx_vit_desc* d, const acx_vit_weights* w, const float* scales, const float* frames,
+                                    int32_t nframes, float* features, void* workspace, size_t workspace_bytes, void* stream) {
+  if (!d || d->prec != ACX_PREC_F32X6_QKV16 || !scales)
+    return acx_fail(ctx, ACX_E_BADARG, "acx_vit_encode_qkv16: needs desc->prec = ACX_PREC_F32X6_QKV16 and the plane scales%s");
+  return vit_encode(ctx, d, w, scales, frames, nframes, features, workspace, workspace_bytes, stream);
+}
diff --git a/anomalyclip_amd/csrc/acx_attn.hip b/anomalyclip_amd/csrc/acx_attn.hip
--- a/anomalyclip_amd/csrc/acx_attn.hip
+++ b/anomalyclip_amd/csrc/acx_attn.hip
@@ -64,7 +64,7 @@
 }
 
 static int ap3_launch(acx_ctx* ctx, int form, const void* src, int64_t ldqkv, void* out_planes, int32_t batch, int32_t L, int32_t heads,
-                      void* stream, const char* name, float oscale = 1.f) {
+                      void* stream, const char* name, float oscale = 1.f, float sscale = 1.f) {
   const int64_t rows = (int64_t)batch * L;
   const int nitems = batch * heads;
   const int ncu = ctx && ctx->multiprocessors > 0 ? ctx->multiprocessors : 256;
@@ -86,6 +86,9 @@
   else if (form == 16)
     acx_launch_lds<attn_p3_o16_kernel>(dev_slot, grid, dim3(512), (size_t)AP3_LDS_B, s, (const u16*)src, ldqkv, rows, (u16*)out_planes,
                                        rows * heads * 64, L, heads, nitems, trace_, oscale);
+  else if (form == 116)
+    acx_launch_lds<attn_p3_h16_kernel>(dev_slot, grid, dim3(512), (size_t)AP3_LDS_B, s, (const u16*)src, rows * 3 * heads * 64, rows,
+                                       (u16*)out_planes, rows * heads * 64, L, heads, nitems, trace_, oscale, sscale);
   else ACX_AP3(ldqkv, 6, 0, 1);
 #undef ACX_AP3
   ACX_CHECK_LAUNCH(ctx, name);
@@ -127,6 +130,20 @@
   if (L <= 192 || L > AP3_ROWS || heads <= 0 || ldqkv < (int64_t)3 * heads * 64 || (ldqkv & 3) || (((uintptr_t)qkv | (uintptr_t)out_planes) & 15))
     return acx_fail(ctx, ACX_E_UNSUPPORTED, "acx_attention_p3f16: 192 < L <= 208, 16-byte aligned qkv and planes, ldqkv %% 4 == 0 and >= 3 heads * 64%s");
   return ap3_launch(ctx, 16, qkv, ldqkv, out_planes, batch, L, heads, stream, "acx_attention_p3f16", out_scale);
+}
+
+extern "C" int acx_attention_p3h16(acx_ctx* ctx, const void* qkv_planes, float in_scale, void* out_planes, float out_scale, int32_t batch,
+                                   int32_t L, int32_t heads, void* stream) {
+  if (!qkv_planes || !out_planes) return acx_fail(ctx, ACX_E_BADARG, "acx_attention_p3h16: null pointer%s");
+  int e = 0;
+  if (!(in_scale >= 0x1p-20f && in_scale <= 0x1p20f) || frexpf(in_scale, &e) != 0.5f || !(out_scale >= 0x1p-20f && out_scale <= 0x1p20f) ||
+      frexpf(out_scale, &e) != 0.5f)
+    return acx_fail(ctx, ACX_E_BADARG, "acx_attention_p3h16: in_scale and out_scale must be powers of two in [2^-20, 2^20]%s");
+  if (batch <= 0) return ACX_OK;
+  if (L <= 192 || L > AP3_ROWS || heads <= 0 || (((uintptr_t)qkv_planes | (uintptr_t)out_planes) & 15))
+    return acx_fail(ctx, ACX_E_UNSUPPORTED, "acx_attention_p3h16: 192 < L <= 208, 16-byte aligned planes%s");
+  return ap3_launch(ctx, 116, qkv_planes, 0, out_planes, batch, L, heads, stream, "acx_attention_p3h16", out_scale / in_scale,
+                    1.f / (in_scale * in_scale));
 }
 
 extern "C" int acx_attention_x3(acx_ctx* ctx, const float* qkv, int64_t ldqkv, void* out_planes, int64_t ldo,
diff --git a/anomalyclip_amd/csrc/acx_attn_p3.h b/anomalyclip_amd/csrc/acx_attn_p3.h
--- a/anomalyclip_amd/csrc/acx_attn_p3.h
+++ b/anomalyclip_amd/csrc/acx_attn_p3.h
@@ -64,8 +64,9 @@
 template <int NPROD, int F16, int F32IN, int O16>
 __device__ __forceinline__ void attn_p3_body(const u16* __restrict__ qkv3, int64_t plane_elems, int64_t rows_total,
                                              u16* __restrict__ out3, int64_t out_plane_elems, int L, int heads, int nitems,
-                                             long long* __restrict__ trace, float oscale) {
-  static_assert(O16 == 0 || (F32IN != 0 && F16 == 0 && NPROD == 6), "fp16 output planes behind bf16 products: the f32-rows arm");
+                                             long long* __restrict__ trace, float oscale, float sscale = 1.f) {
+  static_assert(O16 == 0 || (F32IN != 0 && F16 == 0 && NPROD == 6) || (F32IN == 0 && F16 != 0 && NPROD == 3),
+                "scaled fp16 output planes: behind bf16 products the f32-rows arm, behind fp16 products the planes arm");
   constexpr int NPL = NPROD == 3 ? 2 : 3;
   constexpr int OF = (F16 != 0 || O16 != 0) ? 1 : 0;
   constexpr int ONPL = O16 ? 2 : NPL;
@@ -118,7 +119,8 @@
 
   int item = blockIdx.x;
   if (item >= nitems) return;
-  const float sc = 0.125f * 1.44269504088896340736f;
+  const float sc0 = 0.125f * 1.44269504088896340736f;
+  const float sc = (O16 != 0 && F16 != 0) ? sc0 * sscale : sc0;
   if (wave == 7) {
     if constexpr (F32IN) ap3f_stage_k(smem, qf32, plane_elems, (int64_t)(item / heads) * L, W + (item % heads) * 64, L, lane); else
     AP3_STAGE(item, 1, 0, 1);
@@ -346,3 +348,9 @@
                                                              long long* __restrict__ trace, float oscale) {
   attn_p3_body<6, 0, 1, 1>(qkv3, plane_elems, rows_total, out3, out_plane_elems, L, heads, nitems, trace, oscale);
 }
+
+__global__ __launch_bounds__(512, 2) void attn_p3_h16_kernel(const u16* __restrict__ qkv3, int64_t plane_elems, int64_t rows_total,
+                                                             u16* __restrict__ out3, int64_t out_plane_elems, int L, int heads, int nitems,
+                                                             long long* __restrict__ trace, float oscale, float sscale) {
+  attn_p3_body<3, 1, 0, 1>(qkv3, plane_elems, rows_total, out3, out_plane_elems, L, heads, nitems, trace, oscale, sscale);
+}
diff --git a/anomalyclip_amd/ops.py b/anomalyclip_amd/ops.py
--- a/anomalyclip_amd/ops.py
+++ b/anomalyclip_amd/ops.py
@@ -466,6 +466,15 @@
     return out
 
 
+def attention_p3_h16(qkv2: torch.Tensor, batch: int, L_: int, heads: int, in_scale: float = 1.0, out_scale: float = 1.0) -> torch.Tensor:
+    W = heads * 64
+    assert qkv2.dtype == torch.float16 and qkv2.is_contiguous() and qkv2.shape == (2, batch * L_, 3 * W)
+    out = torch.empty(2, batch * L_, W, dtype=torch.float16, device=qkv2.device)
+    h = _h(qkv2)
+    L.check(L.lib().acx_attention_p3h16(h, qkv2.data_ptr(), float(in_scale), out.data_ptr(), float(out_scale), batch, L_, heads, _stream()), h)
+    return out
+
+
 def attention_bf16(qkv: torch.Tensor, batch: int, L_: int, heads: int) -> torch.Tensor:
     assert qkv.dtype == torch.bfloat16 and qkv.is_contiguous()
     W = heads * 64
diff --git a/include/acx.h b/include/acx.h
--- a/include/acx.h
+++ b/include/acx.h
@@ -32,6 +32,7 @@
 enum { ACX_PREC_BF16X6 = 5 };
 enum { ACX_PREC_F32X6_LN16 = 6 };
 enum { ACX_PREC_F32X6_R16 = 7 };
+enum { ACX_PREC_F32X6_QKV16 = 8 };
 #define ACX_F16X3_WSCALE 1024.0f
 enum { ACX_ACT_NONE = 0, ACX_ACT_QUICKGELU = 1, ACX_ACT_LEAKYRELU = 2,
        ACX_ACT_RELU = 3,
@@ -137,6 +138,8 @@
                       void* stream);
 int acx_attention_p3f16(acx_ctx* ctx, const float* qkv, int64_t ldqkv, void* out_planes, float out_scale, int32_t batch, int32_t L,
                         int32_t heads, void* stream);
+int acx_attention_p3h16(acx_ctx* ctx, const void* qkv_planes, float in_scale, void* out_planes, float out_scale, int32_t batch, int32_t L,
+                        int32_t heads, void* stream);
 int acx_attention_x3_panel(acx_ctx* ctx, const float* qkv, int64_t ldqkv, void* out_planes, int64_t ldo,
                            int32_t batch, int32_t L, int32_t heads, void* stream);
 
@@ -189,6 +192,8 @@
                         int32_t nframes, float* features, void* workspace, size_t workspace_bytes, void* stream);
 int acx_vit_encode_r16(acx_ctx* ctx, const acx_vit_desc* d, const acx_vit_weights* w, const float* scales, const float* frames,
                        int32_t nframes, float* features, void* workspace, size_t workspace_bytes, void* stream);
+int acx_vit_encode_qkv16(acx_ctx* ctx, const acx_vit_desc* d, const acx_vit_weights* w, const float* scales, const float* frames,
+                         int32_t nframes, float* features, void* workspace, size_t workspace_bytes, void* stream);
 
 
 int acx_resnet_stem_im2col(acx_ctx* ctx, const float* frames, float* cols, int32_t F, int32_t R, void* stream);
```

New measurement: 10660 frames/s (median of 6 runs). +3.4%, better.
